# endomapper/NR-SLAM

Measured on AMD Instinct MI355X. Metric: deformable-BA LM iters/sec, higher is better.
Workload: dtype f64; 1 GPU; C2: 5000 map points x 20 keyframes, pinhole, every point a graph node; optimize(5) per step; landmarks=91749, springs=570178, dampers=512857, parallelism=1 GPU

## Files before the change

### nr-slam_amd/csrc/nrs_engine.hip

```cpp
#include <algorithm>
#include <atomic>
#include <chrono>
#include <climits>
#include <cmath>
#include <cstdlib>
#include <memory>
#include <new>
#include <system_error>
#include <thread>
#include "nrs_engine.hpp"

#include "nrs_engine_types.hpp"
#include "nrs_engine_linearize.hpp"
#include "nrs_engine_coarse.hpp"
#include "nrs_engine_pcg.hpp"
#include "nrs_engine_skin.hpp"
#include "nrs_engine_nd.hpp"
#include "nrs_engine_kft.hpp"
#include "nrs_engine_setup.hpp"
#include "nrs_engine_kft_setup.hpp"
#include "nrs_engine_devpack.hpp"

namespace nrs {

// ... 19 lines not shown
};

template <bool LIN, bool LDS>
static void launch_reg2(nrs_ctx* c, const Dev& d, const double* xl, size_t shm, int n, int cls) {
    const dim3 g(((n + 7) / 8) * 8), b(BLK);
    if constexpr (LIN && LDS) {
        if (d.plain) {
            const bool tp = d.tp_ok != 0;
            switch (d.T) {
                case 1: hipLaunchKernelGGL((k_lin_plain<1>), g, b, shm, c->stream, d, xl, cls); break;
                case 4: hipLaunchKernelGGL((k_lin_plain<4>), g, b, shm, c->stream, d, xl, cls); break;
                case 8:
                    if (tp) hipLaunchKernelGGL((k_lin_plain<8, 4, -1, true>), g, b, shm, c->stream, d, xl, cls);
                    else hipLaunchKernelGGL((k_lin_plain<8>), g, b, shm, c->stream, d, xl, cls);
                    break;
                case 16: hipLaunchKernelGGL((k_lin_plain<16>), g, b, shm, c->stream, d, xl, cls); break;
                default:
#ifdef NRS_DEBUG_PROBES
                    if (d.cam.model == 0 && tp && c->env("NRS_LIN_EXP")) {
                        switch (atoi(c->env("NRS_LIN_EXP"))) {
                            case 1: hipLaunchKernelGGL((k_lin_plain<2, 4, 0, true, 1>), g, b, shm, c->stream, d, xl, cls); break;
                            case 2: hipLaunchKernelGGL((k_lin_plain<2, 4, 0, true, 2>), g, b, shm, c->stream, d, xl, cls); break;
                            case 3: hipLaunchKernelGGL((k_lin_plain<2, 4, 0, true, 3>), g, b, shm, c->stream, d, xl, cls); break;
                            case 4: hipLaunchKernelGGL((k_lin_plain<2, 4, 0, true, 4>), g, b, shm, c->stream, d, xl, cls); break;
                            case 5: hipLaunchKernelGGL((k_lin_plain<2, 4, 0, true, 5, true>), g, b, shm, c->stream, d, xl, cls); break;
                            case 6: hipLaunchKernelGGL((k_lin_plain<2, 4, 0, true, 0, true, false, false, 4, true>), g, b, shm, c->stream, d, xl, cls); break;
                            case 7: hipLaunchKernelGGL((k_lin_plain<2, 2, 0, true, 0, true, false, false, 8>), g, b, shm, c->stream, d, xl, cls); break;
                            case 8: hipLaunchKernelGGL((k_lin_plain<2, 2, 0, true, 0, true, false, false, 10>), g, b, shm, c->stream, d, xl, cls); break;
                            case 9: hipLaunchKernelGGL((k_lin_plain<2, 3, 0, true, 0, true, false, false, 6>), g, b, shm, c->stream, d, xl, cls); break;
                            case 10: hipLaunchKernelGGL((k_lin_plain<2, 2, 0, true, 0, true, false, false, 8, true>), g, b, shm, c->stream, d, xl, cls); break;
                            default: hipLaunchKernelGGL((k_lin_plain<2, 4, 0, true, 0, true>), g, b, shm, c->stream, d, xl, cls); break;
                        }
                        break;
                    }
#endif
                    if (d.h4 && rc_of(d, cls)) {
#define NRS_LIN_RC(CAMV) switch (rc_of(d, cls)) { \
    case 1: hipLaunchKernelGGL((k_lin_plain<2, 4, CAMV, true, 0, true, true, false>), g, b, shm, c->stream, d, xl, cls); break; \
    case 2: hipLaunchKernelGGL((k_lin_plain<2, 4, CAMV, true, 0, true, false, true>), g, b, shm, c->stream, d, xl, cls); break; \
    default: hipLaunchKernelGGL((k_lin_plain<2, 4, CAMV, true, 0, true, true, true>), g, b, shm, c->stream, d, xl, cls); break; }
                        if (d.cam.model == 0) { NRS_LIN_RC(0) } else { NRS_LIN_RC(1) }
#undef NRS_LIN_RC
                    } else if (d.h4 && d.nt) {
                        if (d.cam.model == 0) hipLaunchKernelGGL((k_lin_plain<2, 4, 0, true, 0, true, false, false, 4, true>), g, b, shm, c->stream, d, xl, cls);
                        else hipLaunchKernelGGL((k_lin_plain<2, 4, 1, true, 0, true, false, false, 4, true>), g, b, shm, c->stream, d, xl, cls);
                    } else if (d.h4) {
                        if (d.cam.model == 0) hipLaunchKernelGGL((k_lin_plain<2, 4, 0, true, 0, true>), g, b, shm, c->stream, d, xl, cls);
                        else hipLaunchKernelGGL((k_lin_plain<2, 4, 1, true, 0, true>), g, b, shm, c->stream, d, xl, cls);
                    } else if (d.cam.model == 0) {
                        if (tp) hipLaunchKernelGGL((k_lin_plain<2, 4, 0, true>), g, b, shm, c->stream, d, xl, cls);
                        else hipLaunchKernelGGL((k_lin_plain<2, 4, 0, false>), g, b, shm, c->stream, d, xl, cls);
                    } else {
                        if (tp) hipLaunchKernelGGL((k_lin_plain<2, 4, 1, true>), g, b, shm, c->stream, d, xl, cls);
                        else hipLaunchKernelGGL((k_lin_plain<2, 4, 1, false>), g, b, shm, c->stream, d, xl, cls);
                    }
                    break;
            }
            return;
        }
        if (d.dform) {
            switch (d.T) {
                case 1: hipLaunchKernelGGL((k_reg<1, true, true, true>), g, b, shm, c->stream, d, xl, cls); break;
                case 4: hipLaunchKernelGGL((k_reg<4, true, true, true>), g, b, shm, c->stream, d, xl, cls); break;
                case 8: hipLaunchKernelGGL((k_reg<8, true, true, true>), g, b, shm, c->stream, d, xl, cls); break;
                case 16: hipLaunchKernelGGL((k_reg<16, true, true, true>), g, b, shm, c->stream, d, xl, cls); break;
                default: hipLaunchKernelGGL((k_reg<2, true, true, true>), g, b, shm, c->stream, d, xl, cls); break;
            }
            return;
        }
    }
    switch (d.T) {
        case 1: hipLaunchKernelGGL((k_reg<1, LIN, LDS>), g, b, shm, c->stream, d, xl, cls); break;
        case 4: hipLaunchKernelGGL((k_reg<4, LIN, LDS>), g, b, shm, c->stream, d, xl, cls); break;
        case 8: hipLaunchKernelGGL((k_reg<8, LIN, LDS>), g, b, shm, c->stream, d, xl, cls); break;
        case 16: hipLaunchKernelGGL((k_reg<16, LIN, LDS>), g, b, shm, c->stream, d, xl, cls); break;
        default: hipLaunchKernelGGL((k_reg<2, LIN, LDS>), g, b, shm, c->stream, d, xl, cls); break;
    }
}

template <bool LIN>
static void launch_reg(nrs_ctx* c, const Dev& d, const double* xl) {
    if (!d.use_lds) { launch_reg2<LIN, false>(c, d, xl, 0, d.n_regblk, 0); return; }
    for (int cls = 0; cls < 2; ++cls) {
        if (d.sh_nt[cls] == 0) continue;
        size_t shm = (LIN && d.dform) ? sizeof(double) * 9 * (size_t)(d.tile_rows + d.cap_h[cls] + 1)
                                      : sizeof(double) * 3 * (size_t)(d.tile_rows + d.cap_h[cls]) * (d.X0 ? 2 : 1);
        if (LIN) shm = std::max(shm, sizeof(double) * 4 * 64 * 8);
        launch_reg2<LIN, true>(c, d, xl, shm, d.sh_nt[cls], cls);
    }
}

template <bool LDS>
static void launch_spmv2(nrs_ctx* c, const Dev& d, double lam, size_t shm, int it) {
    const dim3 g(((d.n_regblk + 7) / 8) * 8), b(BLK);
    switch (d.T) {
        case 1: hipLaunchKernelGGL((k_spmv<1, LDS>), g, b, shm, c->stream, d, lam, it); break;
        case 4: hipLaunchKernelGGL((k_spmv<4, LDS>), g, b, shm, c->stream, d, lam, it); break;
        case 8: hipLaunchKernelGGL((k_spmv<8, LDS>), g, b, shm, c->stream, d, lam, it); break;
        case 16: hipLaunchKernelGGL((k_spmv<16, LDS>), g, b, shm, c->stream, d, lam, it); break;
        default: hipLaunchKernelGGL((k_spmv<2, LDS>), g, b, shm, c->stream, d, lam, it); break;
    }
}

static bool launch_spmv(nrs_ctx* c, const Dev& d0, double lam, int it, double tol2, bool with_skin_op = false) {
    if (!d0.use_lds) { launch_spmv2<false>(c, d0, lam, 0, it); return false; }
    bool merged = false;
    Dev d = d0;
#ifdef NRS_DEBUG_PROBES
    long long* dbg = nullptr;
    static bool dbg_done = false;
    if (d.h4 && it == 3 && !dbg_done && c->env("NRS_SPMV_DBG")) {
        dbg_done = true;
        const size_t ns = (size_t)d.n_rows / (64 / d.T);
        if (hipMalloc((void**)&dbg, sizeof(long long) * 8 * ns) == hipSuccess) { (void)hipMemsetAsync(dbg, 0, sizeof(long long) * 8 * ns, c->stream); d.dbg_clk = dbg; }
    }
    struct Dump {
        nrs_ctx* c; long long* buf; size_t ns;
        ~Dump() {
            if (!buf) return;
            (void)hipStreamSynchronize(c->stream);
            std::vector<long long> h(8 * ns);
            (void)hipMemcpy(h.data(), buf, sizeof(long long) * 8 * ns, hipMemcpyDeviceToHost);
            (void)hipFree(buf);
            double acc[5] = {0, 0, 0, 0, 0};
            long long t_min = LLONG_MAX, t_max = 0;
            size_t n = 0;
            for (size_t i = 0; i < ns; ++i) {
                const long long* q = &h[8 * i];
                if (!q[0] || !q[5]) continue;
                for (int k = 0; k < 5; ++k) acc[k] += (double)(q[k + 1] - q[k]);
                t_min = std::min(t_min, q[0]); t_max = std::max(t_max, q[5]);
                ++n;
            }
            if (n) fprintf(stderr, "[nrs] k_spmv_f phases (us per wave, mean over %zu waves): stage %.2f springs %.2f dampers %.2f row %.2f reduce %.2f | launch span %.1f us\n",
                           n, acc[0] / n / 100.0, acc[1] / n / 100.0, acc[2] / n / 100.0, acc[3] / n / 100.0, acc[4] / n / 100.0, (double)(t_max - t_min) / 100.0);
        }
    } dump{c, dbg, dbg ? (size_t)d.n_rows / (64 / d.T) : 0};
#endif
    for (int cls = 0; cls < 2; ++cls) {
        const int n = d.sh_nt[cls] + d.sh_ntb[cls];
        if (n == 0) continue;
        const dim3 g(((n + 7) / 8) * 8), b(BLK);
        if (d.dform) {
            const size_t shm = sizeof(double) * 3 * (3 * (size_t)(d.tile_rows + d.cap_h[cls] + 1) + d.tile_rows + d.cap_s[cls] + 1);
            switch (d.T) {
                case 1: hipLaunchKernelGGL((k_spmv_f<1, true>), g, b, shm, c->stream, d, lam, cls, it, tol2); break;
                case 4: hipLaunchKernelGGL((k_spmv_f<4, true>), g, b, shm, c->stream, d, lam, cls, it, tol2); break;
                case 8: hipLaunchKernelGGL((k_spmv_f<8, true>), g, b, shm, c->stream, d, lam, cls, it, tol2); break;
                case 16: hipLaunchKernelGGL((k_spmv_f<16, true>), g, b, shm, c->stream, d, lam, cls, it, tol2); break;
                default: hipLaunchKernelGGL((k_spmv_f<2, true>), g, b, shm, c->stream, d, lam, cls, it, tol2); break;
            }
            continue;
        }
        const size_t shm = sizeof(double) * 3 * (size_t)(2 * d.tile_rows + d.cap_h[cls] + ((rc_of(d, cls) & 2) ? d.cap_h[cls] : d.cap_s[cls]) + 2);
        const bool last_cls = cls == 1 || d.sh_nt[1] + d.sh_ntb[1] == 0;
        if (with_skin_op && last_cls && !(d.T == 2 && d.plain && d.tp_ok) && !c->env("NRS_SKIN_OP_OWN_LAUNCH")) {
            const dim3 g2(g.x + d.sk_nblk);
            switch (d.T) {
                case 1: hipLaunchKernelGGL((k_spmv_f_skin<1>), g2, b, shm, c->stream, d, lam, cls, it, tol2, (int)g.x); break;
                case 2: hipLaunchKernelGGL((k_spmv_f_skin<2>), g2, b, shm, c->stream, d, lam, cls, it, tol2, (int)g.x); break;
                case 4: hipLaunchKernelGGL((k_spmv_f_skin<4>), g2, b, shm, c->stream, d, lam, cls, it, tol2, (int)g.x); break;
                case 16: hipLaunchKernelGGL((k_spmv_f_skin<16>), g2, b, shm, c->stream, d, lam, cls, it, tol2, (int)g.x); break;
                default: hipLaunchKernelGGL((k_spmv_f_skin<8>), g2, b, shm, c->stream, d, lam, cls, it, tol2, (int)g.x); break;
            }
            merged = true;
            continue;
        }
        switch (d.T) {
            case 1: hipLaunchKernelGGL((k_spmv_f<1, false>), g, b, shm, c->stream, d, lam, cls, it, tol2); break;
            case 4: hipLaunchKernelGGL((k_spmv_f<4, false>), g, b, shm, c->stream, d, lam, cls, it, tol2); break;
            case 8: hipLaunchKernelGGL((k_spmv_f<8, false>), g, b, shm, c->stream, d, lam, cls, it, tol2); break;
            case 16: hipLaunchKernelGGL((k_spmv_f<16, false>), g, b, shm, c->stream, d, lam, cls, it, tol2); break;
            default:
                if (d.plain && d.tp_ok && d.h4 && rc_of(d, cls) == 1) hipLaunchKernelGGL((k_spmv_f<2, false, true, true, true, false>), g, b, shm, c->stream, d, lam, cls, it, tol2);
                else if (d.plain && d.tp_ok && d.h4 && rc_of(d, cls) == 2) hipLaunchKernelGGL((k_spmv_f<2, false, true, true, false, true>), g, b, shm, c->stream, d, lam, cls, it, tol2);
                else if (d.plain && d.tp_ok && d.h4 && rc_of(d, cls) == 3) hipLaunchKernelGGL((k_spmv_f<2, false, true, true, true, true>), g, b, shm, c->stream, d, lam, cls, it, tol2);
                else if (d.plain && d.tp_ok && d.h4 && d.nt) hipLaunchKernelGGL((k_spmv_f<2, false, true, true, false, false, true>), g, b, shm, c->stream, d, lam, cls, it, tol2);
                else if (d.plain && d.tp_ok && d.h4) hipLaunchKernelGGL((k_spmv_f<2, false, true, true>), g, b, shm, c->stream, d, lam, cls, it, tol2);
                else if (d.plain && d.tp_ok) hipLaunchKernelGGL((k_spmv_f<2, false, true>), g, b, shm, c->stream, d, lam, cls, it, tol2);
                else hipLaunchKernelGGL((k_spmv_f<2, false>), g, b, shm, c->stream, d, lam, cls, it, tol2);
                break;
        }
    }
    return merged;
}

template <bool LIN>
static int evaluate(nrs_ctx* c, Engine* e, int which, bool reproj_done = false) {
    if (LIN) { e->d.lin_pose = e->d.pose[which]; e->d.lin_xl = e->d.xl[which]; }
    const Dev& d = e->d;
    const dim3 gg(((d.sh_ng + 7) / 8) * 8), b(BLK);
#ifdef NRS_DEBUG_PROBES
    if (LIN && d.plain && c->env("NRS_LIN_DBG")) {
        static bool done = false;
        if (!done) {
            done = true;
            const size_t ns = (size_t)d.n_rows / (64 / d.T);
            long long* buf = nullptr;
            NRS_HIP(c, hipMalloc((void**)&buf, sizeof(long long) * 8 * ns));
            NRS_HIP(c, hipMemsetAsync(buf, 0, sizeof(long long) * 8 * ns, c->stream));
            Dev dd = d;
            dd.dbg_clk = buf;
            launch_reg<LIN>(c, dd, d.xl[which]);
            NRS_HIP(c, hipStreamSynchronize(c->stream));
            std::vector<long long> h(8 * ns);
            NRS_HIP(c, hipMemcpy(h.data(), buf, sizeof(long long) * 8 * ns, hipMemcpyDeviceToHost));
            (void)hipFree(buf);
            double acc[5] = {0, 0, 0, 0, 0};
            long long t_min = LLONG_MAX, t_max = 0;
            size_t n = 0;
            for (size_t i = 0; i < ns; ++i) {
                const long long* q = &h[8 * i];
                if (!q[0] || !q[5]) continue;
                for (int k = 0; k < 5; ++k) acc[k] += (double)(q[k + 1] - q[k]);
                t_min = std::min(t_min, q[0]); t_max = std::max(t_max, q[5]);
                ++n;
            }
            fprintf(stderr, "[nrs] k_lin_plain phases (us per wave, mean over %zu waves): stage %.2f springs %.2f dampers %.2f reproj %.2f tail %.2f | launch span %.1f us\n",
                    n, acc[0] / n / 100.0, acc[1] / n / 100.0, acc[2] / n / 100.0, acc[3] / n / 100.0, acc[4] / n / 100.0, (double)(t_max - t_min) / 100.0);
        }
    }
#endif
    if (LIN) {
        const int reps = c->opt.profile ? PROFILE_REPS : 1;
        Timer t(c, &c->prof.linearize_ms, &c->prof.linearize_launches, reps);
        for (int r = 0; r < reps; ++r) {
            if (!d.use_lds) hipLaunchKernelGGL((k_reproj<LIN>), gg, b, 0, c->stream, d, d.pose[which], d.xl[which]);
            launch_reg<LIN>(c, d, d.xl[which]);
        }
    } else {
        if (!reproj_done) hipLaunchKernelGGL((k_reproj<LIN>), gg, b, 0, c->stream, d, d.pose[which], d.xl[which]);
        if (d.ec_on) hipLaunchKernelGGL(k_chi_edges, dim3(std::max(1, d.ec_nblk)), b, 0, c->stream, d, d.xl[which]);
        else launch_reg<LIN>(c, d, d.xl[which]);
    }
    if (LIN) hipLaunchKernelGGL(k_pose_sums, dim3(d.sh_nk), b, 0, c->stream, d);
    if (LIN && d.coarse && !(e->nd && e->nd->on)) {
        const size_t rows = (size_t)(d.tile_rows + d.max_halo);
        const size_t shm = sizeof(double) * 3 * rows + 3 * (rows + 8) + 16;
        const dim3 g(d.n_regblk);
        switch (d.T) {
            case 1: hipLaunchKernelGGL((k_coarse_tile<1>), g, b, shm, c->stream, d); break;
            case 2: hipLaunchKernelGGL((k_coarse_tile<2>), g, b, shm, c->stream, d); break;
            case 4: hipLaunchKernelGGL((k_coarse_tile<4>), g, b, shm, c->stream, d); break;
            case 16: hipLaunchKernelGGL((k_coarse_tile<16>), g, b, shm, c->stream, d); break;
            default: hipLaunchKernelGGL((k_coarse_tile<8>), g, b, shm, c->stream, d); break;
        }
        hipLaunchKernelGGL(k_coarse_reduce, dim3(1), b, 0, c->stream, d);
    }
    if (d.sk_n > 0) hipLaunchKernelGGL((k_skin<LIN>), dim3(d.sk_nblk), b, 0, c->stream, d, d.pose[which], d.xl[which]);
    if (LIN && d.sk_pcg) {
        if (d.D_op) NRS_HIP(c, hipMemcpyAsync(d.D_op, d.D, sizeof(double) * 6 * (size_t)d.n_rows, hipMemcpyDeviceToDevice, c->stream));
        if (d.sk_nrl > 0) hipLaunchKernelGGL(k_skin_rows, dim3((d.sk_nrl + SK_RPB - 1) / SK_RPB), b, 0, c->stream, d);
        hipLaunchKernelGGL(k_skin_pose, dim3((27 * d.sh_nk + BLK - 1) / BLK), b, 0, c->stream, d);
    }
    if (LIN && e->nd && e->nd->on) {
        const NdVals& nv = e->nd->slot->vals;
        if (nv.ske_ptr) hipLaunchKernelGGL(k_nd_values<true>, dim3((nv.n_ent * ND_SKL + 255) / 256), dim3(256), 0, c->stream, d, nv);
        else hipLaunchKernelGGL(k_nd_values<false>, dim3((nv.n_ent + 255) / 256), dim3(256), 0, c->stream, d, nv);
    }
    if (d.sh_on) {
        hipLaunchKernelGGL((k_finalize_pack<LIN>), dim3(1), b, 0, c->stream, d);
        NRS_HIP(c, hipGetLastError());
        NRS_TRY(c->comm->allreduce(c, d.pk_loc, d.pk, (size_t)(2 + d.sh_world + (LIN ? 27 * d.K : 0))));
        hipLaunchKernelGGL((k_finalize_unpack<LIN>), dim3(1), b, 0, c->stream, d, ++c->seq);
    } else {
        hipLaunchKernelGGL((k_finalize<LIN>), dim3(1), b, 0, c->stream, d, ++c->seq, (e->nd && e->nd->on) ? 1 : 0);
    }
    NRS_HIP(c, hipGetLastError());
    return NRS_OK;
}

static int wait_published(nrs_ctx* c, Engine* e) {
    volatile int* w = e->h_flags + 7;
    const auto t0 = std::chrono::steady_clock::now();
    for (uint64_t spins = 0; *w != c->seq; ++spins) {
        if (spins > 200000) std::this_thread::yield();
        if ((spins & 0xFFFF) == 0xFFFF && std::chrono::steady_clock::now() - t0 > std::chrono::seconds(2)) {
            NRS_HIP(c, hipStreamSynchronize(c->stream));
            if (*w != c->seq) return c->fail(NRS_ERR_HIP, "device results were not published");
            break;
        }
    }
    std::atomic_thread_fence(std::memory_order_acquire);
    return NRS_OK;
}

static int read_scalars(nrs_ctx* c, Engine* e) { return wait_published(c, e); }

static int wait_published_at(nrs_ctx* c, const int* hf, int seq, hipStream_t st) {
    const volatile int* w = hf + 7;
    const auto t0 = std::chrono::steady_clock::now();
    for (uint64_t spins = 0; *w != seq; ++spins) {
        if (spins > 200000) std::this_thread::yield();
        if ((spins & 0xFFFF) == 0xFFFF && std::chrono::steady_clock::now() - t0 > std::chrono::seconds(2)) {
            NRS_HIP(c, hipStreamSynchronize(st));
            if (*w != seq) return c->fail(NRS_ERR_HIP, "device results were not published");
            break;
        }
    }
    std::atomic_thread_fence(std::memory_order_acquire);
    return NRS_OK;
}

static int direct_trial_enqueue(nrs_ctx* c, Engine* e, int set, double lam, int* seq, int* solve_id, bool in_batch) {
    Dev& d = e->d;
    const int cur = e->cur, trial = 1 - e->cur;
    const dim3 g(((d.sh_ng + 7) / 8) * 8), b(BLK);
    if (set < 0) {
        NRS_TRY(nd_solve_enqueue(c, e->nd->S(), lam, nullptr, solve_id, nullptr, in_batch ? c->spec_back[0] : nullptr));
        hipLaunchKernelGGL(k_apply_reproj, g, b, 0, c->stream, d, lam, d.pose[cur], d.xl[cur], d.pose[trial], d.xl[trial]);
        NRS_TRY(evaluate<false>(c, e, trial, true));
        *seq = c->seq;
        return NRS_OK;
    }
    const SpecSet& q = e->spec[set];
    struct Restore {
        nrs_ctx* c; Engine* e; Dev saved; hipStream_t main;
        ~Restore() { e->d = saved; c->stream = main; }
    } restore{c, e, d, c->stream};
    d.xv = q.xv; d.xp = q.xp; d.part_apply = q.part_apply; d.part_rchi = q.part_rchi; d.part_reg = q.part_reg; d.scal = q.scal; d.flags = q.flags;
    d.h_scal = q.h_scal; d.h_flags = q.h_flags;
    if (d.sk_n > 0) { d.sk_part = q.sk_part; d.sk_chi = q.sk_chi; }
    d.pose[trial] = q.pose; d.xl[trial] = q.xl;
    c->stream = c->spec_stream[set];
    NRS_HIP(c, hipStreamWaitEvent(c->stream, c->spec_fork, 0));
    NdDev nd = nd_alt_dev(e->nd->S(), set);
    nd.out_rows = q.xv; nd.out_pose = q.xp; nd.flags = q.flags; nd.abort = q.abort;
    NRS_TRY(nd_solve_enqueue(c, e->nd->S(), lam, &nd, solve_id, c->spec_back[set], c->spec_back[set + 1]));
    hipLaunchKernelGGL(k_apply_reproj, g, b, 0, c->stream, d, lam, d.pose[cur], d.xl[cur], q.pose, q.xl);
    NRS_TRY(evaluate<false>(c, e, trial, true));
    *seq = c->seq;
    NRS_HIP(c, hipEventRecord(c->spec_join[set], c->stream));
    return NRS_OK;
}

struct PcgSetView {
    nrs_ctx* c; Engine* e; Dev saved; hipStream_t main; double* hs; int* hf; bool on;
    PcgSetView(nrs_ctx* c_, Engine* e_, int set, int abort_id)
        : c(c_), e(e_), saved(e_->d), main(c_->stream), hs(e_->h_scal), hf(e_->h_flags), on(set >= 0) {
        if (!on) return;
        const SpecSet& q = e->spec[set];
        Dev& d = e->d;
        d.xv = q.xv; d.rv = q.rv; d.uv3 = q.uv3; d.pv = q.pv; d.sv = q.sv; d.wv = q.wv; d.Dinv = q.Dinv; d.Hppinv = q.Hppinv;
        d.xp = q.xp; d.rp = q.rp; d.rp2 = q.rp2; d.up = q.up; d.up2 = q.up2; d.pp = q.pp; d.sp = q.sp;
        d.part_spmv = q.part_spmv; d.part_ru = q.part_ru; d.red = q.red; d.part_ec = q.part_ec;
        d.part_apply = q.part_apply; d.part_rchi = q.part_rchi; d.part_reg = q.part_reg; d.scal = q.scal; d.flags = q.flags;
        d.h_scal = q.h_scal; d.h_flags = q.h_flags;
        d.pose[1 - e->cur] = q.pose; d.xl[1 - e->cur] = q.xl;
        d.abort = q.abort; d.abort_id = abort_id;
        e->h_scal = q.h_scal; e->h_flags = q.h_flags;
        c->stream = c->spec_stream[set];
    }
    ~PcgSetView() { if (on) { e->d = saved; c->stream = main; e->h_scal = hs; e->h_flags = hf; } }
    PcgSetView(const PcgSetView&) = delete;
    PcgSetView& operator=(const PcgSetView&) = delete;
};

constexpr double PEEK_RTOL = 1e-1;
constexpr int PEEK_LEVELS = 4;
constexpr double PEEK_MIN_REL_INCREASE = 1e-5;
constexpr double PEEK_RHO_LVL[5] = {0, -1.0, -0.25, -0.1, -0.03};

static int pcg_begin(nrs_ctx* c, Engine* e, double lam, int* it) {
    const Dev& d = e->d;
    NRS_HIP(c, hipMemsetAsync(d.flags, 0, sizeof(int) * 8, c->stream));
    if (d.coarse) hipLaunchKernelGGL(k_coarse_invert, dim3(1), dim3(BLK), sizeof(double) * (size_t)d.co_n * d.co_n, c->stream, d, lam);
    hipLaunchKernelGGL(k_trial_setup, dim3(d.sh_nvb), dim3(BLK), 0, c->stream, d, lam);
    if (e->kft && e->kft->on) {
        NRS_TRY(kft_factor(c, e, e->kft, lam));
        NRS_TRY(kft_apply(c, e->kft, d.rv, d.rp, d.uv3, d.up, d.flags));
        e->kft->apply_pending = false;
    }
    *it = 0;
    return NRS_OK;
}

static int pcg_enqueue_batch(nrs_ctx* c, Engine* e, double lam, int* it_io, int count = 0, int pub_seq = 0) {
    const Dev& d = e->d;
    const int n_poseblk = (d.K + 3) / 4;
    const double tol2 = c->opt.pcg_rtol * c->opt.pcg_rtol;
    int it = *it_io;
    int stop = std::min(it + (c->opt.profile ? 1 : count > 0 ? count : c->opt.pcg_batch), c->opt.pcg_max_iters);
    const bool kft_on = e->kft && e->kft->on;
    const bool kft_lazy = kft_on && it == 0 && stop > 0 && !c->opt.profile && !c->env("NRS_KFT_NO_RESIDUAL_TEST");
    if (kft_lazy) stop = 1;
    if (kft_on && e->kft->apply_pending) {
        NRS_TRY(kft_apply(c, e->kft, d.rv, ((it - 1) & 1) ? d.rp : d.rp2, d.uv3, ((it - 1) & 1) ? d.up : d.up2, d.flags));
        e->kft->apply_pending = false;
    }
    for (; it < stop; ++it) {
        const int pub = it + 1 == stop && !kft_lazy ? pub_seq : 0;
#ifdef NRS_DEBUG_PROBES
        if (d.fused && it == 20 && d.coarse && c->env("NRS_PCG_DBG")) {
            static bool dbg_done = false;
            if (!dbg_done) {
                dbg_done = true;
                long long* buf = nullptr;
                const size_t nb8 = 8 * (size_t)d.n_regblk;
                if (hipMalloc((void**)&buf, sizeof(long long) * nb8) == hipSuccess) {
                    (void)hipMemsetAsync(buf, 0, sizeof(long long) * nb8, c->stream);
                    Dev dd = d;
                    dd.dbg_clk = buf;
                    const dim3 g(((d.n_regblk + 7) / 8) * 8), bb(BLK);
                    const size_t shm = sizeof(double) * (6 * (size_t)(d.tile_rows + d.max_halo) + 12 * (size_t)d.n_regblk + 16 * CO_MAX);
                    (void)hipStreamSynchronize(c->stream);
                    std::vector<long long> h(nb8);
                    hipLaunchKernelGGL((k_pcg_fused<8, true>), g, bb, shm, c->stream, dd, lam, it, tol2, PEEK_RTOL * PEEK_RTOL, pub);
                    (void)hipStreamSynchronize(c->stream);
                    (void)hipMemcpy(h.data(), buf, sizeof(long long) * nb8, hipMemcpyDeviceToHost);
                    (void)hipFree(buf);
                    double acc[6] = {0, 0, 0, 0, 0, 0};
                    long long t_min = LLONG_MAX, t_max = 0;
                    int n = 0;
                    for (int b2 = 0; b2 < d.n_regblk; ++b2) {
                        const long long* q = &h[8 * (size_t)b2];
                        if (!q[0] || !q[6]) continue;
                        for (int k = 0; k < 6; ++k) acc[k] += (double)(q[k + 1] - q[k]);
                        t_min = std::min(t_min, q[0]); t_max = std::max(t_max, q[6]);
                        ++n;
                    }
                    if (n) fprintf(stderr, "[nrs] k_pcg_fused<8,true> phases (us per tile, mean over %d tiles): loads+pose %.2f coarse products %.2f scalars+corrections %.2f update+stage %.2f operator %.2f reduce+store %.2f | launch span %.1f us\n",
                                   n, acc[0] / n / 100.0, acc[1] / n / 100.0, acc[2] / n / 100.0, acc[3] / n / 100.0, acc[4] / n / 100.0, acc[5] / n / 100.0, (double)(t_max - t_min) / 100.0);
                    continue;
                }
            }
        }
#endif
        if (d.fused) {
            const bool one_xcd_off = c->env("NRS_NO_ONE_XCD") != nullptr;
            const bool one_xcd = !one_xcd_off && d.n_regblk <= 32;
            Dev d1 = d;
            d1.one_xcd = one_xcd ? 1 : 0;
            const Dev& d = d1;
            const dim3 g(one_xcd ? 8 * d.n_regblk : ((d.n_regblk + 7) / 8) * 8), bb(BLK);
            const size_t shm = sizeof(double) * (6 * (size_t)(d.tile_rows + d.max_halo) + (d.coarse ? 12 * (size_t)d.n_regblk + 16 * CO_MAX : 0));
            const bool check_fused = c->env("NRS_CHECK_FUSED") != nullptr;
            if (check_fused && !d.coarse && d.T == 8) {
                struct Arr { void* p; size_t bytes; const char* name; };
                const size_t nv = sizeof(double) * 3 * (size_t)d.n_rows, np6 = sizeof(double) * 6 * (size_t)d.K, npart = sizeof(double) * NPART * (size_t)d.n_regblk;
                const Arr arr[] = {{d.rv, nv, "r0"}, {d.rv2, nv, "r1"}, {d.sv, nv, "s0"}, {d.sv2, nv, "s1"}, {d.wv, nv, "w0"}, {d.wv2, nv, "w1"}, {d.xv, nv, "x"},
                                   {d.pv, nv, "p"}, {d.uv3, nv, "u"}, {d.rp, np6, "rp0"}, {d.rp2, np6, "rp1"}, {d.sp, np6, "sp0"}, {d.sp2, np6, "sp1"},
                                   {d.up, np6, "up0"}, {d.up2, np6, "up1"}, {d.pp, np6, "pp"}, {d.xp, np6, "xp"}, {d.part_spmv, npart, "part0"},
                                   {d.part_spmv2, npart, "part1"}, {d.scal, sizeof(double) * SC_N, "scal"}, {d.flags, sizeof(int) * 8, "flags"}};
                size_t total = 0;
                for (const Arr& a : arr) total += (a.bytes + 255) & ~(size_t)255;
                static char* snap = nullptr; static size_t snap_cap = 0;
                if (snap_cap < total) { if (snap) (void)hipFree(snap); NRS_HIP(c, hipMalloc((void**)&snap, total)); snap_cap = total; }
                std::vector<char> h1(total), h2(total);
                auto gather = [&](char* dst, hipMemcpyKind kind) -> int {
                    size_t o = 0;
                    for (const Arr& a : arr) { NRS_HIP(c, hipMemcpyAsync(dst + o, a.p, a.bytes, kind, c->stream)); o += (a.bytes + 255) & ~(size_t)255; }
                    NRS_HIP(c, hipStreamSynchronize(c->stream));
                    return NRS_OK;
                };
                NRS_TRY(gather(snap, hipMemcpyDeviceToDevice));
                hipLaunchKernelGGL((k_pcg_fused<8, false>), g, bb, shm, c->stream, d, lam, it, tol2, PEEK_RTOL * PEEK_RTOL, pub);
                NRS_TRY(gather(h1.data(), hipMemcpyDeviceToHost));
                { size_t o = 0; for (const Arr& a : arr) { NRS_HIP(c, hipMemcpyAsync(a.p, snap + o, a.bytes, hipMemcpyDeviceToDevice, c->stream)); o += (a.bytes + 255) & ~(size_t)255; } }
                hipLaunchKernelGGL((k_pcg_fused<8, false>), g, bb, shm, c->stream, d, lam, it, tol2, PEEK_RTOL * PEEK_RTOL, pub);
                NRS_TRY(gather(h2.data(), hipMemcpyDeviceToHost));
                size_t o = 0;
                bool any = false;
                for (const Arr& a : arr) {
                    if (memcmp(h1.data() + o, h2.data() + o, a.bytes) != 0) {
                        any = true;
                        const size_t nel = a.bytes / 8;
                        size_t ndiff = 0, first = 0, last = 0;
                        for (size_t el = 0; el < nel; ++el)
                            if (memcmp(h1.data() + o + 8 * el, h2.data() + o + 8 * el, 8) != 0) { if (!ndiff) first = el; last = el; ++ndiff; }
                        double v1, v2; memcpy(&v1, h1.data() + o + 8 * first, 8); memcpy(&v2, h2.data() + o + 8 * first, 8);
                        fprintf(stderr, "[nrs] fused launch it %d: array %s differs in %zu elements, first %zu (tile %zu) last %zu (tile %zu): %.6g / %.6g\n", it, a.name, ndiff, first,
                                first / 3 / (size_t)d.tile_rows, last, last / 3 / (size_t)d.tile_rows, v1, v2);
                    }
                    o += (a.bytes + 255) & ~(size_t)255;
                }
                if (any) {
                    const size_t o_fl = total - 256, o_sc = o_fl - ((sizeof(double) * SC_N + 255) & ~(size_t)255);
                    const int* f1 = reinterpret_cast<const int*>(h1.data() + o_fl); const int* f2 = reinterpret_cast<const int*>(h2.data() + o_fl);
                    const int* f0 = nullptr; (void)f0;
                    fprintf(stderr, "[nrs]    flags after run 1: %d %d %d %d | run 2: %d %d %d %d ; scal gamma0 %.6g/%.6g slot0 %.6g %.6g / %.6g %.6g slot1 %.6g %.6g / %.6g %.6g\n", f1[0], f1[1], f1[2], f1[3], f2[0], f2[1], f2[2], f2[3],
                            reinterpret_cast<const double*>(h1.data() + o_sc)[SC_GAMMA0], reinterpret_cast<const double*>(h2.data() + o_sc)[SC_GAMMA0],
                            reinterpret_cast<const double*>(h1.data() + o_sc)[SC_SLOT0], reinterpret_cast<const double*>(h1.data() + o_sc)[SC_SLOT0 + 1],
                            reinterpret_cast<const double*>(h2.data() + o_sc)[SC_SLOT0], reinterpret_cast<const double*>(h2.data() + o_sc)[SC_SLOT0 + 1],
                            reinterpret_cast<const double*>(h1.data() + o_sc)[SC_SLOT1], reinterpret_cast<const double*>(h1.data() + o_sc)[SC_SLOT1 + 1],
                            reinterpret_cast<const double*>(h2.data() + o_sc)[SC_SLOT1], reinterpret_cast<const double*>(h2.data() + o_sc)[SC_SLOT1 + 1]);
                }
            } else
            switch (d.T) {
                case 1: if (d.coarse) hipLaunchKernelGGL((k_pcg_fused<1, true>), g, bb, shm, c->stream, d, lam, it, tol2, PEEK_RTOL * PEEK_RTOL, pub);
                        else hipLaunchKernelGGL((k_pcg_fused<1, false>), g, bb, shm, c->stream, d, lam, it, tol2, PEEK_RTOL * PEEK_RTOL, pub);
                        break;
                case 2: if (d.coarse) hipLaunchKernelGGL((k_pcg_fused<2, true>), g, bb, shm, c->stream, d, lam, it, tol2, PEEK_RTOL * PEEK_RTOL, pub);
                        else hipLaunchKernelGGL((k_pcg_fused<2, false>), g, bb, shm, c->stream, d, lam, it, tol2, PEEK_RTOL * PEEK_RTOL, pub);
                        break;
                case 4: if (d.coarse) hipLaunchKernelGGL((k_pcg_fused<4, true>), g, bb, shm, c->stream, d, lam, it, tol2, PEEK_RTOL * PEEK_RTOL, pub);
                        else hipLaunchKernelGGL((k_pcg_fused<4, false>), g, bb, shm, c->stream, d, lam, it, tol2, PEEK_RTOL * PEEK_RTOL, pub);
// ... 539 lines not shown
```

### nr-slam_amd/csrc/nrs_engine_devpack.hpp

```cpp
#pragma once
#include <rocprim/rocprim.hpp>

namespace nrs {

constexpr int DP_HCAP = 2048, DP_HASH = 4096;

__device__ inline uint64_t dp_spread(uint64_t v) {
    v &= 0x1fffff;
    v = (v | v << 32) & 0x1f00000000ffffULL;
    v = (v | v << 16) & 0x1f0000ff0000ffULL;
    v = (v | v << 8) & 0x100f00f00f00f00fULL;
    v = (v | v << 4) & 0x10c30c30c30c30c3ULL;
    v = (v | v << 2) & 0x1249249249249249ULL;
    return v;
}

__global__ __launch_bounds__(1024) void k_dp_minmax(int M, const double* __restrict__ xyz, double* out ) {
    __shared__ double lo[3][1024], hi[3][1024];
    const int tid = threadIdx.x;
    double l[3] = {1e300, 1e300, 1e300}, h[3] = {-1e300, -1e300, -1e300};
    for (int v = tid; v < M; v += 1024)
        for (int a = 0; a < 3; ++a) { const double p = xyz[3 * (size_t)v + a]; l[a] = fmin(l[a], p); h[a] = fmax(h[a], p); }
    for (int a = 0; a < 3; ++a) { lo[a][tid] = l[a]; hi[a][tid] = h[a]; }
    __syncthreads();
// ... 562 lines not shown
    NRS_HIP(c, hipMemsetAsync(S_side, 0, nnz_s, st));
    NRS_HIP(c, hipMemsetAsync(D_o, 0xFF, sizeof(int) * 3 * nnz_d, st));
    NRS_HIP(c, hipMemsetAsync(D_role, 0xFF, nnz_d, st));
    NRS_HIP(c, hipMemsetAsync(d_flag, 0, sizeof(int) * 16, st));
    NRS_HIP(c, hipMemsetAsync(t_d0, 0, sizeof(float) * nnz_s, st));
    NRS_HIP(c, hipMemsetAsync(t_w, 0, sizeof(float) * nnz_d, st));
    hipLaunchKernelGGL(k_dp_fill_s, nb(ni_s), dim3(256), 0, st, ni_s, T, key_s2, rs_s, d_ss, r_sp, r_d0, vrow, S_other, t_d0, S_side);
    hipLaunchKernelGGL(k_dp_fill_d, nb(ni_d), dim3(256), 0, st, ni_d, T, key_d2, rs_d, d_sd, r_dm, r_w, vrow, D_o, t_w, D_role);
    hipLaunchKernelGGL((k_dp_halo<0>), dim3(n_tiles), dim3(256), 0, st, d.tile_rows, T, (uint16_t*)nullptr, d_ss, d_sd, S_other, S_side, D_o, D_role, hs, hns, (const int*)nullptr,
                       (int*)nullptr, (uint32_t*)nullptr, (uint2*)nullptr, d_flag);
    std::vector<int> h_hs(n_tiles), h_hns(n_tiles), h_vrow(M);
    int h_flag = 0;
    NRS_HIP(c, hipMemcpyAsync(h_hs.data(), hs, sizeof(int) * n_tiles, hipMemcpyDeviceToHost, st));
    NRS_HIP(c, hipMemcpyAsync(h_hns.data(), hns, sizeof(int) * n_tiles, hipMemcpyDeviceToHost, st));
    NRS_HIP(c, hipMemcpyAsync(&h_flag, d_flag, sizeof(int), hipMemcpyDeviceToHost, st));
    NRS_HIP(c, hipMemcpyAsync(h_vrow.data(), vrow, sizeof(int) * (size_t)M, hipMemcpyDeviceToHost, st));
    NRS_HIP(c, hipStreamSynchronize(st));
    mark("fill + halo sizes");
    if (h_flag) return NRS_OK;
    std::vector<int> halo_ptr(n_tiles + 1, 0), tile_list(n_tiles);
    d.max_halo = 0; d.max_halo_s = 0;
    for (int b = 0; b < n_tiles; ++b) {
        halo_ptr[b + 1] = halo_ptr[b] + h_hs[b];
        d.max_halo = std::max(d.max_halo, h_hs[b]);
        d.max_halo_s = std::max(d.max_halo_s, h_hns[b]);
    }
    const size_t n_halo = (size_t)halo_ptr[n_tiles];
    {
        std::vector<int> sorted = h_hs;
        std::sort(sorted.begin(), sorted.end());
        int cut = d.max_halo;
        if (n_tiles >= 1024) {
            const int p97 = sorted[(size_t)(0.97 * (n_tiles - 1))];
            const bool fits = sizeof(double) * 3 * (size_t)(2 * d.tile_rows + d.max_halo + d.max_halo_s + 2) <= 48 * 1024;
            if (4 * d.max_halo > 5 * p97 && (n_tiles - (int)(0.97 * n_tiles) >= 1024 || !fits) && !c->env("NRS_ONE_CLASS")) cut = p97;
        }
        int n0 = 0;
        for (int b = 0; b < n_tiles; ++b) if (h_hs[b] <= cut) tile_list[n0++] = b;
        int n1 = n0;
        for (int b = 0; b < n_tiles; ++b) if (h_hs[b] > cut) tile_list[n1++] = b;
        d.n_tiles_cls[0] = n0; d.n_tiles_cls[1] = n_tiles - n0;
        for (int b = 0; b < n_tiles; ++b) {
            const int cls = h_hs[b] <= cut ? 0 : 1;
            d.cap_h[cls] = std::max(d.cap_h[cls], h_hs[b]);
            d.cap_s[cls] = std::max(d.cap_s[cls], h_hns[b]);
        }
    }
    size_t lds_need = 0;
    for (int cls = 0; cls < 2; ++cls) {
        if (!d.n_tiles_cls[cls]) continue;
        lds_need = std::max(lds_need, sizeof(double) * 3 * (size_t)(d.tile_rows + d.cap_h[cls]));
        lds_need = std::max(lds_need, sizeof(double) * 3 * (size_t)(2 * d.tile_rows + d.cap_h[cls] + d.cap_s[cls] + 2));
    }
    if (lds_need > 64 * 1024 - 512 || d.tile_rows + d.max_halo >= 65535) return NRS_OK;
    d.use_lds = 1; d.dform = 0; d.coarse = 0;
    d.fused = d.n_rows < 32768 ? 1 : 0;
    d.hier = n_tiles > 4096 ? 1 : 0;
    d.ecd = (!d.fused && !c->opt.profile) ? 1 : 0;
    d.co_n = 3 * d.n_groups + 6;
    d.sh_on = 0; d.sh_rank = 0; d.sh_world = 1; d.sh_lead = 1;
    d.sh_k0 = 0; d.sh_nk = K; d.sh_g0 = 0; d.sh_ng = d.n_groups; d.sh_vb0 = 0; d.sh_nvb = d.n_vecblk;
    for (int cls = 0; cls < 2; ++cls) { d.sh_t0[cls] = 0; d.sh_nt[cls] = d.n_tiles_cls[cls]; }
    d.ec_on = 1; d.plain = 1;
    d.lin_rb = ROW_ALIGN / (64 / T);
    d.ec_nsp = n_sp; d.ec_ndm = n_dm;
    d.ec_nblk = std::min((n_sp + n_dm + BLK - 1) / BLK, 2048);
    e->pack_rows = n_rows;
    if (tm) fprintf(stderr, "[nrs] device pack: tiles %d x %d rows, halo rows: max %d, mean %.1f, spring part max %d, classes %d (cap %d/%d) + %d (cap %d/%d)\n", n_tiles, d.tile_rows,
                    d.max_halo, (double)n_halo / n_tiles, d.max_halo_s, d.n_tiles_cls[0], d.cap_h[0], d.cap_s[0], d.n_tiles_cls[1], d.cap_h[1], d.cap_s[1]);
    ArenaPlan dry{arena, true};
    {
        Dev tmpd = d;
        Engine te;
        spec_pcg_sets(c, e, 0);
        te.n_spec = e->n_spec; te.spec_pcg = e->spec_pcg;
        carve(dry, tmpd, false, nnz_s, nnz_d, (size_t)n_slices, n_halo, &te);
    }
    if (dry.off > arena->cap) {
        arena_release(arena);
        const size_t want = dry.off + dry.off / 8;
        hipError_t he = hipMalloc((void**)&arena->base, want);
        if (he != hipSuccess) return c->fail(NRS_ERR_ALLOC, "hipMalloc(%zu) failed: %s", want, hipGetErrorString(he));
        arena->cap = want;
        if (c->env("NRS_POISON")) { (void)hipMemset(arena->base, 0xFF, want); (void)hipDeviceSynchronize(); }
    }
    ArenaPlan real{arena, false};
    carve(real, d, false, nnz_s, nnz_d, (size_t)n_slices, n_halo, e);
    e->arena_bytes = real.off;
    mark("arena");
    NRS_HIP(c, hipMemcpyAsync(d.grp_pose, grp_pose.data(), sizeof(int) * grp_pose.size(), hipMemcpyHostToDevice, st));
    NRS_HIP(c, hipMemcpyAsync(d.pose_grp_ptr, pose_grp_ptr.data(), sizeof(int) * (K + 1), hipMemcpyHostToDevice, st));
    NRS_HIP(c, hipMemcpyAsync(d.halo_ptr, halo_ptr.data(), sizeof(int) * (n_tiles + 1), hipMemcpyHostToDevice, st));
    NRS_HIP(c, hipMemcpyAsync(d.tile_list, tile_list.data(), sizeof(int) * n_tiles, hipMemcpyHostToDevice, st));
    NRS_HIP(c, hipMemcpyAsync(d.halo_ns, hns, sizeof(int) * n_tiles, hipMemcpyDeviceToDevice, st));
    NRS_HIP(c, hipMemcpyAsync(d.ss_ptr, d_ss, sizeof(int) * ((size_t)n_slices + 1), hipMemcpyDeviceToDevice, st));
    NRS_HIP(c, hipMemcpyAsync(d.sd_ptr, d_sd, sizeof(int) * ((size_t)n_slices + 1), hipMemcpyDeviceToDevice, st));
    NRS_HIP(c, hipMemcpyAsync(d.s_d0, t_d0, sizeof(float) * nnz_s, hipMemcpyDeviceToDevice, st));
    NRS_HIP(c, hipMemcpyAsync(d.d_w, t_w, sizeof(float) * nnz_d, hipMemcpyDeviceToDevice, st));
    std::vector<Pose> poses(s.poses, s.poses + K);
    NRS_HIP(c, hipMemcpyAsync(d.pose_init, poses.data(), sizeof(Pose) * K, hipMemcpyHostToDevice, st));
    NRS_HIP(c, hipMemsetAsync(d.pose_fixed, 0, K, st));
    NRS_HIP(c, hipMemsetAsync(d.row_tp, 0xFF, sizeof(uint32_t) * (size_t)n_rows, st));
    hipLaunchKernelGGL((k_dp_halo<1>), dim3(n_tiles), dim3(256), 0, st, d.tile_rows, T, reinterpret_cast<uint16_t*>(d.row_tp), d.ss_ptr, d.sd_ptr, S_other, S_side, D_o, D_role, hs, hns, d.halo_ptr,
                       d.halo_rows, d.s_om, d.d_hdr, d_flag);
    if (d.fused) {
        std::vector<int> tile_desc(8 * (size_t)n_tiles, 0);
        const int rb = ROW_ALIGN / d.tile_rows;
        for (int b = 0; b < n_tiles; ++b) {
            const int kf = grp_pose[(size_t)b * d.tile_rows / ROW_ALIGN];
            int* td = &tile_desc[8 * (size_t)b];
            td[0] = kf; td[1] = pose_grp_ptr[kf] * rb; td[2] = pose_grp_ptr[kf + 1] * rb;
            td[3] = halo_ptr[b]; td[4] = halo_ptr[b + 1] - halo_ptr[b];
        }
        NRS_HIP(c, hipMemcpyAsync(d.tile_desc, tile_desc.data(), sizeof(int) * tile_desc.size(), hipMemcpyHostToDevice, st));
        hipLaunchKernelGGL(k_dp_halofix, dim3(n_tiles), dim3(BLK), 0, st, n_tiles, d.halo_ptr, d.halo_rows, d.halo_fix, BLK, 0);
        NRS_HIP(c, hipStreamSynchronize(st));
    } else if (d.use_lds)
        hipLaunchKernelGGL(k_dp_halofix, dim3(n_tiles), dim3(BLK), 0, st, n_tiles, d.halo_ptr, d.halo_rows, d.halo_fix, HALO_FIX, -1);
    hipLaunchKernelGGL(k_dp_rowdata, nb(n_rows), dim3(256), 0, st, n_rows, row_v, r_x, r_uv, d.rflag, d.uv, d.xl_init);
    hipLaunchKernelGGL(k_dp_rowcnt, nb(n_rows), dim3(256), 0, st, n_rows, cnt_s, cnt_d, d.row_cnt);
    hipLaunchKernelGGL(k_dp_eckeys, nb(std::max(n_sp, n_dm)), dim3(256), 0, st, n_sp, r_sp, n_dm, r_dm, vrow, ek_s, ek_d);
    tb = tmp_bytes; NRS_HIP(c, rocprim::radix_sort_keys(tmp, tb, ek_s, ek_s2, (size_t)n_sp, 0, 32 + row_bits, st));
    tb = tmp_bytes; NRS_HIP(c, rocprim::radix_sort_keys(tmp, tb, ek_d, ek_d2, (size_t)n_dm, 0, 32 + row_bits, st));
    hipLaunchKernelGGL(k_dp_ecfill, nb(std::max(n_sp, n_dm)), dim3(256), 0, st, n_sp, ek_s2, r_sp, r_d0, n_dm, ek_d2, r_dm, r_w, vrow, d.ec_sp, d.ec_dm, d.ec_w);
    NRS_HIP(c, hipMemsetAsync(d.s_qc, 0, sizeof(double) * nnz_s, st));
    NRS_HIP(c, hipMemsetAsync(d.d_s, 0, sizeof(double) * nnz_d, st));
    NRS_HIP(c, hipMemsetAsync(d.part_apply, 0, sizeof(double) * (size_t)d.n_vecblk, st));
    NRS_HIP(c, hipMemsetAsync(d.scal, 0, sizeof(double) * SC_N, st));
    NRS_HIP(c, hipMemsetAsync(d.flags, 0, sizeof(int) * 8, st));
    NRS_HIP(c, hipGetLastError());
    e->vrow.swap(h_vrow);
    e->h_rflag.assign(n_rows, RF_FIXED);
    for (int v = 0; v < M; ++v) e->h_rflag[e->vrow[v]] = RF_OBS | RF_REPROJ_ACTIVE;
    e->h_pose_fixed.assign(K, 0);
    e->dev_edges = true;
    e->raw_sp = r_sp; e->raw_d0 = r_d0; e->raw_dm = r_dm; e->raw_w = r_w;
    e->serial = ++c->engine_serial;
    if (!c->pin_scal) NRS_HIP(c, hipHostMalloc((void**)&c->pin_scal, sizeof(double) * SC_N, hipHostMallocMapped | hipHostMallocCoherent));
    if (!c->pin_flags) {
        NRS_HIP(c, hipHostMalloc((void**)&c->pin_flags, sizeof(int) * 8, hipHostMallocMapped | hipHostMallocCoherent));
        memset(c->pin_flags, 0, sizeof(int) * 8);
    }
    e->h_scal = c->pin_scal; e->h_flags = c->pin_flags;
    d.h_scal = c->pin_scal; d.h_flags = c->pin_flags;
    if (e->n_spec > 0) NRS_TRY(spec_prepare(c, e));
    NRS_HIP(c, hipStreamSynchronize(st));
    int h_fl2[2] = {0, 0};
    NRS_HIP(c, hipMemcpy(h_fl2, d_flag, sizeof(int) * 2, hipMemcpyDeviceToHost));
    if (h_fl2[0]) return c->fail(NRS_ERR_HIP, "device pack: halo hash overflow in the second pass");
    d.tp_ok = h_fl2[1] ? 0 : 1;
    if (c->pack_ws2.cap > ((size_t)512 << 20)) c->release(c->pack_ws2);
    mark("final arrays");
    engine_compact_headers(c, e);
    NRS_TRY(engine_reset(c, e));
    *done = true;
    return NRS_OK;
}

}
```

### nr-slam_amd/csrc/nrs_engine_linearize.hpp

```cpp
#pragma once

namespace nrs {

template <bool LIN>
__global__ __launch_bounds__(BLK) void k_reproj(Dev P, const Pose* __restrict__ poses,
                                                const double* __restrict__ xl) {
    __shared__ double lds[4 * 28];
    const int gi = xcd_tile(blockIdx.x, P.sh_ng);
    if (gi >= P.sh_ng) return;
    const int g = P.sh_g0 + gi;
    const int tid = threadIdx.x, lane = tid & 63, wave = tid >> 6;
    const int row = g * ROW_ALIGN + tid;
    const int kf = P.grp_pose[g];
    const Pose Tcw = poses[kf];
    const bool pfix = P.pose_fixed[kf] != 0;
    double R[9];
    quat_to_R(Tcw.q, R);
    double acc[28];
#pragma unroll
    for (int k = 0; k < 28; ++k) acc[k] = 0;
    const int rf = P.rflag[row];
    const bool rfix = (rf & RF_FIXED) != 0;
    const bool active = (rf & RF_OBS) && (rf & RF_REPROJ_ACTIVE) && !(pfix && rfix);
    bool wrote = false;
// ... 430 lines not shown
            double* Dr = P.D + 6 * (size_t)row;
            double dd[6];
            if (LDS) {
#pragma unroll
                for (int k = 0; k < 6; ++k) { dd[k] = D[k]; Dr[k] = dd[k]; }
#pragma unroll
                for (int k = 0; k < 3; ++k) P.bl[3 * row + k] = bb[k];
            } else {
#pragma unroll
                for (int k = 0; k < 6; ++k) { dd[k] = Dr[k] + D[k]; Dr[k] = dd[k]; }
#pragma unroll
                for (int k = 0; k < 3; ++k) P.bl[3 * row + k] += bb[k];
            }
            part[1] = fmax(fabs(dd[0]), fmax(fabs(dd[3]), fabs(dd[5])));
        }
    }
    double c = wave_sum(part[0]);
    double m = part[1];
#pragma unroll
    for (int off = 32; off > 0; off >>= 1) m = fmax(m, __shfl_xor(m, off, 64));
    if (lane == 0) { lds[wave * 2] = c; lds[wave * 2 + 1] = m; }
    __syncthreads();
    if (tid == 0) {
        P.part_reg[2 * (size_t)b] = lds[0] + lds[2] + lds[4] + lds[6];
        P.part_reg[2 * (size_t)b + 1] = fmax(fmax(lds[1], lds[3]), fmax(lds[5], lds[7]));
    }
}

__device__ inline double fast_rcp_pos(double a) {
    double y = __builtin_amdgcn_rcp(a);
    double e = fma(-a, y, 1.0);
    y = fma(y, e, y);
    e = fma(-a, y, 1.0);
    return fma(y, e, y);
}
__device__ inline double fast_rsqrt_pos(double a) {
    const double y = __builtin_amdgcn_rsq(a);
    const double e = fma(-a * y, y, 1.0);
    return fma(y * e, fma(e, 0.375, 0.5), y);
}
__device__ inline double fast_sqrt_pos(double a) {
    const double y = __builtin_amdgcn_rsq(a);
    double g = a * y, h = 0.5 * y;
    const double e = fma(-h, g, 0.5);
    g = fma(g, e, g);
    h = fma(h, e, h);
    const double e2 = fma(-g, g, a);
    return fma(e2, h, g);
}

__device__ inline double sq3(double a, double b, double c) { return fma(c, c, fma(b, b, a * a)); }
__device__ inline double spring_qc(double d2, double d0, double ks, double ip) {
#pragma clang fp contract(off)
    const double c = 2.0 * ks * fast_rcp_pos(d0);
    return ip * (c * c) * fast_rsqrt_pos(d2);
}
__device__ inline double damper_s(double g0, double g1, double g2, double w, double isp, double dsp, double& rho0) {
#pragma clang fp contract(off)
    const double r0 = w * g0, r1 = w * g1, r2 = w * g2;
    const double e = isp * sq3(r0, r1, r2), dsqr = dsp * dsp;
    const bool act = dsp > 0 && e > dsqr;
    const double ea = act ? e : 1.0, y = fast_rsqrt_pos(ea);
    rho0 = act ? 2.0 * (ea * y) * dsp - dsqr : e;
    return (act ? dsp * y : 1.0) * isp * w * w;
}

template <int T, int OCC = 4, int CAM = -1, bool TPC = false, int EXP = 0, bool H4 = false, bool RCS = false, bool RCD = false, int NBT = 4, bool NT = false>
__global__ __launch_bounds__(BLK, OCC) void k_lin_plain(Dev P, const double* __restrict__ xl_g, int cls) {
    __shared__ double mfb[4 * 128];
    __shared__ double spose[8];
    extern __shared__ double dyn[];
    constexpr int R = 64 / T;
    int b = xcd_tile(blockIdx.x, P.sh_nt[cls]);
    if (b >= P.sh_nt[cls]) return;
    b = P.tile_list[(cls ? P.n_tiles_cls[0] : 0) + P.sh_t0[cls] + b];
    const int tid = threadIdx.x, lane = tid & 63, wave = __builtin_amdgcn_readfirstlane(tid >> 6);
    const int slice = b * 4 + wave;
    const int row = slice * R + lane / T;
    const int t = lane % T;
    auto stamp = [&](int k) { if (P.dbg_clk && lane == 0) P.dbg_clk[(size_t)slice * 8 + k] = wall_clock64(); };
    stamp(0);
    const uint32_t rcn = P.row_cnt[row];
    const int my_s = ((int)(rcn & 0xFFFFu) + T - 1 - t) / T, my_d = ((int)(rcn >> 16) + T - 1 - t) / T;
    if (tid < 7) spose[tid] = reinterpret_cast<const double*>(P.lin_pose + P.grp_pose[row / ROW_ALIGN])[tid];
    const int s_beg = P.ss_ptr[slice], s_end = P.ss_ptr[slice + 1];
    const int d_beg = P.sd_ptr[slice], d_end = EXP == 5 ? P.sd_ptr[slice] + (((P.sd_ptr[slice + 1] - P.sd_ptr[slice]) / 64 + 1) / 2) * 64 : P.sd_ptr[slice + 1];
    constexpr int NB = NBT;
    uint32_t rs_om[NB], rs_d0[NB];
    auto req_s = [&](int q, int idx) {
        if (EXP == 3) { rs_om[q] = (uint32_t)(idx & 63) | 0x10000u; rs_d0[q] = 0x3F800000u; return; }
        rs_om[q] = 0xFFFFu; rs_d0[q] = 0x3F800000u;
        if ((idx - s_beg - lane) / 64 < my_s) {
            if (NT) { rs_om[q] = __builtin_nontemporal_load(P.s_om + idx); rs_d0[q] = __float_as_uint(__builtin_nontemporal_load(P.s_d0 + idx)); }
            else { rs_om[q] = P.s_om[idx]; rs_d0[q] = __float_as_uint(P.s_d0[idx]); }
        }
    };
#pragma unroll
    for (int q = 0; q < NB; ++q) req_s(q, s_beg + lane + 64 * q);
    __builtin_amdgcn_sched_barrier(0);
    double* lx = dyn;
    if (P.fused) stage_rows(P, b, tid, xl_g, nullptr, lx);
    else stage_rows<true>(P, b, tid, xl_g, nullptr, lx);
    __syncthreads();
    stamp(1);
    const int self = row - b * P.tile_rows;
    const double xo0 = lx[3 * self], xo1 = lx[3 * self + 1], xo2 = lx[3 * self + 2];
    double D0 = 0, D1 = 0, D2 = 0, D3 = 0, D4 = 0, D5 = 0, bb0 = 0, bb1 = 0, bb2 = 0, chi = 0;
    const double ks = P.k_spring, ip = P.info_pos;
    auto do_s = [&](int o16, bool live, bool count, float d0f, int idx) {
        const bool pad = !live || o16 == REC_NONE;
        const int o = EXP == 2 ? self : (pad ? self : o16) & 0xFFFF;
        const double v0 = xo0 - lx[3 * o], v1 = xo1 - lx[3 * o + 1], v2 = xo2 - lx[3 * o + 2];
        double d2 = sq3(v0, v1, v2);
        d2 = pad ? 1.0 : d2;
        const double d0 = pad ? 1.0 : (double)d0f;
        const double rs = fast_rsqrt_pos(d2), id0 = fast_rcp_pos(d0);
        const double r = ks * fma(d2, rs, -d0) * id0;
        const double cg = 2.0 * ks * id0 * fast_sqrt_pos(rs);
        const double qc = pad ? 0.0 : spring_qc(d2, d0, ks, ip);
        if (live && EXP != 1 && !RCS) { if (NT) __builtin_nontemporal_store(qc, P.s_qc + idx); else P.s_qc[idx] = qc; }
        chi += count && !pad ? ip * r * r : 0.0;
        const double t0 = qc * v0, t1 = qc * v1, t2 = qc * v2;
        D0 = fma(t0, v0, D0); D1 = fma(t0, v1, D1); D2 = fma(t0, v2, D2);
        D3 = fma(t1, v1, D3); D4 = fma(t1, v2, D4); D5 = fma(t2, v2, D5);
        const double qr = ip * r * cg;
        bb0 = fma(-qr, v0, bb0); bb1 = fma(-qr, v1, bb1); bb2 = fma(-qr, v2, bb2);
    };
    for (int ub = s_beg; ub < (EXP == 4 ? s_beg : s_end); ub += 64 * NB) {
        const int base = ub + lane;
        if (ub != s_beg) {
#pragma unroll
            for (int q = 0; q < NB; ++q) req_s(q, base + 64 * q);
        }
        __builtin_amdgcn_sched_barrier(0);
#pragma unroll
        for (int q = 0; q < NB; ++q) {
            const uint32_t om = consume(rs_om[q]);
            const float d0f = __uint_as_float(consume(rs_d0[q]));
            do_s((int)(om & 0xFFFFu), base + 64 * q < s_end, (om & ((uint32_t)SR_COUNT << 16)) != 0, d0f, base + 64 * q);
        }
        __builtin_amdgcn_sched_barrier(0);
    }
    stamp(2);
    double en0 = 0, en1 = 0, en2 = 0, ep0 = 0, ep1 = 0, ep2 = 0;
    if (TPC) {
        const uint32_t tp = P.row_tp[row];
        const int tn = (int)(tp & 0xFFFFu) == REC_NONE ? self : (int)(tp & 0xFFFFu), tq = (int)(tp >> 16) == REC_NONE ? self : (int)(tp >> 16);
        en0 = xo0 - lx[3 * tn]; en1 = xo1 - lx[3 * tn + 1]; en2 = xo2 - lx[3 * tn + 2];
        ep0 = xo0 - lx[3 * tq]; ep1 = xo1 - lx[3 * tq + 1]; ep2 = xo2 - lx[3 * tq + 2];
    }
    const double isp = P.info_spatial, dsp = P.delta_spatial;
    uint32_t rd_w[NB];
    uint2 rd_h[NB];
    auto req_d = [&](int q, int idx) {
        if (EXP == 3) { rd_h[q] = make_uint2((uint32_t)(idx & 63) | ((uint32_t)((idx + 1) & 63) << 16), (uint32_t)((idx + 2) & 63) | 0x80000u); rd_w[q] = 0x3F800000u; return; }
        rd_h[q] = make_uint2(0xFFFFFFFFu, 0xFFFFFFFFu); rd_w[q] = 0u;
        if (H4) { if ((idx - d_beg - lane) / 64 < my_d) {
            if (NT) { rd_h[q].x = __builtin_nontemporal_load(P.d_h4 + idx); rd_w[q] = __float_as_uint(__builtin_nontemporal_load(P.d_w + idx)); }
            else { rd_h[q].x = P.d_h4[idx]; rd_w[q] = __float_as_uint(P.d_w[idx]); } } }
        else if ((idx - d_beg - lane) / 64 < my_d) { rd_h[q] = P.d_hdr[idx]; rd_w[q] = __float_as_uint(P.d_w[idx]); }
    };
    auto do_d = [&](uint32_t hx, uint32_t hy, float wf, int idx) {
        const uint32_t m16 = H4 ? (hx == 0xFFFFFFFFu ? (uint32_t)REC_NONE : hx >> 24) : hy >> 16;
        const bool live = idx < d_end;
        const bool pad = !live || m16 == REC_NONE;
        const int o0 = EXP == 2 ? self : (pad ? self : (int)(hx & (H4 ? 0xFFFu : 0xFFFFu))) & 0xFFFF, o1 = EXP == 2 || H4 ? self : (pad ? self : (int)(hx >> 16)) & 0xFFFF,
                  o2 = EXP == 2 ? self : (pad ? self : (int)(H4 ? (hx >> 12) & 0xFFFu : hy & 0xFFFFu)) & 0xFFFF;
        double g0, g1, g2;
        if (TPC) {
            const bool fwd = (m16 & 2u) == 0;
            g0 = (fwd ? en0 : ep0) - (lx[3 * o0] - lx[3 * o2]);
            g1 = (fwd ? en1 : ep1) - (lx[3 * o0 + 1] - lx[3 * o2 + 1]);
            g2 = (fwd ? en2 : ep2) - (lx[3 * o0 + 2] - lx[3 * o2 + 2]);
        } else {
            g0 = (xo0 - lx[3 * o1]) - (lx[3 * o0] - lx[3 * o2]);
            g1 = (xo1 - lx[3 * o1 + 1]) - (lx[3 * o0 + 1] - lx[3 * o2 + 1]);
            g2 = (xo2 - lx[3 * o1 + 2]) - (lx[3 * o0 + 2] - lx[3 * o2 + 2]);
        }
        const double w = pad ? 0.0 : (double)wf;
        double rho0;
        const double sfac = damper_s(g0, g1, g2, w, isp, dsp, rho0);
        chi += (m16 & DM_COUNT) ? rho0 : 0.0;
        if (live && EXP != 1 && !RCD) { if (NT) __builtin_nontemporal_store(sfac, P.d_s + idx); else P.d_s[idx] = sfac; }
        D0 += sfac; D3 += sfac; D5 += sfac;
        bb0 = fma(-sfac, g0, bb0); bb1 = fma(-sfac, g1, bb1); bb2 = fma(-sfac, g2, bb2);
    };
    for (int ub = d_beg; ub < (EXP == 4 ? d_beg : d_end); ub += 64 * NB) {
        const int base = ub + lane;
#pragma unroll
        for (int q = 0; q < NB; ++q) req_d(q, base + 64 * q);
        __builtin_amdgcn_sched_barrier(0);
#pragma unroll
        for (int q = 0; q < NB; ++q) {
            const uint32_t hx = consume(rd_h[q].x), hy = H4 ? 0u : consume(rd_h[q].y);
            const float wf = __uint_as_float(consume(rd_w[q]));
            do_d(hx, hy, wf, base + 64 * q);
        }
        __builtin_amdgcn_sched_barrier(0);
    }
    stamp(3);
    constexpr int NRR = T == 1 ? 2 : 1;
    const int rf = P.rflag[row];
    const float uvx = P.uv[2 * row], uvy = P.uv[2 * row + 1];
    const bool active = (rf & RF_OBS) && (rf & RF_REPROJ_ACTIVE);
    RowRec rc;
#pragma unroll
    for (int q = 0; q < 6; ++q) rc.J[q] = 0.f;
    rc.w = 0;
    double Jp[NRR][6], rres[NRR], w = 0, chi_r = 0;
#pragma unroll
    for (int a = 0; a < NRR; ++a) {
        rres[a] = 0;
#pragma unroll
        for (int q = 0; q < 6; ++q) Jp[a][q] = 0;
    }
    if (active && t < (T == 1 ? 1 : 2)) {
        Pose Tcw;
#pragma unroll
        for (int q = 0; q < 4; ++q) Tcw.q[q] = spose[q];
#pragma unroll
        for (int q = 0; q < 3; ++q) Tcw.t[q] = spose[4 + q];
        double Rm[9];
        quat_to_R(Tcw.q, Rm);
        const double px = Rm[0] * xo0 + Rm[1] * xo1 + Rm[2] * xo2 + Tcw.t[0];
        const double py = Rm[3] * xo0 + Rm[4] * xo1 + Rm[5] * xo2 + Tcw.t[1];
        const double pz = Rm[6] * xo0 + Rm[7] * xo1 + Rm[8] * xo2 + Tcw.t[2];
        float u, v, Jf[6];
        Cam cam = P.cam;
        if (CAM >= 0) cam.model = CAM;
        project_f32(cam, (float)px, (float)py, (float)pz, u, v);
        projection_jacobian_f32(cam, (float)px, (float)py, (float)pz, Jf);
        const double r2[2] = {(double)uvx - (double)u, (double)uvy - (double)v};
        double rho0, rho1;
        huber(P.info_reproj * (r2[0] * r2[0] + r2[1] * r2[1]), P.delta_reproj, rho0, rho1);
        if (t == 0) chi_r = rho0;
        w = rho1 * P.info_reproj;
#pragma unroll
        for (int a = 0; a < NRR; ++a) {
            const int rr = T == 1 ? a : t;
            const double j0 = -(double)(rr ? Jf[3] : Jf[0]), j1 = -(double)(rr ? Jf[4] : Jf[1]), j2 = -(double)(rr ? Jf[5] : Jf[2]);
            const double r = rr ? r2[1] : r2[0];
            rres[a] = r;
            Jp[a][0] = -j1 * pz + j2 * py;
            Jp[a][1] = j0 * pz - j2 * px;
            Jp[a][2] = -j0 * py + j1 * px;
            Jp[a][3] = j0; Jp[a][4] = j1; Jp[a][5] = j2;
            const double Jl0 = j0 * Rm[0] + j1 * Rm[3] + j2 * Rm[6];
            const double Jl1 = j0 * Rm[1] + j1 * Rm[4] + j2 * Rm[7];
            const double Jl2 = j0 * Rm[2] + j1 * Rm[5] + j2 * Rm[8];
            D0 += w * (Jl0 * Jl0); D1 += w * (Jl0 * Jl1); D2 += w * (Jl0 * Jl2);
            D3 += w * (Jl1 * Jl1); D4 += w * (Jl1 * Jl2); D5 += w * (Jl2 * Jl2);
            bb0 -= w * (Jl0 * r); bb1 -= w * (Jl1 * r); bb2 -= w * (Jl2 * r);
        }
        if (t == 0) {
#pragma unroll
            for (int q = 0; q < 6; ++q) rc.J[q] = Jf[q];
            rc.w = w;
        }
    }
    if (t == 0) P.rowrec[row] = rc;
    stamp(4);
    double* slot = P.part_lin + (size_t)slice * 32;
    {
        typedef double v4d __attribute__((ext_vector_type(4)));
        double* mb = mfb + wave * 128;
        const int e = lane & 15, kk = lane >> 4;
        v4d acc = {0.0, 0.0, 0.0, 0.0};
#pragma unroll
        for (int a = 0; a < NRR; ++a) {
#pragma unroll
            for (int c4 = 0; c4 < 4; ++c4) {
                __builtin_amdgcn_fence(__ATOMIC_ACQ_REL, "wavefront");
                __builtin_amdgcn_wave_barrier();
                if (kk == c4) {
#pragma unroll
                    for (int q = 0; q < 6; ++q) mb[e * 8 + q] = Jp[a][q];
                    mb[e * 8 + 6] = -rres[a];
                    mb[e * 8 + 7] = w;
                }
                __builtin_amdgcn_fence(__ATOMIC_RELEASE, "wavefront");
                __builtin_amdgcn_wave_barrier();
                __builtin_amdgcn_fence(__ATOMIC_ACQUIRE, "wavefront");
#pragma unroll
                for (int m = 0; m < 4; ++m) {
                    const int kq = 4 * m + kk;
                    const double val = e < 7 ? mb[kq * 8 + e] : 0.0;
                    const double av = e < 6 ? mb[kq * 8 + 7] * val : 0.0;
                    acc = __builtin_amdgcn_mfma_f64_16x16x4f64(av, val, acc, 0, 0, 0);
                }
            }
        }
        auto put = [&](int prow, double c) {
            if (prow < 6) {
                if (e >= prow && e < 6) slot[prow * 6 - (prow * (prow - 1)) / 2 + (e - prow)] = c;
                if (e == 6) slot[21 + prow] = c;
            }
        };
        put(kk, acc.x);
        put(4 + kk, acc.y);
    }
    D0 = sub_sum_t<T>(D0); D1 = sub_sum_t<T>(D1); D2 = sub_sum_t<T>(D2);
    D3 = sub_sum_t<T>(D3); D4 = sub_sum_t<T>(D4); D5 = sub_sum_t<T>(D5);
    bb0 = sub_sum_t<T>(bb0); bb1 = sub_sum_t<T>(bb1); bb2 = sub_sum_t<T>(bb2);
    double md = 0;
    if (t == 0) {
        double* Dr = P.D + 6 * (size_t)row;
        Dr[0] = D0; Dr[1] = D1; Dr[2] = D2; Dr[3] = D3; Dr[4] = D4; Dr[5] = D5;
        P.bl[3 * row] = bb0; P.bl[3 * row + 1] = bb1; P.bl[3 * row + 2] = bb2;
        md = fmax(fabs(D0), fmax(fabs(D3), fabs(D5)));
    }
    const double cr = wave_sum(chi_r), cg2 = wave_sum(chi);
#pragma unroll
    for (int off = 32; off > 0; off >>= 1) md = fmax(md, __shfl_xor(md, off, 64));
    if (lane == 0) { slot[27] = cr; slot[28] = cg2; slot[29] = md; }
    stamp(5);
}

__global__ __launch_bounds__(BLK) void k_chi_edges(Dev P, const double* __restrict__ xl) {
    __shared__ double lds[4];
    if (spec_aborted(P)) return;
    const int tid = threadIdx.x, n = P.ec_nsp + P.ec_ndm;
    const int per = (int)((((int64_t)n + P.ec_nblk - 1) / P.ec_nblk + BLK - 1) / BLK) * BLK;
    const int64_t beg = (int64_t)blockIdx.x * per;
    const int end = (int)(beg + per < n ? beg + per : n);
    double rho[1] = {0};
    for (int i = (int)beg + tid; i < end; i += BLK) {
        double r0v, rho1;
        if (i < P.ec_nsp) {
            const EcSpring s = P.ec_sp[i];
            const double v0 = xl[3 * (size_t)s.a] - xl[3 * (size_t)s.b], v1 = xl[3 * (size_t)s.a + 1] - xl[3 * (size_t)s.b + 1],
                         v2 = xl[3 * (size_t)s.a + 2] - xl[3 * (size_t)s.b + 2];
            const double d = sqrt(v0 * v0 + v1 * v1 + v2 * v2), d0 = (double)s.d0;
            const double r = P.k_spring * (d - d0) / d0;
            huber(P.info_pos * r * r, P.delta_pos, r0v, rho1);
        } else {
            const EcDamper dd = P.ec_dm[i - P.ec_nsp];
            const double w = (double)P.ec_w[i - P.ec_nsp];
            double s0 = 0, s1 = 0, s2 = 0;
#pragma unroll
            for (int k = 0; k < 4; ++k) {
                if (dd.r[k] >= 0) {
                    const double sg = damper_sign(k);
                    s0 += sg * xl[3 * (size_t)dd.r[k]]; s1 += sg * xl[3 * (size_t)dd.r[k] + 1]; s2 += sg * xl[3 * (size_t)dd.r[k] + 2];
                }
            }
            const double r0 = w * s0, r1 = w * s1, r2 = w * s2;
            huber(P.info_spatial * (r0 * r0 + r1 * r1 + r2 * r2), P.delta_spatial, r0v, rho1);
        }
        rho[0] += r0v;
// ... 165 lines not shown
```

### nr-slam_amd/csrc/nrs_engine_pcg.hpp

```cpp
#pragma once

namespace nrs {

__device__ inline bool inv6_spd(const double* Hu, double lam, double* Ainv ) {
    double L[6][6];
    double A[6][6];
    int k = 0;
    for (int i = 0; i < 6; ++i)
        for (int j = i; j < 6; ++j) { A[i][j] = Hu[k]; A[j][i] = Hu[k]; ++k; }
    for (int i = 0; i < 6; ++i) A[i][i] += lam;
    for (int i = 0; i < 6; ++i)
        for (int j = 0; j < 6; ++j) L[i][j] = 0;
    bool ok = true;
    for (int j = 0; j < 6; ++j) {
        double d = A[j][j];
        for (int q = 0; q < j; ++q) d -= L[j][q] * L[j][q];
        if (!(d > 0)) { ok = false; d = 1; }
        const double l = sqrt(d);
        L[j][j] = l;
        for (int i = j + 1; i < 6; ++i) {
            double s = A[i][j];
            for (int q = 0; q < j; ++q) s -= L[i][q] * L[j][q];
            L[i][j] = s / l;
        }
    }
    for (int c = 0; c < 6; ++c) {
        double y[6], x[6];
        for (int i = 0; i < 6; ++i) {
            double s = (i == c) ? 1.0 : 0.0;
            for (int q = 0; q < i; ++q) s -= L[i][q] * y[q];
            y[i] = s / L[i][i];
        }
        for (int i = 5; i >= 0; --i) {
            double s = y[i];
            for (int q = i + 1; q < 6; ++q) s -= L[q][i] * x[q];
            x[i] = s / L[i][i];
        }
        for (int i = 0; i < 6; ++i) Ainv[i * 6 + c] = x[i];
    }
    return ok;
}

__global__ __launch_bounds__(BLK) void k_trial_setup(Dev P, double lam) {
    __shared__ double lds_ru[4];
    if (spec_aborted(P)) return;
    const int i = (P.sh_vb0 + blockIdx.x) * BLK + threadIdx.x;
    double ru[1] = {0};
    if (i < P.n_rows) {
        double Di[6];
        const bool ok = inv3_sym(P.D + 6 * (size_t)i, lam, Di);
        if (!ok || !isfinite(Di[0])) P.flags[2] = 1;
#pragma unroll
        for (int k = 0; k < 6; ++k) P.Dinv[6 * (size_t)i + k] = Di[k];
        const double r0 = P.bl[3 * i], r1 = P.bl[3 * i + 1], r2 = P.bl[3 * i + 2];
        P.rv[3 * i] = r0; P.rv[3 * i + 1] = r1; P.rv[3 * i + 2] = r2;
        double y0 = 0, y1 = 0, y2 = 0;
        if (P.coarse && !(P.rflag[i] & RF_FIXED)) {
            const int g = i / ROW_ALIGN, tl = i / P.tile_rows;
            double yt[3];
            tile_level(P.co_bti + 6 * (size_t)tl, P.co_tb + 4 * (size_t)tl, yt);
            y0 = P.co_y0[3 * g] + yt[0]; y1 = P.co_y0[3 * g + 1] + yt[1]; y2 = P.co_y0[3 * g + 2] + yt[2];
        }
        const double u0 = Di[0] * r0 + Di[1] * r1 + Di[2] * r2 + y0;
        const double u1 = Di[1] * r0 + Di[3] * r1 + Di[4] * r2 + y1;
        const double u2 = Di[2] * r0 + Di[4] * r1 + Di[5] * r2 + y2;
        P.uv3[3 * i] = u0; P.uv3[3 * i + 1] = u1; P.uv3[3 * i + 2] = u2;
        ru[0] = r0 * u0 + r1 * u1 + r2 * u2;
#pragma unroll
        for (int k = 0; k < 3; ++k) { P.xv[3 * i + k] = 0; P.pv[3 * i + k] = 0; P.sv[3 * i + k] = 0; }
    }
    if (blockIdx.x * BLK + threadIdx.x < P.K) {
        const int i = blockIdx.x * BLK + threadIdx.x;
        double Ai[36];
        if (!inv6_spd(P.Hpp + 21 * i, lam, Ai)) P.flags[2] = 1;
        for (int k = 0; k < 36; ++k) P.Hppinv[36 * i + k] = Ai[k];
        for (int a = 0; a < 6; ++a) {
            double s = 0;
            for (int c = 0; c < 6; ++c) s += Ai[a * 6 + c] * P.bp[6 * i + c];
            if (P.coarse && !P.pose_fixed[i]) s += P.co_y0[3 * P.n_groups + a];
            P.up[6 * i + a] = s;
            P.rp[6 * i + a] = P.bp[6 * i + a];
            P.xp[6 * i + a] = 0; P.pp[6 * i + a] = 0; P.sp[6 * i + a] = 0;
        }
    }
    if (P.ecd) {
        block_sum<1>(ru, lds_ru, threadIdx.x & 63, threadIdx.x >> 6);
        if (threadIdx.x == 0) P.part_ru[P.sh_vb0 + blockIdx.x] = ru[0];
    }
}

template <int T, bool LDS>
__global__ __launch_bounds__(BLK) void k_spmv(Dev P, double lam, int it) {
    static_assert(!LDS, "gather fallback only: the LDS-staged path is k_spmv_f");
    __shared__ double lds[4 * 9];
    constexpr int R = 64 / T;
    const int b = xcd_tile(blockIdx.x, P.n_regblk);
    if (b >= P.n_regblk) return;
    const int tid = threadIdx.x, lane = tid & 63, wave = tid >> 6;
    const int slice = b * 4 + wave;
    const int row = slice * R + lane / T;
    const int t = lane % T;
    const bool rfix = (P.rflag[row] & RF_FIXED) != 0;
    const double* u = P.uv3;
    const int self = row;
    double a0 = 0, a1 = 0, a2 = 0;
    double part[9] = {0, 0, 0, 0, 0, 0, 0, 0, 0};
    const double ul0 = u[3 * self], ul1 = u[3 * self + 1], ul2 = u[3 * self + 2];
    {
        const int kf = P.grp_pose[row / ROW_ALIGN];
        if (t == 0) {
            const double* D = (P.D_op ? P.D_op : P.D) + 6 * (size_t)row;
            a0 = (D[0] + lam) * ul0 + D[1] * ul1 + D[2] * ul2;
            a1 = D[1] * ul0 + (D[3] + lam) * ul1 + D[4] * ul2;
            a2 = D[2] * ul0 + D[4] * ul1 + (D[5] + lam) * ul2;
        }
        double h0 = 0, h1 = 0, h2 = 0;
#pragma unroll
        for (int p = t; p < 6; p += T) {
            const double upk = ((it & 1) ? P.up2 : P.up)[6 * kf + p];
            const double e0 = P.Hpl[(size_t)(p * 3) * P.n_rows + row];
            const double e1 = P.Hpl[(size_t)(p * 3 + 1) * P.n_rows + row];
            const double e2 = P.Hpl[(size_t)(p * 3 + 2) * P.n_rows + row];
            h0 += e0 * upk; h1 += e1 * upk; h2 += e2 * upk;
            part[3 + p] = e0 * ul0 + e1 * ul1 + e2 * ul2;
        }
        a0 += h0; a1 += h1; a2 += h2;
        part[2] = ul0 * h0 + ul1 * h1 + ul2 * h2;
    }
    if (!rfix) {
        const int beg = P.ss_ptr[slice], end = P.ss_ptr[slice + 1];
        const size_t nz = (size_t)P.ss_nnz;
        for (int idx = beg + lane; idx < end; idx += 64) {
            const int o = P.s_other[idx];
            if (o < 0) continue;
            const double g0 = P.s_g[idx], g1 = P.s_g[nz + idx], g2 = P.s_g[2 * nz + idx];
            const double dot = g0 * u[3 * o] + g1 * u[3 * o + 1] + g2 * u[3 * o + 2];
            a0 -= g0 * dot; a1 -= g1 * dot; a2 -= g2 * dot;
        }
    }
    if (!rfix) {
        const int beg = P.sd_ptr[slice], end = P.sd_ptr[slice + 1];
        for (int idx = beg + lane; idx < end; idx += 64) {
            const int meta = P.d_meta[idx];
            if (meta < 0 || (meta & DM_UNARY)) continue;
            const int o[3] = {P.d_o0[idx], P.d_o1[idx], P.d_o2[idx]};
            const int role = meta & 3;
            double s0 = 0, s1 = 0, s2 = 0;
#pragma unroll
            for (int k = 0; k < 3; ++k) {
                const double sg = damper_sign(k + (k >= role ? 1 : 0));
                if (o[k] >= 0) { s0 += sg * u[3 * o[k]]; s1 += sg * u[3 * o[k] + 1]; s2 += sg * u[3 * o[k] + 2]; }
            }
            const double c = damper_sign(role) * P.d_s[idx];
            a0 += c * s0; a1 += c * s1; a2 += c * s2;
        }
    }
    a0 = sub_sum_t<T>(a0); a1 = sub_sum_t<T>(a1); a2 = sub_sum_t<T>(a2);
    if (t == 0) {
        P.wv[3 * row] = a0; P.wv[3 * row + 1] = a1; P.wv[3 * row + 2] = a2;
        part[0] = P.rv[3 * row] * ul0 + P.rv[3 * row + 1] * ul1 + P.rv[3 * row + 2] * ul2;
        part[1] = a0 * ul0 + a1 * ul1 + a2 * ul2;
    }
    block_sum_store<9>(part, lds, tid, P.part_spmv + (size_t)b * NPART);
}

template <int T, bool DF, bool TPC = false, bool H4 = false, bool RCS = false, bool RCD = false, bool NT = false>
__device__ __forceinline__ void spmv_f_body(const Dev& P, const double lam, const int cls, const int it, const double tol2, const int blk) {
    static_assert(!(RCS || RCD) || (TPC && H4 && !DF), "factor recomputation: plain windows with cached partners and 4-byte headers");
    __shared__ double lds[4 * 9];
    extern __shared__ double dyn[];
    constexpr int R = 64 / T;
    constexpr int U = 2;
    const int bi = xcd_tile(blk, P.sh_nt[cls] + P.sh_ntb[cls]);
    if (bi >= P.sh_nt[cls] + P.sh_ntb[cls]) return;
    const int b = P.tile_list[(cls ? P.n_tiles_cls[0] : 0) + (bi < P.sh_nt[cls] ? P.sh_t0[cls] + bi : P.sh_t0b[cls] + bi - P.sh_nt[cls])];
    const int tid = threadIdx.x, lane = tid & 63, wave = __builtin_amdgcn_readfirstlane(tid >> 6);
    const int slice = b * 4 + wave;
    const int row = slice * R + lane / T;
    const int t = lane % T;
    auto stamp = [&](int k) { if (H4 && P.dbg_clk && lane == 0) P.dbg_clk[(size_t)slice * 8 + k] = wall_clock64(); };
    stamp(0);
    const bool rfix = (P.rflag[row] & RF_FIXED) != 0;
    const uint32_t tp = TPC ? P.row_tp[row] : 0u;
    const uint32_t rcn = TPC ? P.row_cnt[row] : 0u;
    const int my_s = ((int)(rcn & 0xFFFFu) + T - 1 - t) / T, my_d = ((int)(rcn >> 16) + T - 1 - t) / T;
    const int kf = P.grp_pose[row / ROW_ALIGN];
    const int sbeg = P.ss_ptr[slice], send = rfix ? sbeg : P.ss_ptr[slice + 1];
    const int dbeg = P.sd_ptr[slice], dend = rfix ? dbeg : P.sd_ptr[slice + 1];
    const size_t nst = (size_t)(P.tile_rows + P.cap_h[cls] + 1);
    double* lu = dyn;
    double* lgf = dyn + 3 * nst;
    double* lgb = dyn + 6 * nst;
    double* lx = dyn + (DF ? 9 : 3) * nst;
    const int ZROW = P.tile_rows + P.cap_h[cls], ZROWX = RCD ? ZROW : P.tile_rows + P.cap_s[cls];
    if (tid < 3) {
        lu[3 * ZROW + tid] = 0; lx[3 * ZROWX + tid] = 0;
        if (DF) { lgf[3 * ZROW + tid] = 0; lgb[3 * ZROW + tid] = 0; }
    }
    double gsum = 0;
    if (P.ecd) {
        const double* pr = P.part_ru + (size_t)(it & 1) * P.n_vecblk;
        if (P.hier) { if (tid == 0) gsum = P.red[3 + 6 * P.K]; }
        else for (int i = tid; i < P.n_vecblk; i += BLK) gsum += pr[i];
        const double* upp = (it & 1) ? P.up2 : P.up;
        const double* rpp = (it & 1) ? P.rp2 : P.rp;
        for (int i = tid; i < 6 * P.K; i += BLK) gsum += rpp[i] * upp[i];
        gsum = wave_sum(gsum);
        if (lane == 0) lds[wave] = gsum;
    }
    const double gamma0 = P.scal[SC_GAMMA0];
    const int done_flag = P.flags[0] | (P.abort && *reinterpret_cast<const volatile int*>(P.abort) == P.abort_id);
    if (DF) {
        stage_rows_d(P, b, tid, P.uv3, lu, lgf, lgb);
        const int row0 = b * P.tile_rows, hb = P.halo_ptr[b], ns = P.halo_ns[b];
        for (int i = tid; i < P.tile_rows + ns; i += BLK) {
            const size_t r = 3 * (size_t)(i < P.tile_rows ? row0 + i : P.halo_rows[hb + i - P.tile_rows]);
            lx[3 * i] = P.lin_xl[r]; lx[3 * i + 1] = P.lin_xl[r + 1]; lx[3 * i + 2] = P.lin_xl[r + 2];
        }
    } else stage_rows2<TPC, RCD>(P, b, tid, P.uv3, P.lin_xl, P.X0, lu, lx);
    RowRec rc;
    rc.w = 0;
    double rv0 = 0, rv1 = 0, rv2 = 0;
    if (t == 0) {
        rc = P.rowrec[row];
        if (!P.ecd) { rv0 = P.rv[3 * row]; rv1 = P.rv[3 * row + 1]; rv2 = P.rv[3 * row + 2]; }
    }
    const int send_u = P.ss_ptr[slice + 1], dend_u = P.sd_ptr[slice + 1];
    const int s_last = max(send_u - 1, 0), d_last = max(dend_u - 1, 0);
    uint32_t somA[U], somB[U], sd0A[U], sd0B[U];
    double sqcA[U], sqcB[U], dsA[U], dsB[U];
    uint2 dhA[U], dhB[U];
    auto load_springs = [&](uint32_t* om, double* qc, uint32_t* d0w, int idx) {
#pragma unroll
        for (int q = 0; q < U; ++q) {
            if (TPC) {
                om[q] = 0xFFFFu; qc[q] = 0.0;
                if (RCS) { d0w[q] = 0x3F800000u; if ((idx + 64 * q - sbeg - lane) / 64 < my_s) { om[q] = P.s_om[idx + 64 * q]; d0w[q] = __float_as_uint(P.s_d0[idx + 64 * q]); } continue; }
                if ((idx + 64 * q - sbeg - lane) / 64 < my_s) {
                    if (NT) { om[q] = __builtin_nontemporal_load(P.s_om + idx + 64 * q); qc[q] = __builtin_nontemporal_load(P.s_qc + idx + 64 * q); }
                    else { om[q] = P.s_om[idx + 64 * q]; qc[q] = P.s_qc[idx + 64 * q]; }
                }
                continue;
            }
            const int j = min(idx + 64 * q, s_last);
            om[q] = P.s_om[j];
            qc[q] = P.s_qc[j];
        }
    };
    auto load_dampers = [&](uint2* h, double* sv, int idx) {
#pragma unroll
        for (int q = 0; q < U; ++q) {
            if (TPC) {
                h[q] = make_uint2(0xFFFFFFFFu, 0xFFFFFFFFu); sv[q] = 0.0;
                if (H4 && RCD) { if ((idx + 64 * q - dbeg - lane) / 64 < my_d) { h[q].x = P.d_h4[idx + 64 * q]; h[q].y = __float_as_uint(P.d_w[idx + 64 * q]); } }
                else if (H4) { if ((idx + 64 * q - dbeg - lane) / 64 < my_d) {
                    if (NT) { h[q].x = __builtin_nontemporal_load(P.d_h4 + idx + 64 * q); sv[q] = __builtin_nontemporal_load(P.d_s + idx + 64 * q); }
                    else { h[q].x = P.d_h4[idx + 64 * q]; sv[q] = P.d_s[idx + 64 * q]; } } }
                else if ((idx + 64 * q - dbeg - lane) / 64 < my_d) { h[q] = P.d_hdr[idx + 64 * q]; sv[q] = P.d_s[idx + 64 * q]; }
                continue;
            }
            const int j = min(idx + 64 * q, d_last);
            if (DF) h[q] = make_uint2(P.d_om[j], 0u);
            else h[q] = P.d_hdr[j];
            sv[q] = P.d_s[j];
        }
    };
    load_springs(somA, sqcA, sd0A, sbeg + lane);
    load_dampers(dhA, dsA, dbeg + lane);
    __builtin_amdgcn_sched_barrier(0);
    const int done_wg = __syncthreads_or(done_flag);
    stamp(1);
    if (done_wg && !(H4 && P.dbg_clk)) return;
    if (P.ecd && it > 0) {
        const double gamma = lds[0] + lds[1] + lds[2] + lds[3];
        const bool bad = !isfinite(gamma);
        if (gamma <= tol2 * gamma0 || bad || gamma == 0.0) {
            if (blk == 0 && tid == 0 && cls == 0) {
                if (bad) P.flags[2] = 1;
                P.flags[1] = it;
                __threadfence();
                P.flags[0] = 1;
            }
            return;
        }
        __syncthreads();
    }
    const int self = row - b * P.tile_rows;
    const double ul[3] = {lu[3 * self], lu[3 * self + 1], lu[3 * self + 2]};
    const double xs[3] = {lx[3 * self], lx[3 * self + 1], lx[3 * self + 2]};
    double a0 = 0, a1 = 0, a2 = 0;
    double en[3] = {0, 0, 0}, ep[3] = {0, 0, 0}, exn[3] = {0, 0, 0}, exq[3] = {0, 0, 0};
    const double ks = P.k_spring, ip = P.info_pos, isp = P.info_spatial;
    if (TPC) {
        const int tn = (int)(tp & 0xFFFFu) == REC_NONE ? ZROW : (int)(tp & 0xFFFFu), tq = (int)(tp >> 16) == REC_NONE ? ZROW : (int)(tp >> 16);
#pragma unroll
        for (int k = 0; k < 3; ++k) { en[k] = ul[k] - lu[3 * tn + k]; ep[k] = ul[k] - lu[3 * tq + k]; }
        if (RCD) {
            const int xn = (int)(tp & 0xFFFFu) == REC_NONE ? self : (int)(tp & 0xFFFFu), xq = (int)(tp >> 16) == REC_NONE ? self : (int)(tp >> 16);
#pragma unroll
            for (int k = 0; k < 3; ++k) { exn[k] = xs[k] - lx[3 * xn + k]; exq[k] = xs[k] - lx[3 * xq + k]; }
        }
    }
    auto do_springs = [&](const uint32_t* om, const double* qcv, const uint32_t* d0w, int idx) {
#pragma unroll
        for (int q = 0; q < U; ++q) {
            const int o16 = (int)(consume(om[q]) & 0xFFFFu);
            const bool pad = idx + 64 * q >= send || o16 == REC_NONE;
            const int o = pad ? ZROW : o16, ox = pad ? ZROWX : o16;
            double qc = pad || RCS ? 0.0 : consume(qcv[q]);
            const double v0 = xs[0] - lx[3 * ox], v1 = xs[1] - lx[3 * ox + 1], v2 = xs[2] - lx[3 * ox + 2];
            if (RCS) { const double d2 = sq3(v0, v1, v2); qc = pad ? 0.0 : spring_qc(pad ? 1.0 : d2, (double)__uint_as_float(consume(d0w[q])), ks, ip); }
            const double dot = qc * (v0 * (ul[0] - lu[3 * o]) + v1 * (ul[1] - lu[3 * o + 1]) + v2 * (ul[2] - lu[3 * o + 2]));
            a0 += dot * v0; a1 += dot * v1; a2 += dot * v2;
        }
    };
    const double gfo[3] = {DF ? lgf[3 * self] : 0.0, DF ? lgf[3 * self + 1] : 0.0, DF ? lgf[3 * self + 2] : 0.0};
    const double gbo[3] = {DF ? lgb[3 * self] : 0.0, DF ? lgb[3 * self + 1] : 0.0, DF ? lgb[3 * self + 2] : 0.0};
    auto do_dampers = [&](const uint2* hd, const double* dsv, int idx) {
#pragma unroll
        for (int q = 0; q < U; ++q) {
            const bool live = idx + 64 * q < dend;
            if (DF) {
                const uint32_t hx = consume(hd[q].x);
                const int p16 = (int)(hx & 0xFFFFu), m16 = (int)(hx >> 16);
                const bool pad = !live || m16 == REC_NONE || p16 == REC_NONE;
                const int o = pad ? ZROW : p16;
                const double sv = pad ? 0.0 : consume(dsv[q]);
                const bool bw = (m16 & 2) != 0;
                const double* lg = bw ? lgb : lgf;
                const double g0 = (bw ? gbo[0] : gfo[0]) - lg[3 * o], g1 = (bw ? gbo[1] : gfo[1]) - lg[3 * o + 1], g2 = (bw ? gbo[2] : gfo[2]) - lg[3 * o + 2];
                a0 += sv * g0; a1 += sv * g1; a2 += sv * g2;
                continue;
            }
            const uint32_t hx = consume(hd[q].x), hy = H4 ? 0u : consume(hd[q].y);
            const int r0 = (int)(hx & (H4 ? 0xFFFu : 0xFFFFu)), r1 = H4 ? 0 : (int)(hx >> 16), r2 = (int)(H4 ? (hx >> 12) & 0xFFFu : hy & 0xFFFFu),
                      m16 = H4 ? (hx == 0xFFFFFFFFu ? (int)REC_NONE : (int)(hx >> 24)) : (int)(hy >> 16);
            const bool pad = !live || m16 == REC_NONE;
            double sv = pad || RCD ? 0.0 : consume(dsv[q]);
            const bool un = pad || (m16 & DM_UNARY) != 0;
            const int o0 = H4 ? (pad ? ZROW : r0) : (un || r0 == REC_NONE) ? ZROW : r0;
            const int o1 = (un || r1 == REC_NONE) ? ZROW : r1;
            const int o2 = H4 ? (pad ? ZROW : r2) : (un || r2 == REC_NONE) ? ZROW : r2;
            double g0, g1, g2;
            if (TPC) {
                const bool fwd = (m16 & 2) == 0;
                g0 = (fwd ? en[0] : ep[0]) - (lu[3 * o0] - lu[3 * o2]);
                g1 = (fwd ? en[1] : ep[1]) - (lu[3 * o0 + 1] - lu[3 * o2 + 1]);
                g2 = (fwd ? en[2] : ep[2]) - (lu[3 * o0 + 2] - lu[3 * o2 + 2]);
                if (RCD) {
                    const double x0 = (fwd ? exn[0] : exq[0]) - (lx[3 * o0] - lx[3 * o2]), x1 = (fwd ? exn[1] : exq[1]) - (lx[3 * o0 + 1] - lx[3 * o2 + 1]),
                                 x2 = (fwd ? exn[2] : exq[2]) - (lx[3 * o0 + 2] - lx[3 * o2 + 2]);
                    double rho0;
                    sv = pad ? 0.0 : damper_s(x0, x1, x2, (double)__uint_as_float(consume(hd[q].y)), isp, P.delta_spatial, rho0);
                }
            } else {
                g0 = (ul[0] - lu[3 * o1]) - (lu[3 * o0] - lu[3 * o2]);
                g1 = (ul[1] - lu[3 * o1 + 1]) - (lu[3 * o0 + 1] - lu[3 * o2 + 1]);
                g2 = (ul[2] - lu[3 * o1 + 2]) - (lu[3 * o0 + 2] - lu[3 * o2 + 2]);
            }
            a0 += sv * g0; a1 += sv * g1; a2 += sv * g2;
        }
    };
    for (int base = sbeg; base < send_u; base += 128 * U) {
        load_springs(somB, sqcB, sd0B, base + 64 * U + lane);
        __builtin_amdgcn_sched_barrier(0);
        do_springs(somA, sqcA, sd0A, base + lane);
        __builtin_amdgcn_sched_barrier(0);
        load_springs(somA, sqcA, sd0A, base + 128 * U + lane);
        __builtin_amdgcn_sched_barrier(0);
        do_springs(somB, sqcB, sd0B, base + 64 * U + lane);
        __builtin_amdgcn_sched_barrier(0);
    }
    stamp(2);
    for (int base = dbeg; base < dend_u; base += 128 * U) {
        load_dampers(dhB, dsB, base + 64 * U + lane);
        __builtin_amdgcn_sched_barrier(0);
        do_dampers(dhA, dsA, base + lane);
        __builtin_amdgcn_sched_barrier(0);
        load_dampers(dhA, dsA, base + 128 * U + lane);
        __builtin_amdgcn_sched_barrier(0);
        do_dampers(dhB, dsB, base + 64 * U + lane);
        __builtin_amdgcn_sched_barrier(0);
    }
    stamp(3);
    double part[9] = {0, 0, 0, 0, 0, 0, 0, 0, 0};
    if (t == 0) {
        a0 += lam * ul[0]; a1 += lam * ul[1]; a2 += lam * ul[2];
        if (rc.w != 0.0) {
            double up[6];
#pragma unroll
            for (int p = 0; p < 6; ++p) up[p] = ((it & 1) ? P.up2 : P.up)[6 * kf + p];
            row_factored(rc, P.lin_pose[kf], xs, ul, up, P.pose_fixed[kf] ? 0.0 : 1.0, a0, a1, a2, part);
        }
    }
    a0 = sub_sum_t<T>(a0); a1 = sub_sum_t<T>(a1); a2 = sub_sum_t<T>(a2);
    if (t == 0) {
        P.wv[3 * row] = a0; P.wv[3 * row + 1] = a1; P.wv[3 * row + 2] = a2;
        part[0] = P.ecd ? 0.0 : rv0 * ul[0] + rv1 * ul[1] + rv2 * ul[2];
        part[1] = a0 * ul[0] + a1 * ul[1] + a2 * ul[2];
    }
    stamp(4);
    block_sum_store<9>(part, lds, tid, P.part_spmv + (size_t)b * NPART);
    stamp(5);
}
template <int T, bool DF, bool TPC = false, bool H4 = false, bool RCS = false, bool RCD = false, bool NT = false>
__global__ __launch_bounds__(BLK, RCD ? 3 : 4) void k_spmv_f(Dev P, double lam, int cls, int it, double tol2) {
    spmv_f_body<T, DF, TPC, H4, RCS, RCD, NT>(P, lam, cls, it, tol2, (int)blockIdx.x);
}

__global__ __launch_bounds__(BLK) void k_reduce_ru(Dev P, int it) {
    __shared__ double lds[4];
    const int tid = threadIdx.x;
    const double* pr = P.part_ru + (size_t)(it & 1) * P.n_vecblk;
    double v[1] = {0};
    for (int i = tid; i < P.n_vecblk; i += BLK) v[0] += pr[i];
    block_sum<1>(v, lds, tid & 63, tid >> 6);
    if (tid == 0) P.red[3 + 6 * P.K] = v[0];
}

__global__ __launch_bounds__(BLK) void k_reduce_partials(Dev P) {
    __shared__ double lds[4 * 6];
    if (P.flags[0]) return;
    const int tid = threadIdx.x, lane = tid & 63, wave = tid >> 6;
    if (blockIdx.x == 0) {
        double v[3] = {0, 0, 0};
        for (int b = tid; b < P.n_regblk; b += BLK) {
            v[0] += P.part_spmv[(size_t)b * NPART];
            v[1] += P.part_spmv[(size_t)b * NPART + 1];
            v[2] += P.part_spmv[(size_t)b * NPART + 2];
        }
        if (P.sk_pcg) {
            for (int b = tid; b < P.sk_nblk; b += BLK) { v[1] += P.sk_opart[(size_t)b * 8 + 7]; v[2] += P.sk_opart[(size_t)b * 8 + 6]; }
        }
        block_sum<3>(v, lds, lane, wave);
        if (tid == 0) { P.red[0] = v[0]; P.red[1] = v[1]; P.red[2] = v[2]; }
    } else {
        const int k = blockIdx.x - 1;
        const int rb = ROW_ALIGN / (BLK / P.T);
        const int g0 = P.pose_grp_ptr[k] * rb, g1 = P.pose_grp_ptr[k + 1] * rb;
        double acc[6] = {0, 0, 0, 0, 0, 0};
        for (int g = g0 + tid; g < g1; g += BLK) {
#pragma unroll
            for (int a = 0; a < 6; ++a) acc[a] += P.part_spmv[(size_t)g * NPART + 3 + a];
        }
        if (P.sk_pcg)
            for (int b = P.sk_pose_blk[k] + tid; b < P.sk_pose_blk[k + 1]; b += BLK) {
#pragma unroll
                for (int a = 0; a < 6; ++a) acc[a] += P.sk_opart[(size_t)b * 8 + a];
            }
        block_sum<6>(acc, lds, lane, wave);
        if (tid == 0) {
#pragma unroll
            for (int a = 0; a < 6; ++a) P.red[3 + 6 * k + a] = acc[a];
        }
    }
}

__device__ __forceinline__ void skin_row_gather(const Dev& P, const int q0, const int q1, const int t, double a[3]) {
    int q = q0 + t;
    for (; q + SK_RL < q1; q += 2 * SK_RL) {
        const double om0 = P.sk_rl_om[q], om1 = P.sk_rl_om[q + SK_RL];
        const double* g0 = P.sk_g + 4 * (size_t)P.sk_rl_obs[q];
        const double* g1 = P.sk_g + 4 * (size_t)P.sk_rl_obs[q + SK_RL];
        const double x0 = g0[0], x1 = g0[1], x2 = g0[2], y0 = g1[0], y1 = g1[1], y2 = g1[2];
        a[0] += om0 * x0; a[1] += om0 * x1; a[2] += om0 * x2;
        a[0] += om1 * y0; a[1] += om1 * y1; a[2] += om1 * y2;
    }
    if (q < q1) {
        const double om = P.sk_rl_om[q];
        const double* g = P.sk_g + 4 * (size_t)P.sk_rl_obs[q];
#pragma unroll
        for (int k = 0; k < 3; ++k) a[k] += om * g[k];
    }
}

template <bool SKR = false>
__global__ __launch_bounds__(BLK) void k_pcg_update(Dev P, double lam, int it, double tol2, double peek_tol2, int pub_seq) {
    __shared__ double lds[4 * 3];
    const int n_vecblk = P.sh_nvb;
    const int tid = threadIdx.x, lane = tid & 63, wave = tid >> 6;
    const double* up_in = (it & 1) ? P.up2 : P.up;   double* up_out = (it & 1) ? P.up : P.up2;
    const double* rp_in = (it & 1) ? P.rp2 : P.rp;   double* rp_out = (it & 1) ? P.rp : P.rp2;
    const int done_flag = P.flags[0] | (P.abort && *reinterpret_cast<const volatile int*>(P.abort) == P.abort_id);
    const double sc_gamma0 = P.scal[SC_GAMMA0];
    const double sc_slot0 = P.scal[(it & 1) ? SC_SLOT1 : SC_SLOT0], sc_slot1 = P.scal[((it & 1) ? SC_SLOT1 : SC_SLOT0) + 1];
    const int n_vec2 = (n_vecblk + 1) >> 1;
    const int n_vec8 = SKR ? n_vecblk * BLK / SK_RPB : ((n_vec2 + 7) >> 3) << 3;
    const bool row_wg = (int)blockIdx.x < n_vec8;
    const int pair = (row_wg && !SKR) ? P.sh_vb0 * (BLK / 2) + xcd_tile(blockIdx.x, n_vec2) * BLK + tid : 0;
    const int sk_r = P.sh_vb0 * BLK + (int)blockIdx.x * SK_RPB + tid / SK_RL, sk_t = tid % SK_RL;
    const bool has_rows = SKR ? row_wg && sk_t == 0 : row_wg && 2 * pair < (P.sh_vb0 + n_vecblk) * BLK;
    const size_t o = SKR ? 3 * (size_t)sk_r : 6 * (size_t)pair;
    double uu[6], pp[6], ww[6], ss[6], rr[6], xx[6], Di[12];
    double ska[3] = {0, 0, 0};
    bool sk_add = false;
    if (SKR) {
        if (row_wg) {
            const int q0 = P.sk_row_q[2 * (size_t)sk_r], q1 = P.sk_row_q[2 * (size_t)sk_r + 1];
            sk_add = q1 > q0 && !(P.rflag[sk_r] & RF_FIXED);
            if (has_rows) {
#pragma unroll
                for (int k = 0; k < 3; ++k) {
                    uu[k] = P.uv3[o + k]; pp[k] = P.pv[o + k]; ww[k] = P.wv[o + k]; ss[k] = P.sv[o + k]; rr[k] = P.rv[o + k]; xx[k] = P.xv[o + k];
                }
#pragma unroll
                for (int k = 0; k < 6; ++k) Di[k] = P.Dinv[2 * o + k];
            }
            if (sk_add) skin_row_gather(P, q0, q1, sk_t, ska);
#pragma unroll
            for (int k = 0; k < 3; ++k) ska[k] = sub_sum_t<SK_RL>(ska[k]);
        }
    } else if (has_rows) {
#pragma unroll
        for (int k = 0; k < 3; ++k) {
            const double2 a = *reinterpret_cast<const double2*>(P.uv3 + o + 2 * k);
            const double2 b = *reinterpret_cast<const double2*>(P.pv + o + 2 * k);
            const double2 c = *reinterpret_cast<const double2*>(P.wv + o + 2 * k);
            const double2 d = *reinterpret_cast<const double2*>(P.sv + o + 2 * k);
            const double2 e = *reinterpret_cast<const double2*>(P.rv + o + 2 * k);
            const double2 f = *reinterpret_cast<const double2*>(P.xv + o + 2 * k);
            uu[2 * k] = a.x; uu[2 * k + 1] = a.y; pp[2 * k] = b.x; pp[2 * k + 1] = b.y;
            ww[2 * k] = c.x; ww[2 * k + 1] = c.y; ss[2 * k] = d.x; ss[2 * k + 1] = d.y;
            rr[2 * k] = e.x; rr[2 * k + 1] = e.y; xx[2 * k] = f.x; xx[2 * k + 1] = f.y;
        }
#pragma unroll
        for (int k = 0; k < 6; ++k) {
            const double2 a = *reinterpret_cast<const double2*>(P.Dinv + 2 * o + 2 * k);
            Di[2 * k] = a.x; Di[2 * k + 1] = a.y;
        }
    }
    const int pk_pose = row_wg ? P.K : (int)(blockIdx.x - n_vec8) * 4 + wave;
    const bool has_pose = pk_pose < P.K;
    const int pa = lane < 6 ? lane : 0;
    double q_up[6], q_H[6], q_Hi[6], q_pp = 0, q_sp = 0, q_rp = 0, q_xp = 0, q_acc[6] = {0, 0, 0, 0, 0, 0};
    int pg0 = 0, pg1 = 0;
    if (has_pose) {
        const int rb = ROW_ALIGN / (BLK / P.T);
        pg0 = P.pose_grp_ptr[pk_pose] * rb; pg1 = P.pose_grp_ptr[pk_pose + 1] * rb;
#pragma unroll
        for (int c = 0; c < 6; ++c) {
            const int lo = pa < c ? pa : c, hi = pa < c ? c : pa;
            const int pk = lo * 6 - (lo * (lo - 1)) / 2 + (hi - lo);
            q_up[c] = up_in[6 * pk_pose + c];
            q_H[c] = P.Hpp[21 * pk_pose + pk];
            q_Hi[c] = P.Hppinv[36 * pk_pose + pa * 6 + c];
        }
        q_pp = P.pp[6 * pk_pose + pa]; q_sp = P.sp[6 * pk_pose + pa]; q_rp = rp_in[6 * pk_pose + pa]; q_xp = P.xp[6 * pk_pose + pa];
        if (P.hier) {
#pragma unroll
            for (int a = 0; a < 6; ++a) q_acc[a] = P.red[3 + 6 * pk_pose + a];
        } else if (pg0 + lane < pg1) {
#pragma unroll
            for (int a = 0; a < 6; ++a) q_acc[a] += P.part_spmv[(size_t)(pg0 + lane) * NPART + 3 + a];
        }
    }
    double v[3] = {0, 0, 0};
    if (P.hier) {
        if (tid == 0) { v[0] = P.ecd ? P.red[3 + 6 * P.K] : P.red[0]; v[1] = P.red[1]; v[2] = P.red[2]; }
    } else {
        for (int b = tid; b < P.n_regblk; b += BLK) {
            if (!P.ecd) v[0] += P.part_spmv[(size_t)b * NPART];
            v[1] += P.part_spmv[(size_t)b * NPART + 1];
            v[2] += P.part_spmv[(size_t)b * NPART + 2];
        }
        if (P.ecd) {
            const double* pr = P.part_ru + (size_t)(it & 1) * P.n_vecblk;
            for (int b = tid; b < P.n_vecblk; b += BLK) v[0] += pr[b];
        }
        if (P.sk_pcg) {
            for (int b = tid; b < P.sk_nblk; b += BLK) { v[1] += P.sk_opart[(size_t)b * 8 + 7]; v[2] += P.sk_opart[(size_t)b * 8 + 6]; }
        }
    }
    for (int i = tid; i < 6 * P.K; i += BLK) {
        const int k = i / 6, a = i % 6;
        const double ua = up_in[i];
        v[0] += rp_in[i] * ua;
        double s = lam * ua;
        for (int c = 0; c < 6; ++c) {
            const int lo = a < c ? a : c, hi = a < c ? c : a;
            const int pk = lo * 6 - (lo * (lo - 1)) / 2 + (hi - lo);
            s += P.Hpp[21 * k + pk] * up_in[6 * k + c];
        }
        v[1] += ua * s;
    }
    const bool publisher = pub_seq != 0 && blockIdx.x == 0 && tid == 0;
    if (__syncthreads_or(done_flag)) {
        if (publisher) publish_flags(P, pub_seq);
        return;
    }
    block_sum<3>(v, lds, lane, wave);
    const double gamma = v[0], delta = v[1] + v[2];
    double* nslot = P.scal + ((it & 1) ? SC_SLOT0 : SC_SLOT1);
    const double gamma0 = it == 0 ? gamma : sc_gamma0;
    const bool bad = !isfinite(gamma) || !isfinite(delta);
    const bool conv = (gamma <= tol2 * gamma0) || bad || gamma == 0.0;
    if (conv) {
        if (blockIdx.x == 0 && tid == 0) {
            if (bad) P.flags[2] = 1;
            P.flags[1] = it;
            __threadfence();
            P.flags[0] = 1;
            if (publisher) publish_flags(P, pub_seq);
        }
        return;
    }
    const double beta = it == 0 ? 0.0 : gamma / sc_slot0;
    const double alpha = it == 0 ? gamma / delta : gamma / (delta - beta * gamma / sc_slot1);
    if (blockIdx.x == 0 && tid == 0) {
        nslot[0] = gamma;
        nslot[1] = alpha;
        if (it == 0) P.scal[SC_GAMMA0] = gamma;
        P.flags[1] = it + 1;
        if (gamma <= peek_tol2 * gamma0) {
            P.flags[3] = max(P.flags[3], (gamma <= 1e-6 * peek_tol2 * gamma0 ? 4 : gamma <= 1e-4 * peek_tol2 * gamma0 ? 3 : gamma <= 1e-2 * peek_tol2 * gamma0 ? 2 : 1));
            if (P.flags[4] == 0) P.flags[4] = it + 1;
        }
        if (publisher) publish_flags(P, pub_seq);
    }
    if (SKR) {
        if (has_rows) {
#pragma unroll
            for (int k = 0; k < 3; ++k) {
                if (sk_add) ww[k] += ska[k];
                pp[k] = uu[k] + beta * pp[k];
                ss[k] = ww[k] + beta * ss[k];
                xx[k] += alpha * pp[k];
                rr[k] -= alpha * ss[k];
            }
            uu[0] = Di[0] * rr[0] + Di[1] * rr[1] + Di[2] * rr[2];
            uu[1] = Di[1] * rr[0] + Di[3] * rr[1] + Di[4] * rr[2];
            uu[2] = Di[2] * rr[0] + Di[4] * rr[1] + Di[5] * rr[2];
#pragma unroll
            for (int k = 0; k < 3; ++k) { P.pv[o + k] = pp[k]; P.sv[o + k] = ss[k]; P.xv[o + k] = xx[k]; P.rv[o + k] = rr[k]; P.uv3[o + k] = uu[k]; }
        }
    }
    if (row_wg && !SKR) {
        if (has_rows) {
#pragma unroll
            for (int k = 0; k < 6; ++k) {
                pp[k] = uu[k] + beta * pp[k];
                ss[k] = ww[k] + beta * ss[k];
                xx[k] += alpha * pp[k];
                rr[k] -= alpha * ss[k];
            }
#pragma unroll
            for (int h = 0; h < 2; ++h) {
                const double* Dh = Di + 6 * h;
                const double r0 = rr[3 * h], r1 = rr[3 * h + 1], r2 = rr[3 * h + 2];
                uu[3 * h] = Dh[0] * r0 + Dh[1] * r1 + Dh[2] * r2;
                uu[3 * h + 1] = Dh[1] * r0 + Dh[3] * r1 + Dh[4] * r2;
                uu[3 * h + 2] = Dh[2] * r0 + Dh[4] * r1 + Dh[5] * r2;
            }
#pragma unroll
            for (int k = 0; k < 3; ++k) {
                *reinterpret_cast<double2*>(P.pv + o + 2 * k) = make_double2(pp[2 * k], pp[2 * k + 1]);
                *reinterpret_cast<double2*>(P.sv + o + 2 * k) = make_double2(ss[2 * k], ss[2 * k + 1]);
                *reinterpret_cast<double2*>(P.xv + o + 2 * k) = make_double2(xx[2 * k], xx[2 * k + 1]);
                *reinterpret_cast<double2*>(P.rv + o + 2 * k) = make_double2(rr[2 * k], rr[2 * k + 1]);
                *reinterpret_cast<double2*>(P.uv3 + o + 2 * k) = make_double2(uu[2 * k], uu[2 * k + 1]);
            }
        }
        if (P.ecd) {
            double ru[1] = {0};
            if (has_rows) {
#pragma unroll
                for (int k = 0; k < 6; ++k) ru[0] += rr[k] * uu[k];
            }
            block_sum<1>(ru, lds, lane, wave);
            const int w2 = 2 * xcd_tile(blockIdx.x, n_vec2);
            double* pw = P.part_ru + (size_t)((it + 1) & 1) * P.n_vecblk;
            if (tid == 0 && w2 < P.n_vecblk) pw[w2] = ru[0];
            if (tid == 1 && w2 + 1 < P.n_vecblk) pw[w2 + 1] = 0.0;
        }
    } else if (!row_wg) {
        if (has_pose) {
            const int k = pk_pose;
            double acc[6];
#pragma unroll
            for (int a = 0; a < 6; ++a) acc[a] = q_acc[a];
            if (!P.hier) {
                for (int g = pg0 + lane + 64; g < pg1; g += 64) {
#pragma unroll
                    for (int a = 0; a < 6; ++a) acc[a] += P.part_spmv[(size_t)g * NPART + 3 + a];
                }
                if (P.sk_pcg)
                    for (int b = P.sk_pose_blk[k] + lane; b < P.sk_pose_blk[k + 1]; b += 64) {
#pragma unroll
                        for (int a = 0; a < 6; ++a) acc[a] += P.sk_opart[(size_t)b * 8 + a];
                    }
#pragma unroll
                for (int a = 0; a < 6; ++a) acc[a] = wave_sum(acc[a]);
            }
            const int a = pa;
            double hw = acc[0], ua = q_up[0];
#pragma unroll
            for (int q = 1; q < 6; ++q) { hw = (a == q) ? acc[q] : hw; ua = (a == q) ? q_up[q] : ua; }
            const int i = 6 * k + a;
            double w = lam * ua + hw;
#pragma unroll
            for (int c = 0; c < 6; ++c) w += q_H[c] * q_up[c];
            const double p = ua + beta * q_pp;
            const double sN = w + beta * q_sp;
            const double rnew = q_rp - alpha * sN;
            double unew = 0;
#pragma unroll
            for (int c = 0; c < 6; ++c) unew += q_Hi[c] * __shfl(rnew, c, 64);
            if (lane < 6) {
                P.pp[i] = p;
                P.sp[i] = sN;
                P.xp[i] = q_xp + alpha * p;
                rp_out[i] = rnew;
                up_out[i] = unew;
            }
        }
    }
}

template <int T, bool CO>
__global__ __launch_bounds__(BLK) void k_pcg_fused(Dev P, double lam, int it, double tol2, double peek_tol2, int pub_seq) {
    __shared__ double lds[4 * 9];
    __shared__ double s_up[6];
    extern __shared__ double dyn[];
    constexpr int R = 64 / T;
    constexpr int U = 4;
    if (P.one_xcd && (blockIdx.x & 7)) return;
    const int b = P.one_xcd ? (int)(blockIdx.x >> 3) : xcd_tile(blockIdx.x, P.n_regblk);
    if (b >= P.n_regblk) return;
    const int tid = threadIdx.x, lane = tid & 63, wave = tid >> 6;
    const int hin = it == 0 ? 0 : ((it + 1) & 1), hout = it & 1;
    const double* r_in = hin ? P.rv2 : P.rv;    double* r_out = hout ? P.rv2 : P.rv;
    const double* s_in = hin ? P.sv2 : P.sv;    double* s_out = hout ? P.sv2 : P.sv;
    const double* w_in = hin ? P.wv2 : P.wv;    double* w_out = hout ? P.wv2 : P.wv;
    const double* rp_in = hin ? P.rp2 : P.rp;   double* rp_out = hout ? P.rp2 : P.rp;
    const double* sp_in = hin ? P.sp2 : P.sp;   double* sp_out = hout ? P.sp2 : P.sp;
    const double* up_in = hin ? P.up2 : P.up;   double* up_out = hout ? P.up2 : P.up;
    const double* part_in = hin ? P.part_spmv2 : P.part_spmv;
    double* part_out = hout ? P.part_spmv2 : P.part_spmv;
    const double* ts_in = hin ? P.part_ts2 : P.part_ts;
    double* ts_out = hout ? P.part_ts2 : P.part_ts;
    const int slice = b * 4 + wave;
    const int row = slice * R + lane / T;
    const int t = lane % T;
    const int row0 = b * P.tile_rows;
    auto stamp = [&](int k) { if (P.dbg_clk && tid == 0) P.dbg_clk[(size_t)b * 8 + k] = wall_clock64(); };
    stamp(0);
    const int4 td = *reinterpret_cast<const int4*>(P.tile_desc + 8 * (size_t)b);
    const int kf = td.x, pg0 = td.y, pg1 = td.z, hb = td.w;
    const int hn = P.tile_desc[8 * (size_t)b + 4];
    const int done_flag = P.flags[0];
    const int ipq = it > 0 ? it - 1 : 0;
    const double sc_gamma0 = P.scal[SC_GAMMA0];
    const double sc_slot0 = P.scal[(ipq & 1) ? SC_SLOT1 : SC_SLOT0], sc_slot1 = P.scal[((ipq & 1) ? SC_SLOT1 : SC_SLOT0) + 1];
    const int self = row - row0;
    const bool rfix = (P.rflag[row] & RF_FIXED) != 0;
    double* lu = dyn;
    double* lx = dyn + 3 * (size_t)(P.tile_rows + P.max_halo);

    double v[3] = {0, 0, 0};
    const bool coarse = CO && it > 0;
    double ts9[9] = {0, 0, 0, 0, 0, 0, 0, 0, 0};
    if (it > 0) {
        for (int q = tid; q < P.n_regblk; q += BLK) {
            v[0] += part_in[(size_t)q * NPART];
            v[1] += part_in[(size_t)q * NPART + 1];
            v[2] += part_in[(size_t)q * NPART + 2];
        }
        if (coarse && tid < P.n_regblk) {
#pragma unroll
            for (int c = 0; c < 9; ++c) ts9[c] = ts_in[(size_t)c * P.n_regblk + tid];
        }
        for (int i = tid; i < 6 * P.K; i += BLK) {
            const int k = i / 6, a = i % 6;
            const double ua = up_in[i];
            v[0] += rp_in[i] * ua;
            double sacc = lam * ua;
            for (int c = 0; c < 6; ++c) {
                const int lo = a < c ? a : c, hi = a < c ? c : a;
                const int pk = lo * 6 - (lo * (lo - 1)) / 2 + (hi - lo);
                sacc += P.Hpp[21 * k + pk] * up_in[6 * k + c];
            }
            v[1] += ua * sacc;
        }
    }
    const bool own = tid < P.tile_rows;
    const size_t orow = (size_t)(row0 + (own ? tid : 0));
    double o_u[3], o_p[3], o_w[3], o_s[3], o_r[3], o_x[3], o_D[6];
    const bool hh = tid < hn;
    const size_t hrow = (size_t)P.halo_fix[(size_t)b * BLK + tid];
    double h_w[3], h_s[3], h_r[3], h_D[6];
    double x_own[3] = {0, 0, 0}, x_h[3] = {0, 0, 0};
    const bool o_free = own && !(P.rflag[orow] & RF_FIXED);
    const bool h_free = hh && !(P.rflag[hrow] & RF_FIXED);
    const int cn = P.co_n, cG = P.n_groups;
    double bt_q[6];
// ... 528 lines not shown
```

### nr-slam_amd/csrc/nrs_engine_setup.hpp

```cpp
#pragma once

namespace nrs {

int engine_num_poses(const Engine* e) { return e->d.K; }
void engine_edge_counts(const Engine* e, int* n_sp, int* n_dm) { *n_sp = e->d.n_sp; *n_dm = e->d.n_dm; }

void arena_release(Arena* a) {
    if (a->base) (void)hipFree(a->base);
    a->base = nullptr;
    a->cap = a->off = 0;
}

struct ArenaPlan {
    Arena* a;
    bool dry;
    size_t off = 0;
    size_t row_lo = 0, row_n = 0;
    template <class Tp> Tp* get(size_t n) {
        const size_t bytes = ((n * sizeof(Tp) + 255) / 256) * 256 + 256;
        Tp* p = dry ? nullptr : reinterpret_cast<Tp*>(a->base + off);
        off += bytes;
        return p;
    }
    template <class Tp> Tp* get_rows(size_t per_row) {
        Tp* p = get<Tp>(row_n * per_row);
        return dry ? nullptr : p - row_lo * per_row;
    }
};

static int spec_prepare(nrs_ctx* c, Engine* e) {
    const Dev& d = e->d;
    if (!c->pin_spec_scal) {
        NRS_HIP(c, hipHostMalloc((void**)&c->pin_spec_scal, sizeof(double) * SC_N * SPEC_MAX, hipHostMallocMapped | hipHostMallocCoherent));
        NRS_HIP(c, hipHostMalloc((void**)&c->pin_spec_flags, sizeof(int) * 8 * SPEC_MAX, hipHostMallocMapped | hipHostMallocCoherent));
        memset(c->pin_spec_flags, 0, sizeof(int) * 8 * SPEC_MAX);
        for (int j = 0; j < SPEC_MAX; ++j) {
            NRS_HIP(c, hipStreamCreateWithFlags(&c->spec_stream[j], hipStreamNonBlocking));
            NRS_HIP(c, hipEventCreateWithFlags(&c->spec_join[j], hipEventDisableTiming));
        }
        NRS_HIP(c, hipEventCreateWithFlags(&c->spec_fork, hipEventDisableTiming));
        for (int j = 0; j < 1 + SPEC_MAX; ++j) NRS_HIP(c, hipEventCreateWithFlags(&c->spec_back[j], hipEventDisableTiming));
    }
    for (int j = 0; j < e->n_spec; ++j) {
        SpecSet& q = e->spec[j];
        q.h_scal = c->pin_spec_scal + SC_N * j; q.h_flags = c->pin_spec_flags + 8 * j;
        NRS_HIP(c, hipMemsetAsync(q.part_apply, 0, sizeof(double) * (size_t)d.n_vecblk, c->stream));
        NRS_HIP(c, hipMemsetAsync(q.part_rchi, 0, sizeof(double) * (size_t)d.n_groups, c->stream));
        NRS_HIP(c, hipMemsetAsync(q.part_reg, 0, sizeof(double) * 2 * (size_t)d.n_regblk, c->stream));
        NRS_HIP(c, hipMemsetAsync(q.scal, 0, sizeof(double) * SC_N, c->stream));
        NRS_HIP(c, hipMemsetAsync(q.flags, 0, sizeof(int) * 8, c->stream));
        NRS_HIP(c, hipMemsetAsync(q.abort, 0, sizeof(int), c->stream));
    }
    return NRS_OK;
}

static int spec_sets(const nrs_ctx* c) {
    if (c->opt.profile) return 0;
    if (const char* v = c->env("NRS_SPEC_TRIALS")) return std::max(0, std::min(SPEC_MAX, atoi(v)));
    return 2;
}

static void spec_pcg_sets(const nrs_ctx* c, Engine* e, int n_skin) {
    const Dev& d = e->d;
    const long max_rows = c->env("NRS_SPEC_MAX_ROWS") ? atol(c->env("NRS_SPEC_MAX_ROWS")) : (1L << 18);
    const bool on = !e->nd && !d.fused && !d.coarse && !d.sh_on && n_skin == 0 && !c->opt.profile && (long)d.n_rows <= max_rows;
    e->spec_pcg = on;
    e->n_spec = on ? spec_sets(c) : 0;
}

static void carve(ArenaPlan& A, Dev& d, bool has_X0, size_t nnz_s, size_t nnz_d, size_t n_slices, size_t n_halo, Engine* e) {
    const size_t nr = (size_t)d.n_rows, K = (size_t)d.K;
    if (d.row_hi <= 0) { d.row_lo = 0; d.row_hi = d.n_rows; }
    A.row_lo = (size_t)d.row_lo; A.row_n = (size_t)(d.row_hi - d.row_lo);
    d.grp_pose = A.get<int>(d.n_groups);
    d.pose_grp_ptr = A.get<int>(K + 1);
    d.rflag = A.get_rows<uint8_t>(1);
    d.pose_fixed = A.get<uint8_t>(K);
    d.uv = A.get_rows<float>(2);
    double* X0 = has_X0 ? A.get_rows<double>(3) : A.get<double>(1);
    d.X0 = has_X0 ? X0 : nullptr;
    d.ss_ptr = A.get<int>(n_slices + 1);
    d.sd_ptr = A.get<int>(n_slices + 1);
    d.halo_ptr = A.get<int>((size_t)d.n_regblk + 1);
    d.halo_rows = A.get<int>(n_halo);
    d.halo_ns = A.get<int>((size_t)d.n_regblk);
    d.tile_list = A.get<int>((size_t)d.n_regblk);
    d.s_om = A.get<uint32_t>(d.use_lds ? nnz_s : 1);
    d.s_qc = A.get<double>(d.use_lds ? nnz_s : 1);
    d.d_hdr = A.get<uint2>(d.use_lds && !d.dform ? nnz_d : 1);
    d.d_om = A.get<uint32_t>(d.use_lds && d.dform ? nnz_d : 1);
    d.nxt_row = A.get<int>(d.dform ? nr : 1); d.prv_row = A.get<int>(d.dform ? nr : 1);
    d.halo_nxt = A.get<int>(d.dform ? std::max<size_t>(1, n_halo) : 1); d.halo_prv = A.get<int>(d.dform ? std::max<size_t>(1, n_halo) : 1);
    const size_t us = d.use_lds ? 1 : nnz_s, ud = d.use_lds ? 1 : nnz_d;
    d.s_other = A.get<int>(us); d.s_d0 = A.get<float>(nnz_s); d.s_meta = A.get<int>(us);
    d.d_o0 = A.get<int>(ud); d.d_o1 = A.get<int>(ud); d.d_o2 = A.get<int>(ud);
    d.d_w = A.get<float>(nnz_d); d.d_meta = A.get<int>(ud);
    for (int s = 0; s < 2; ++s) { d.pose[s] = A.get<Pose>(K); d.xl[s] = A.get_rows<double>(3); }
    d.pose_init = A.get<Pose>(K);
    d.xl_init = A.get_rows<double>(3);
    d.D = A.get_rows<double>(6);
    d.Hpl = A.get<double>(d.use_lds ? 1 : 18 * nr);
    d.rowrec = d.use_lds ? A.get_rows<RowRec>(1) : A.get<RowRec>(1);
    d.row_tp = d.plain ? A.get_rows<uint32_t>(1) : A.get<uint32_t>(1);
    d.row_cnt = d.plain ? A.get_rows<uint32_t>(1) : A.get<uint32_t>(1);
    d.d_h4 = A.get<uint32_t>(d.plain && d.use_lds && !d.fused ? nnz_d : 1);
    d.s_g = A.get<double>(3 * us);
    d.d_s = A.get<double>(nnz_d);
    d.Hpp = A.get<double>(21 * K);
    d.bp = A.get<double>(6 * K);
    d.bl = A.get_rows<double>(3);
    d.Dinv = A.get_rows<double>(6);
    d.Hppinv = A.get<double>(36 * K);
    double** pv[] = {&d.xp, &d.rp, &d.up, &d.pp, &d.sp, &d.wp};
    for (auto p : pv) *p = A.get<double>(6 * K);
    double** rvv[] = {&d.xv, &d.rv, &d.uv3, &d.pv, &d.sv, &d.wv};
    for (auto p : rvv) *p = A.get_rows<double>(3);
    d.rp2 = A.get<double>(6 * K); d.sp2 = A.get<double>(6 * K); d.up2 = A.get<double>(6 * K);
    d.rv2 = A.get<double>(d.fused ? 3 * nr : 1); d.sv2 = A.get<double>(d.fused ? 3 * nr : 1); d.wv2 = A.get<double>(d.fused ? 3 * nr : 1);
    d.part_spmv2 = A.get<double>(d.fused ? NPART * (size_t)d.n_regblk : 1);
    {
        const size_t nb = d.coarse ? (size_t)d.n_regblk : 1, nc = d.coarse ? (size_t)d.co_n : 1;
        d.co_ct = A.get<double>(nb * (d.coarse ? (size_t)d.n_groups : 1) * 6);
        d.co_cp = A.get<double>(nb * 18);
        d.co_tb = A.get<double>(nb * 4);
        d.co_bt = A.get<double>(nb * 6);
        d.co_bti = A.get<double>(nb * 6);
        d.part_ts = A.get<double>(nb * 9); d.part_ts2 = A.get<double>(nb * 9);
        d.co_c0 = A.get<double>(nc * nc); d.co_nn = A.get<double>(nc); d.co_bc = A.get<double>(nc);
        d.co_inv = A.get<double>(nc * nc); d.co_y0 = A.get<double>(nc);
    }
    d.tile_desc = A.get<int>(d.fused ? 8 * (size_t)d.n_regblk : 4);
    d.halo_fix = A.get<int>(d.fused ? BLK * (size_t)d.n_regblk : d.plain && d.use_lds ? HALO_FIX * (size_t)d.n_regblk : 4);
    d.red = A.get<double>(4 + 6 * K);
    d.red_loc = A.get<double>(4 + 6 * K);
    d.pk = A.get<double>(2 + 8 + 27 * K);
    d.pk_loc = A.get<double>(2 + 8 + 27 * K);
    d.part_ru = A.get<double>(d.ecd ? 2 * (size_t)d.n_vecblk : 1);
    d.part_lin = A.get<double>(32 * (size_t)d.n_groups * (size_t)d.lin_rb);
    d.part_rchi = A.get<double>((size_t)d.n_groups);
    d.part_pchi = A.get<double>(K);
    d.part_reg = A.get<double>(2 * (size_t)d.n_regblk);
    d.part_spmv = A.get<double>(NPART * (size_t)d.n_regblk);
    d.part_apply = A.get<double>((size_t)d.n_vecblk);
    d.scal = A.get<double>(SC_N);
    d.flags = A.get<int>(8);
    d.ec_sp = A.get<EcSpring>(d.ec_on ? std::max(1, d.ec_nsp) : 1);
    d.ec_dm = A.get<EcDamper>(d.ec_on ? std::max(1, d.ec_ndm) : 1);
    d.ec_w = A.get<float>(d.ec_on ? std::max(1, d.ec_ndm) : 1);
    d.part_ec = A.get<double>(d.ec_on ? std::max(1, d.ec_nblk) : 1);
    for (int j = 0; j < e->n_spec; ++j) {
        SpecSet& q = e->spec[j];
        q.xv = A.get_rows<double>(3); q.xp = A.get<double>(6 * K);
        q.pose = A.get<Pose>(K); q.xl = A.get_rows<double>(3);
        q.part_apply = A.get<double>((size_t)d.n_vecblk); q.part_rchi = A.get<double>((size_t)d.n_groups); q.part_reg = A.get<double>(2 * (size_t)d.n_regblk);
        q.scal = A.get<double>(SC_N); q.flags = A.get<int>(8); q.abort = A.get<int>(1);
        q.sk_part = q.sk_chi = nullptr;
        q.rv = q.uv3 = q.pv = q.sv = q.wv = q.Dinv = q.Hppinv = q.rp = q.rp2 = q.up = q.up2 = q.pp = q.sp = nullptr;
        q.part_spmv = q.part_ru = q.red = q.part_ec = nullptr;
        if (!e->spec_pcg) continue;
        double** rows[] = {&q.rv, &q.uv3, &q.pv, &q.sv, &q.wv};
        for (auto p : rows) *p = A.get_rows<double>(3);
        q.Dinv = A.get_rows<double>(6);
        q.Hppinv = A.get<double>(36 * K);
        double** poses[] = {&q.rp, &q.rp2, &q.up, &q.up2, &q.pp, &q.sp};
        for (auto p : poses) *p = A.get<double>(6 * K);
        q.part_spmv = A.get<double>(NPART * (size_t)d.n_regblk);
        q.part_ru = A.get<double>(d.ecd ? 2 * (size_t)d.n_vecblk : 1);
        q.red = A.get<double>(4 + 6 * K);
        q.part_ec = A.get<double>(d.ec_on ? std::max(1, d.ec_nblk) : 1);
    }
}

template <class Tp>
static int h2d(nrs_ctx* c, Tp* dst, const std::vector<Tp>& src) {
    if (!src.empty()) NRS_HIP(c, hipMemcpyAsync(dst, src.data(), sizeof(Tp) * src.size(), hipMemcpyHostToDevice, c->stream));
    return NRS_OK;
}

template <class Tp>
static int h2d_rows(nrs_ctx* c, const Dev& d, Tp* dst, const std::vector<Tp>& src, size_t per_row) {
    const size_t o = (size_t)d.row_lo * per_row, n = (size_t)(d.row_hi - d.row_lo) * per_row;
    if (n) NRS_HIP(c, hipMemcpyAsync(dst + o, src.data() + o, sizeof(Tp) * n, hipMemcpyHostToDevice, c->stream));
    return NRS_OK;
}

static int host_threads(const nrs_ctx* c, size_t work) {
    if (work < 600000) {
        if (const char* ev = c->env("NRS_HOST_THREADS_SMALL")) if (work >= 100000) return std::max(1, std::min(8, atoi(ev)));
        return 1;
    }
    int n = (int)std::min<unsigned>(16u, std::max(1u, std::thread::hardware_concurrency()));
    if (const char* ev = c->env("NRS_HOST_THREADS")) n = std::max(1, std::min(64, atoi(ev)));
    return n;
}
__global__ void k_compact_headers(size_t n, const uint2* __restrict__ hdr, uint32_t* __restrict__ h4) {
    const size_t i = (size_t)blockIdx.x * blockDim.x + threadIdx.x;
    if (i >= n) return;
    const uint2 h = hdr[i];
    const uint32_t m16 = h.y >> 16;
    h4[i] = m16 == REC_NONE ? 0xFFFFFFFFu : ((h.x & 0xFFFu) | ((h.y & 0xFFFu) << 12) | ((m16 & 0xFFu) << 24));
}
static void engine_compact_headers(nrs_ctx* c, Engine* e) {
    Dev& d = e->d;
    d.h4 = 0; d.rc = 0; d.nt = 0;
    if (!(d.plain && d.tp_ok && d.use_lds && !d.fused && d.T == 2) || c->env("NRS_NO_H4")) return;
    if (d.tile_rows + std::max(d.cap_h[0], d.cap_h[1]) + 2 >= 4096 || d.sd_nnz <= 0) return;
    hipLaunchKernelGGL(k_compact_headers, dim3((unsigned)(((size_t)d.sd_nnz + 255) / 256)), dim3(256), 0, c->stream, (size_t)d.sd_nnz, d.d_hdr, d.d_h4);
    d.h4 = 1;
    if (const char* v = c->env("NRS_RC")) d.rc = atoi(v) & 3;
    d.nt = 12 * ((size_t)d.ss_nnz + (size_t)d.sd_nnz) > ((size_t)128 << 20);
    if (const char* v = c->env("NRS_NT")) d.nt = atoi(v) != 0;
}

template <class F>
static void parallel_for(int nt, F&& fn) {
    if (nt <= 1) { fn(0, 1); return; }
    std::vector<std::thread> th;
    th.reserve(nt - 1);
    for (int t = 1; t < nt; ++t) {
        try { th.emplace_back([&fn, t, nt] { fn(t, nt); }); }
        catch (const std::system_error&) { fn(t, nt); }
    }
    fn(0, nt);
    for (auto& x : th) x.join();
}
static inline void chunk(int64_t n, int t, int nt, int64_t& a, int64_t& b) { a = n * t / nt; b = n * (t + 1) / nt; }
static inline void count_up(int* p, int nt) { if (nt == 1) ++*p; else __atomic_fetch_add(p, 1, __ATOMIC_RELAXED); }

static int push_masks(nrs_ctx* c, Engine* e, const uint8_t* sp_active, const uint8_t* dm_active) {
    Dev& d = e->d;
    auto vfixed = [&](int v) { return (e->h_rflag[e->vrow[v]] & RF_FIXED) != 0; };
    const int nt = host_threads(c, (size_t)d.n_sp + (size_t)d.n_dm);
    parallel_for(nt, [&](int ti, int n_thr) {
    int64_t q0, q1;
    chunk(d.n_sp, ti, n_thr, q0, q1);
    for (int s = (int)q0; s < (int)q1; ++s) {
        const int i = e->sp_ij[2 * s], j = e->sp_ij[2 * s + 1];
        const bool act = (!sp_active || sp_active[s]) && !(vfixed(i) && vfixed(j));
        const int m = act ? SM_ACTIVE : 0;
        if (e->sp_pos[2 * s] >= 0) e->h_s_meta[e->sp_pos[2 * s]] = m | (act ? SM_COUNT : 0);
        if (e->sp_pos[2 * s + 1] >= 0) e->h_s_meta[e->sp_pos[2 * s + 1]] = m;
    }
    chunk(d.n_dm, ti, n_thr, q0, q1);
    for (int s = (int)q0; s < (int)q1; ++s) {
        bool allfix = true;
        int first = -1;
        for (int r = 0; r < 4; ++r) {
            const int v = e->dm_idx[4 * s + r];
            if (v >= 0) { if (first < 0) first = r; allfix = allfix && vfixed(v); }
        }
        const bool act = (!dm_active || dm_active[s]) && !allfix;
        for (int r = 0; r < 4; ++r) {
            const int p = e->dm_pos[4 * s + r];
            if (p < 0) continue;
            e->h_d_meta[p] = r | (act ? DM_ACTIVE : 0) | ((act && r == first) ? DM_COUNT : 0);
        }
    }
    chunk(d.n_un, ti, n_thr, q0, q1);
    for (int s = (int)q0; s < (int)q1; ++s) {
        const bool act = !vfixed(e->un_ij[2 * s]);
        if (e->un_pos[s] >= 0) e->h_d_meta[e->un_pos[s]] = 2 | DM_UNARY | (act ? (DM_ACTIVE | DM_COUNT) : 0);
    }
    });
    if (d.use_lds) {
        parallel_for(nt, [&](int ti, int n_thr) {
            int64_t a, b;
            chunk((int64_t)e->h_s_om.size(), ti, n_thr, a, b);
            for (int64_t i = a; i < b; ++i) {
                const int m = e->h_s_meta[i];
                const uint32_t m16 = (uint32_t)(((m & SM_ACTIVE) ? SR_ACTIVE : 0) | ((m & SM_COUNT) ? SR_COUNT : 0));
                e->h_s_om[i] = (e->h_s_om[i] & 0xFFFFu) | (m16 << 16);
            }
            chunk((int64_t)e->h_d_hdr.size(), ti, n_thr, a, b);
            for (int64_t i = a; i < b; ++i) {
                const uint32_t m16 = e->h_d_meta[i] < 0 ? (uint32_t)REC_NONE : (uint32_t)(e->h_d_meta[i] & 0xFFFF);
                e->h_d_hdr[i].y = (e->h_d_hdr[i].y & 0xFFFFu) | (m16 << 16);
            }
        });
        for (size_t i = 0; i < e->h_d_om.size(); ++i) {
            const uint32_t m16 = e->h_d_meta[i] < 0 ? (uint32_t)REC_NONE : (uint32_t)(e->h_d_meta[i] & 0xFFFF);
            e->h_d_om[i] = (e->h_d_om[i] & 0xFFFFu) | (m16 << 16);
        }
        NRS_TRY(h2d(c, d.s_om, e->h_s_om));
        if (d.dform) NRS_TRY(h2d(c, d.d_om, e->h_d_om));
        else NRS_TRY(h2d(c, d.d_hdr, e->h_d_hdr));
    } else {
        NRS_TRY(h2d(c, d.s_meta, e->h_s_meta));
        NRS_TRY(h2d(c, d.d_meta, e->h_d_meta));
    }
    NRS_TRY(h2d_rows(c, d, d.rflag, e->h_rflag, 1));
    NRS_TRY(h2d(c, d.pose_fixed, e->h_pose_fixed));
    return NRS_OK;
}

void shard_plan(int K, const int* grp_ptr, int world, int* kb) {
    const int total = grp_ptr[K];
    kb[0] = 0;
    for (int r = 1; r < world; ++r) {
        const int64_t want = (int64_t)total * r / world;
        int k = kb[r - 1] + 1;
        while (k < K - (world - r) && grp_ptr[k] < want) ++k;
        if (k - 1 > kb[r - 1] && want - grp_ptr[k - 1] < grp_ptr[k] - want) --k;
        kb[r] = k;
    }
    kb[world] = K;
}

static bool devpack_eligible(nrs_ctx* c, const EngineSpec& s, int n_pad_rows);
static int engine_create_device(nrs_ctx* c, const EngineSpec& s, Arena* arena, Engine* e, bool* done);

int engine_create(nrs_ctx* c, const EngineSpec& s, Arena* arena, Engine** out) {
    *out = nullptr;
    c->err_local = false;
    if (s.K <= 0 || s.M <= 0 || !s.poses || !s.x || !s.lm_pose || !s.uv || !s.rflag || s.n_sp < 0 || s.n_dm < 0 || s.n_un < 0)
        return c->fail(NRS_ERR_INVALID, "engine: bad specification");
    for (int i = 0; i < s.M; ++i)
        if (s.lm_pose[i] < 0 || s.lm_pose[i] >= s.K || (i > 0 && s.lm_pose[i] < s.lm_pose[i - 1]))
            return c->fail(NRS_ERR_INVALID, "vertex pose index must be non-decreasing and in [0, n_poses)");
    if (!s.edges_on_device) {
        for (int64_t i = 0; i < 2 * (int64_t)s.n_sp; ++i)
            if (s.sp_ij[i] < 0 || s.sp_ij[i] >= s.M) return c->fail(NRS_ERR_INVALID, "spring index out of range");
        for (int64_t i = 0; i < 4 * (int64_t)s.n_dm; ++i)
            if (s.dm_idx[i] < -1 || s.dm_idx[i] >= s.M) return c->fail(NRS_ERR_INVALID, "damper index out of range");
    }
    for (int64_t i = 0; i < 2 * (int64_t)s.n_un; ++i)
        if (s.un_ij[i] < 0 || s.un_ij[i] >= s.M) return c->fail(NRS_ERR_INVALID, "unary damper index out of range");
    if (c->comm && s.shard) {
        if (c->comm->world > 8) return c->fail(NRS_ERR_INVALID, "sharded solve: at most 8 ranks");
        if (s.K < c->comm->world) return c->fail(NRS_ERR_INVALID, "sharded solve: %d keyframes cannot be split over %d ranks", s.K, c->comm->world);
    }
    c->err_local = true;
    const bool tm = c->env("NRS_TIMING") != nullptr;
    auto t_prev = std::chrono::steady_clock::now();
    auto mark = [&](const char* what) {
        if (!tm) return;
        auto now = std::chrono::steady_clock::now();
        fprintf(stderr, "[nrs] engine_create %-18s %.2f ms\n", what, std::chrono::duration<double, std::milli>(now - t_prev).count());
        t_prev = now;
    };
    NRS_HIP(c, hipSetDevice(c->device));
    Engine* e = new (std::nothrow) Engine();
    if (!e) return c->fail(NRS_ERR_ALLOC, "out of host memory");
    struct Guard { nrs_ctx* c; Engine* e; bool keep = false; ~Guard() { if (!keep) engine_destroy(c, e); } } guard{c, e};
    e->arena = arena;
    Dev& d = e->d;
    memset(&d, 0, sizeof(d));
    int n_pad_rows = 0;
    {
        std::vector<int> cnt(s.K, 0);
        for (int i = 0; i < s.M; ++i) cnt[s.lm_pose[i]]++;
        for (int k = 0; k < s.K; ++k) n_pad_rows += std::max(1, (cnt[k] + ROW_ALIGN - 1) / ROW_ALIGN) * ROW_ALIGN;
    }
    if (devpack_eligible(c, s, n_pad_rows)) {
        bool done = false;
        NRS_TRY(engine_create_device(c, s, arena, e, &done));
        if (done) { guard.keep = true; *out = e; return NRS_OK; }
        *e = Engine();
        e->arena = arena;
        memset(&d, 0, sizeof(d));
    }
    if (s.edges_on_device) return c->fail(NRS_ERR_STATE, "device-built edge lists need the device-side construction, which this window does not qualify for");
    if (s.n_skin > 0) {
        if ((!(arena == &c->arena_trk && s.K == 1) && !s.sk_pose) || !s.sk_uv || !s.sk_X0 || !s.sk_node || !s.sk_om)
            return c->fail(NRS_ERR_INVALID, "skinned observations: single-frame tracking engines, or BA windows with a pose per observation");
// ... 543 lines not shown
    e->dm_idx.assign(s.dm_idx, s.dm_idx + 4 * (size_t)s.n_dm);
    e->dm_w.assign(s.dm_w, s.dm_w + (size_t)s.n_dm);
    e->un_ij.assign(s.un_ij, s.un_ij + 2 * (size_t)s.n_un);
    e->un_w.assign(s.un_w, s.un_w + (size_t)s.n_un);
    e->h_rflag.assign(d.n_rows, RF_FIXED);
    for (int v = 0; v < s.M; ++v) e->h_rflag[e->vrow[v]] = s.rflag[v];
    e->h_pose_fixed.assign(s.K, 0);
    if (s.pose_fixed) e->h_pose_fixed.assign(s.pose_fixed, s.pose_fixed + s.K);
    std::vector<float> uv((size_t)d.n_rows * 2, 0.f);
    std::vector<double> xl((size_t)d.n_rows * 3, 0.0), X0;
    if (s.X0) X0.assign((size_t)d.n_rows * 3, 0.0);
    for (int v = 0; v < s.M; ++v) {
        const size_t row = (size_t)e->vrow[v];
        uv[2 * row] = s.uv[2 * v];
        uv[2 * row + 1] = s.uv[2 * v + 1];
        for (int k = 0; k < 3; ++k) {
            xl[3 * row + k] = s.x[3 * (size_t)v + k];
            if (s.X0) X0[3 * row + k] = s.X0[3 * (size_t)v + k];
        }
    }
    e->h_s_meta.assign(nnz_s, 0);
    e->h_d_meta.assign(nnz_d, -1);
    const int nt_mir = nt_all;
    parallel_for(nt_mir, [&](int ti, int n) {
        int64_t a, b;
        chunk((int64_t)nnz_d, ti, n, a, b);
        for (int64_t i = a; i < b; ++i)
            if (D_role[i] >= 0) e->h_d_meta[i] = D_role[i];
    });
    std::vector<int> d_o0, d_o1, d_o2;
    if (d.use_lds) {
        auto u16 = [](int v) { return v < 0 ? (uint32_t)REC_NONE : (uint32_t)(v & 0xFFFF); };
        e->h_s_om.resize(nnz_s);
        parallel_for(nt_mir, [&](int ti, int n) {
            int64_t a, b;
            chunk((int64_t)nnz_s, ti, n, a, b);
            for (int64_t i = a; i < b; ++i) e->h_s_om[i] = u16(L_s[i]);
        });
        if (d.dform) {
            e->h_d_om.resize(nnz_d);
            for (size_t i = 0; i < nnz_d; ++i) e->h_d_om[i] = D_role[i] < 0 ? (uint32_t)REC_NONE : u16(L_d[3 * i + (D_role[i] < 2 ? 0 : 2)]);
        } else {
            static const int perm[4][3] = {{0, 1, 2}, {0, 2, 1}, {2, 0, 1}, {2, 1, 0}};
            e->h_d_hdr.resize(nnz_d);
            parallel_for(nt_mir, [&](int ti, int n) {
                int64_t a, b;
                chunk((int64_t)nnz_d, ti, n, a, b);
                for (int64_t i = a; i < b; ++i) {
                    const int* pm = perm[D_role[i] < 0 ? 0 : D_role[i]];
                    e->h_d_hdr[i] = make_uint2(u16(L_d[3 * i + pm[0]]) | (u16(L_d[3 * i + pm[1]]) << 16), u16(L_d[3 * i + pm[2]]) | ((uint32_t)REC_NONE << 16));
                }
            });
        }
    } else {
        d_o0.resize(nnz_d); d_o1.resize(nnz_d); d_o2.resize(nnz_d);
        for (size_t i = 0; i < nnz_d; ++i) { d_o0[i] = D_o[3 * i]; d_o1[i] = D_o[3 * i + 1]; d_o2[i] = D_o[3 * i + 2]; }
    }
    const std::vector<int>& s_other = S_other;
    const std::vector<float>& s_d0 = S_d0;
    const std::vector<float>& d_w = D_w;
    mark("host mirrors");
    std::vector<Pose> poses(s.poses, s.poses + s.K);
    NRS_TRY(h2d(c, d.grp_pose, grp_pose));
    NRS_TRY(h2d(c, d.pose_grp_ptr, pose_grp_ptr));
    NRS_TRY(h2d_rows(c, d, d.uv, uv, 2));
    if (d.row_hi - d.row_lo < d.n_rows) e->h_uv = uv;
    NRS_TRY(h2d_rows(c, d, d.xl_init, xl, 3));
    if (s.X0) NRS_TRY(h2d_rows(c, d, d.X0, X0, 3));
    NRS_TRY(h2d(c, d.pose_init, poses));
    NRS_TRY(h2d(c, d.ss_ptr, ss_ptr));
    NRS_TRY(h2d(c, d.sd_ptr, sd_ptr));
    NRS_TRY(h2d(c, d.halo_ptr, halo_ptr));
    NRS_TRY(h2d(c, d.halo_rows, halo_rows));
    NRS_TRY(h2d(c, d.halo_ns, halo_ns));
    NRS_TRY(h2d(c, d.tile_list, tile_list));
    if (d.dform) {
        std::vector<int> hn(halo_rows.size()), hp(halo_rows.size());
        for (size_t i = 0; i < halo_rows.size(); ++i) { hn[i] = nxt_row[halo_rows[i]]; hp[i] = prv_row[halo_rows[i]]; }
        NRS_TRY(h2d(c, d.nxt_row, nxt_row));
        NRS_TRY(h2d(c, d.prv_row, prv_row));
        NRS_TRY(h2d(c, d.halo_nxt, hn));
        NRS_TRY(h2d(c, d.halo_prv, hp));
        NRS_HIP(c, hipStreamSynchronize(c->stream));
    }
    if (d.fused) {
        std::vector<int> tile_desc(8 * (size_t)d.n_regblk, 0), halo_fix((size_t)BLK * d.n_regblk, 0);
        const int rb = ROW_ALIGN / d.tile_rows;
        for (int b = 0; b < d.n_regblk; ++b) {
            const int kf = grp_pose[(size_t)b * d.tile_rows / ROW_ALIGN];
            int* td = &tile_desc[8 * (size_t)b];
            td[0] = kf; td[1] = pose_grp_ptr[kf] * rb; td[2] = pose_grp_ptr[kf + 1] * rb;
            td[3] = halo_ptr[b]; td[4] = halo_ptr[b + 1] - halo_ptr[b];
            for (int i = 0; i < td[4] && i < BLK; ++i) halo_fix[(size_t)b * BLK + i] = halo_rows[td[3] + i];
        }
        NRS_TRY(h2d(c, d.tile_desc, tile_desc));
        NRS_TRY(h2d(c, d.halo_fix, halo_fix));
    } else if (d.plain && d.use_lds) {
        std::vector<int> halo_fix((size_t)HALO_FIX * d.n_regblk, -1);
        for (int b = 0; b < d.n_regblk; ++b) {
            const int hn = std::min(halo_ptr[b + 1] - halo_ptr[b], HALO_FIX);
            for (int i = 0; i < hn; ++i) halo_fix[(size_t)b * HALO_FIX + i] = halo_rows[halo_ptr[b] + i];
        }
        NRS_TRY(h2d(c, d.halo_fix, halo_fix));
    }
    NRS_TRY(h2d(c, d.s_d0, s_d0));
    if (d.use_lds) {
        NRS_HIP(c, hipMemsetAsync(d.s_qc, 0, sizeof(double) * nnz_s, c->stream));
        NRS_HIP(c, hipMemsetAsync(d.d_s, 0, sizeof(double) * nnz_d, c->stream));
    }
    if (!d.use_lds) {
        NRS_TRY(h2d(c, d.s_other, s_other));
        NRS_TRY(h2d(c, d.d_o0, d_o0));
        NRS_TRY(h2d(c, d.d_o1, d_o1));
        NRS_TRY(h2d(c, d.d_o2, d_o2));
    }
    NRS_TRY(h2d(c, d.d_w, d_w));
    if (d.plain) NRS_TRY(h2d_rows(c, d, d.row_tp, row_tp, 1));
    if (d.plain) {
        std::vector<uint32_t> rc((size_t)d.n_rows);
        for (int r = 0; r < d.n_rows; ++r) rc[r] = (uint32_t)cnt_s[r] | ((uint32_t)cnt_d[r] << 16);
        NRS_TRY(h2d_rows(c, d, d.row_cnt, rc, 1));
        NRS_HIP(c, hipStreamSynchronize(c->stream));
    }
    if (d.ec_on) {
        NRS_TRY(h2d(c, d.ec_sp, ec_sp));
        NRS_TRY(h2d(c, d.ec_dm, ec_dm));
        NRS_TRY(h2d(c, d.ec_w, ec_w));
    }
    NRS_TRY(push_masks(c, e, s.sp_active, s.dm_active));
    e->serial = ++c->engine_serial;
    NRS_HIP(c, hipMemsetAsync(d.part_apply, 0, sizeof(double) * (size_t)d.n_vecblk, c->stream));
    if (d.sh_on) {
        NRS_HIP(c, hipMemsetAsync(d.part_lin, 0, sizeof(double) * 32 * (size_t)d.n_groups * (size_t)d.lin_rb, c->stream));
        NRS_HIP(c, hipMemsetAsync(d.part_rchi, 0, sizeof(double) * (size_t)d.n_groups, c->stream));
        NRS_HIP(c, hipMemsetAsync(d.part_reg, 0, sizeof(double) * 2 * (size_t)d.n_regblk, c->stream));
        NRS_HIP(c, hipMemsetAsync(d.part_spmv, 0, sizeof(double) * NPART * (size_t)d.n_regblk, c->stream));
        NRS_HIP(c, hipMemsetAsync(d.red, 0, sizeof(double) * (4 + 6 * (size_t)d.K), c->stream));
        NRS_HIP(c, hipMemsetAsync(d.red_loc, 0, sizeof(double) * (4 + 6 * (size_t)d.K), c->stream));
    }
    NRS_HIP(c, hipMemsetAsync(d.scal, 0, sizeof(double) * SC_N, c->stream));
    NRS_HIP(c, hipMemsetAsync(d.flags, 0, sizeof(int) * 8, c->stream));
    mark("uploads enqueued");
    if (!c->pin_scal) NRS_HIP(c, hipHostMalloc((void**)&c->pin_scal, sizeof(double) * SC_N, hipHostMallocMapped | hipHostMallocCoherent));
    if (!c->pin_flags) {
        NRS_HIP(c, hipHostMalloc((void**)&c->pin_flags, sizeof(int) * 8, hipHostMallocMapped | hipHostMallocCoherent));
        memset(c->pin_flags, 0, sizeof(int) * 8);
    }
    e->h_scal = c->pin_scal;
    e->h_flags = c->pin_flags;
    e->d.h_scal = c->pin_scal;
    e->d.h_flags = c->pin_flags;
    if (e->n_spec > 0) NRS_TRY(spec_prepare(c, e));
    engine_compact_headers(c, e);
    NRS_HIP(c, hipStreamSynchronize(c->stream));
    mark("pinned+sync");
    if (s.n_skin > 0) {
        const bool ba_form = s.sk_pose != nullptr;
        if (d.fused || (d.sh_on && !ba_form) || !s.sk_uv || !s.sk_X0 || !s.sk_node || !s.sk_om) return c->fail(NRS_ERR_INVALID, "skinned observations: two-kernel PCG path");
        if (!ba_form && !(arena == &c->arena_trk && s.K == 1)) return c->fail(NRS_ERR_INVALID, "skinned observations without a pose index: single-frame tracking engines only");
        const size_t n_in = (size_t)s.n_skin;
        std::vector<int> pose0;
        if (!ba_form) pose0.assign(n_in, 0);
        const int* sk_pose = ba_form ? s.sk_pose : pose0.data();
        const int own_k0 = d.sh_k0, own_k1 = d.sh_k0 + d.sh_nk;
        auto held = [&](size_t i) { return sk_pose[i] >= own_k0 && sk_pose[i] < own_k1; };
        std::vector<int> cnt(s.K + 1, 0), pose_blk(s.K + 1, 0);
        for (size_t i = 0; i < n_in; ++i) {
            if (sk_pose[i] < 0 || sk_pose[i] >= s.K) return c->fail(NRS_ERR_INVALID, "skinned observation: pose index out of range");
            if (held(i)) cnt[sk_pose[i] + 1]++;
        }
        for (int k = 0; k < s.K; ++k) pose_blk[k + 1] = pose_blk[k] + (cnt[k + 1] + BLK - 1) / BLK;
        if (d.sh_on && pose_blk[s.K] == 0)
            for (int k = own_k0; k < s.K; ++k) pose_blk[k + 1]++;
        const size_t nblk = (size_t)pose_blk[s.K], n = nblk * BLK;
        std::vector<int> next(s.K), blk_pose(nblk);
        for (int k = 0; k < s.K; ++k) { next[k] = pose_blk[k] * BLK; for (int b2 = pose_blk[k]; b2 < pose_blk[k + 1]; ++b2) blk_pose[b2] = k; }
        e->sk_slot.assign(n_in, -1);
        std::vector<float> uv(2 * n, 0.f);
        std::vector<double> X0(3 * n, 0.0), om(SK_MAX * n, 0.0);
        std::vector<int> rows(SK_MAX * n, -1);
        std::vector<uint8_t> act(n, 0);
        std::vector<int> rl_cnt(d.n_rows + 1, 0);
        for (size_t i = 0; i < n_in; ++i) {
            if (!held(i)) continue;
            const size_t sl = (size_t)next[sk_pose[i]]++;
            e->sk_slot[i] = (int)sl;
            uv[2 * sl] = s.sk_uv[2 * i]; uv[2 * sl + 1] = s.sk_uv[2 * i + 1];
            for (int k = 0; k < 3; ++k) X0[3 * sl + k] = s.sk_X0[3 * i + k];
            act[sl] = 1;
            for (int k = 0; k < SK_MAX; ++k) {
                const int v = s.sk_node[SK_MAX * i + k];
                if (v < 0) continue;
                if (s.lm_pose[v] != sk_pose[i]) return c->fail(NRS_ERR_INVALID, "skinned observation: a node copy of another keyframe");
                rows[(size_t)k * n + sl] = e->vrow[v];
                om[(size_t)k * n + sl] = s.sk_om[SK_MAX * i + k];
                rl_cnt[e->vrow[v] + 1]++;
            }
        }
        std::vector<int> rl_row, rl_ptr(1, 0), row_list(d.n_rows, -1);
        for (int r = 0; r < d.n_rows; ++r)
            if (rl_cnt[r + 1] > 0) { row_list[r] = (int)rl_row.size(); rl_row.push_back(r); rl_ptr.push_back(rl_ptr.back() + rl_cnt[r + 1]); }
        const size_t n_ent = (size_t)rl_ptr.back(), nrl = rl_row.size();
        if (d.sh_on) {
            const int own_lo = d.sh_g0 * ROW_ALIGN, own_hi = (d.sh_g0 + d.sh_ng) * ROW_ALIGN;
            for (size_t q = 0; q < rows.size(); ++q)
                if (rows[q] >= 0 && (rows[q] < own_lo || rows[q] >= own_hi)) return c->fail(NRS_ERR_INVALID, "skinned observation: node row %d outside the rank's rows [%d, %d)", rows[q], own_lo, own_hi);
            for (size_t l = 0; l < nrl; ++l)
                if (rl_row[l] < own_lo || rl_row[l] >= own_hi) return c->fail(NRS_ERR_INVALID, "skinned observations: row list %d outside the rank's rows [%d, %d)", rl_row[l], own_lo, own_hi);
        }
        std::vector<int> rl_obs(n_ent + 1), fill(rl_ptr.begin(), rl_ptr.end() - 1);
        std::vector<double> rl_om(n_ent + 1);
        for (size_t sl = 0; sl < n; ++sl)
            for (int k = 0; k < SK_MAX; ++k) {
                const int r = rows[(size_t)k * n + sl];
                if (r < 0) continue;
                const int q = fill[row_list[r]]++;
                rl_obs[q] = (int)sl; rl_om[q] = om[(size_t)k * n + sl];
            }
        auto al = [](size_t b2) { return (b2 + 255) & ~(size_t)255; };
        const size_t o_uv = 0, o_X0 = o_uv + al(8 * n), o_row = o_X0 + al(24 * n), o_om = o_row + al(4 * SK_MAX * n), o_act = o_om + al(8 * SK_MAX * n),
                     o_bp = o_act + al(n), o_pb = o_bp + al(4 * nblk), o_rr = o_pb + al(4 * (s.K + 1)), o_rp = o_rr + al(4 * (nrl + 1)), o_ro = o_rp + al(4 * (nrl + 1)),
                     o_rw = o_ro + al(4 * (n_ent + 1)), o_rec = o_rw + al(8 * (n_ent + 1)), o_part = o_rec + al(8 * 27 * n), o_chi = o_part + al(8 * 32 * nblk),
                     o_md = o_chi + al(8 * n), o_g = o_md + 256, o_op = o_g + al(8 * 4 * n), o_rq = o_op + al(8 * 8 * nblk), o_recT = o_rq + al(8 * (size_t)d.n_rows),
                     o_dop = o_recT + al(8 * 24 * n), o_spec = o_dop + (d.use_lds ? 0 : al(8 * 6 * (size_t)d.n_rows)),
                     spec_stride = al(8 * 32 * nblk) + al(8 * n), total = o_spec + (size_t)e->n_spec * spec_stride;
        DevBuf& buf = arena == &c->arena_trk ? c->nd_skin : c->dba_skin;
        NRS_TRY(c->ensure(buf, total));
        e->sk_bytes = total;
        char* sb = buf.as<char>();
        auto up = [&](size_t off, const void* src, size_t bytes) { return bytes ? hipMemcpyAsync(sb + off, src, bytes, hipMemcpyHostToDevice, c->stream) : hipSuccess; };
        NRS_HIP(c, up(o_uv, uv.data(), 8 * n)); NRS_HIP(c, up(o_X0, X0.data(), 24 * n)); NRS_HIP(c, up(o_row, rows.data(), 4 * SK_MAX * n));
        NRS_HIP(c, up(o_om, om.data(), 8 * SK_MAX * n)); NRS_HIP(c, up(o_act, act.data(), n)); NRS_HIP(c, up(o_bp, blk_pose.data(), 4 * nblk));
        NRS_HIP(c, up(o_pb, pose_blk.data(), 4 * (size_t)(s.K + 1))); NRS_HIP(c, up(o_rr, rl_row.data(), 4 * nrl)); NRS_HIP(c, up(o_rp, rl_ptr.data(), 4 * (nrl + 1)));
        NRS_HIP(c, up(o_ro, rl_obs.data(), 4 * n_ent)); NRS_HIP(c, up(o_rw, rl_om.data(), 8 * n_ent));
        NRS_HIP(c, hipMemsetAsync(sb + o_rec, 0, total - o_rec, c->stream));
        std::vector<int> row_q(2 * (size_t)d.n_rows, 0);
        for (size_t l = 0; l < nrl; ++l) { row_q[2 * (size_t)rl_row[l]] = rl_ptr[l]; row_q[2 * (size_t)rl_row[l] + 1] = rl_ptr[l + 1]; }
        NRS_HIP(c, up(o_rq, row_q.data(), 8 * (size_t)d.n_rows));
        NRS_HIP(c, hipStreamSynchronize(c->stream));
        d.sk_n = (int)n; d.sk_nblk = (int)nblk; d.sk_pcg = 1;
        d.sk_uv = reinterpret_cast<const float*>(sb + o_uv); d.sk_X0 = reinterpret_cast<const double*>(sb + o_X0);
        d.sk_row = reinterpret_cast<const int*>(sb + o_row); d.sk_om = reinterpret_cast<const double*>(sb + o_om);
        d.sk_active = reinterpret_cast<const uint8_t*>(sb + o_act);
        d.sk_blk_pose = reinterpret_cast<const int*>(sb + o_bp); d.sk_pose_blk = reinterpret_cast<const int*>(sb + o_pb);
        d.sk_nrl = (int)nrl; d.sk_rl_row = reinterpret_cast<const int*>(sb + o_rr); d.sk_rl_ptr = reinterpret_cast<const int*>(sb + o_rp);
        d.sk_rl_obs = reinterpret_cast<const int*>(sb + o_ro); d.sk_rl_om = reinterpret_cast<const double*>(sb + o_rw);
        d.sk_rec = reinterpret_cast<double*>(sb + o_rec); d.sk_part = reinterpret_cast<double*>(sb + o_part);
        d.sk_chi = reinterpret_cast<double*>(sb + o_chi); d.sk_maxdiag = reinterpret_cast<double*>(sb + o_md);
        d.sk_g = reinterpret_cast<double*>(sb + o_g); d.sk_opart = reinterpret_cast<double*>(sb + o_op); d.sk_row_q = reinterpret_cast<const int*>(sb + o_rq);
        d.sk_recT = reinterpret_cast<double*>(sb + o_recT);
        d.D_op = d.use_lds ? nullptr : reinterpret_cast<double*>(sb + o_dop);
        for (int j = 0; j < e->n_spec; ++j) {
            e->spec[j].sk_part = reinterpret_cast<double*>(sb + o_spec + (size_t)j * spec_stride);
            e->spec[j].sk_chi = reinterpret_cast<double*>(sb + o_spec + (size_t)j * spec_stride + al(8 * 32 * nblk));
        }
        d.sk_base = ba_form ? d.xl_init : nullptr;
        e->sk_vert.assign(s.sk_node, s.sk_node + SK_MAX * n_in);
        e->sk_om.assign(s.sk_om, s.sk_om + SK_MAX * n_in);
        e->sk_X0.assign(s.sk_X0, s.sk_X0 + 3 * n_in);
    }
    if (e->nd) {
        NRS_TRY(nd_engine_finish(c, e, e->nd, nd_prep));
        mark("direct solve plan");
    }
    d.sk_pcg = (d.sk_n > 0 && !(e->nd && e->nd->on)) ? 1 : 0;
    if (d.sk_pcg) d.ecd = 0;
    if (d.sk_pcg && s.sk_pose && d.use_lds && (d.sh_on ? c->opt.sharded_kft == 1 : !d.hier) && c->opt.embedded_solver != 2) {
        NRS_TRY(kft_setup(c, e, s, pose_grp_ptr));
        mark("keyframe-block factorisation plan");
    }
    NRS_TRY(engine_reset(c, e));
    guard.keep = true;
    *out = e;
    return NRS_OK;
}

void engine_stats(const Engine* e, int64_t stats[5]) {
    stats[0] = e->d.n_rows; stats[1] = e->pack_rows; stats[2] = e->d.ss_nnz; stats[3] = e->d.sd_nnz; stats[4] = (int64_t)e->arena_bytes;
}

void engine_destroy(nrs_ctx* c, Engine* e) {
    if (!e) return;
    (void)hipStreamSynchronize(c->stream);
    nd_engine_free(c, e->nd);
    delete e->kft;
    delete e;
}

int engine_update_flags(nrs_ctx* c, Engine* e, const uint8_t* rflag, const uint8_t* pose_fixed,
                        const uint8_t* sp_active, const uint8_t* dm_active) {
    if (e->d.plain) return c->fail(NRS_ERR_STATE, "masks on a plain BA window: not supported (its partial slots are per slice)");
    if (rflag)
        for (int v = 0; v < e->d.M; ++v) e->h_rflag[e->vrow[v]] = rflag[v];
    if (pose_fixed) e->h_pose_fixed.assign(pose_fixed, pose_fixed + e->d.K);
    e->d.ec_on = 0;
    NRS_TRY(push_masks(c, e, sp_active, dm_active));
    NRS_HIP(c, hipStreamSynchronize(c->stream));
    if (e->nd) {
        bool same = e->nd->sig.size() == (size_t)e->d.M + 1 && e->nd->sig[e->d.M] == e->h_pose_fixed[0];
        for (int v = 0; v < e->d.M && same; ++v) same = e->nd->sig[v] == (e->h_rflag[e->vrow[v]] & RF_FIXED);
        if (!same) NRS_TRY(nd_engine_setup(c, e, e->nd));
        e->d.sk_pcg = (e->d.sk_n > 0 && !e->nd->on) ? 1 : 0;
        if (e->d.sk_pcg) e->d.ecd = 0;
    }
    return NRS_OK;
}
// ... 76 lines not shown
```

### nr-slam_amd/csrc/nrs_engine_types.hpp

```cpp
#pragma once

namespace nrs {

constexpr int ROW_ALIGN = 256;
constexpr int BLK = 256;
constexpr int NPART = 12;
constexpr int SK_MAX = 11;
constexpr int SK_RL = 16;
constexpr int SK_RPB = BLK / SK_RL;
constexpr int CO_MAX = 84;
constexpr int CO_GMAX = (CO_MAX - 6) / 3;
static_assert(CO_GMAX <= 32, "k_coarse_tile keeps the reached groups in a 32-bit mask");

constexpr int SM_COUNT = 1 << 30;
constexpr int SM_ACTIVE = 1 << 29;
constexpr int DM_COUNT = 1 << 2;
constexpr int DM_ACTIVE = 1 << 3;
constexpr int DM_UNARY = 1 << 4;

struct SpringRec { double qc; uint16_t other, meta; };
struct __attribute__((aligned(16))) RowRec { float J[6]; double w; };
struct DamperRec { uint16_t o0, o1, o2, meta; double s; };
constexpr uint16_t REC_NONE = 0xFFFF;
constexpr uint16_t SR_ACTIVE = 1, SR_COUNT = 2;

struct __attribute__((aligned(16))) EcSpring { int a, b; float d0; int pad; };
struct __attribute__((aligned(16))) EcDamper { int r[4]; };

struct Dev {
    int K, M, n_rows, n_groups;
    int row_lo, row_hi;
    int T;
    int n_sp, n_dm, n_un;
    int n_regblk, n_vecblk;
    Cam cam;
    double info_reproj, delta_reproj, info_pos, delta_pos, info_spatial, delta_spatial, k_spring;
    int spring_form;
    int* grp_pose;
    int* pose_grp_ptr;
    uint8_t* rflag;
    uint8_t* pose_fixed;
    float* uv;
    double* X0;
    int* ss_ptr; int ss_nnz; int* sd_ptr; int sd_nnz;
    int* s_other; float* s_d0; int* s_meta;
    int* d_o0; int* d_o1; int* d_o2; float* d_w; int* d_meta;
    int use_lds, tile_rows, max_halo;
    int max_halo_s;
    int* tile_list; int n_tiles_cls[2]; int cap_h[2], cap_s[2];
    int* halo_ptr; int* halo_rows; int* halo_ns;
    uint32_t* s_om; double* s_qc; uint2* d_hdr;
    int dform;
    uint32_t* d_om;
    int* nxt_row; int* prv_row;
    int* halo_nxt; int* halo_prv;
    uint32_t* row_tp; int tp_ok;
    int rc;
    int nt;
    uint32_t* d_h4; int h4;
    uint32_t* row_cnt;
    RowRec* rowrec;
    Pose* lin_pose; double* lin_xl;
    Pose* pose[2]; double* xl[2];
    Pose* pose_init; double* xl_init;
    double* D;
    double* Hpl;
    double* s_g;
    double* d_s;
    double* Hpp;
    double* bp; double* bl;
    double* Dinv; double* Hppinv;
    double *xp, *rp, *up, *pp, *sp, *wp;
    double *xv, *rv, *uv3, *pv, *sv, *wv;
    double *rp2, *sp2, *up2, *rv2, *sv2, *wv2, *part_spmv2;
    int fused;
    int coarse, co_n;
    double* co_ct;
    double* co_cp;
    double* co_tb;
    double* part_ts; double* part_ts2;
    double* co_bt;
    double* co_bti;
    double* co_c0;
    double* co_nn; double* co_bc;
    double* co_inv;
    double* co_y0;
    int* tile_desc;
    int* halo_fix;
    int hier;
    int ecd; double* part_ru;
    double* red;
    double* part_lin;
    double* part_rchi;
    double* part_pchi;
    int lin_rb;
    double* part_reg;
    double* part_spmv;
    double* part_apply;
    double* scal;
    int ec_on, ec_nsp, ec_ndm, ec_nblk;
    long long* dbg_clk; int one_xcd;
    int plain;
    EcSpring* ec_sp; EcDamper* ec_dm; float* ec_w; double* part_ec;
    double* h_scal; int* h_flags;
    int* flags;
    const int* abort; int abort_id;
    int sh_on, sh_rank, sh_world;
    int sh_lead;
    int sh_k0, sh_nk;
    int sh_g0, sh_ng;
    int sh_vb0, sh_nvb;
    int sh_t0[2], sh_nt[2];
    int sh_t0b[2], sh_ntb[2];
    int sh_front[2], sh_back[2];
    double* red_loc;
    int sk_n, sk_nblk;
    const float* sk_uv; const double* sk_X0; const int* sk_row; const double* sk_om; const uint8_t* sk_active;
    double* sk_rec;
    double* sk_part;
    double* sk_chi;
    double* sk_maxdiag;
    int sk_pcg;
    const int* sk_blk_pose;
    const int* sk_pose_blk;
    const double* sk_base;
    int sk_nrl;
    const int* sk_rl_row; const int* sk_rl_ptr; const int* sk_rl_obs; const double* sk_rl_om;
    double* sk_recT;
    double* sk_g;
    double* sk_opart;
    const int* sk_row_q;
    double* D_op;
    double* pk; double* pk_loc;
};

inline int rc_of(const Dev& d, int cls) {
    if (!(d.rc & 2)) return d.rc;
    return sizeof(double) * 3 * (size_t)(2 * (d.tile_rows + d.cap_h[cls]) + 2) > 64 * 1024 - 512 ? (d.rc & 1) : d.rc;
}

enum { SC_CHI = 0, SC_MAXDIAG = 1, SC_SCALE = 2, SC_GAMMA0 = 3, SC_SLOT0 = 4, SC_SLOT1 = 6, SC_N = 16 };

constexpr int SPEC_MAX = 3;
struct SpecSet {
    double *xv, *xp, *part_apply, *part_rchi, *part_reg, *scal;
    double *sk_part, *sk_chi;
    int* flags;
    int* abort;
    Pose* pose; double* xl;
    double* h_scal; int* h_flags;
    double *rv, *uv3, *pv, *sv, *wv, *Dinv, *Hppinv;
    double *rp, *rp2, *up, *up2, *pp, *sp;
    double *part_spmv, *part_ru, *red, *part_ec;
};

struct NdEngine;
struct KftHost;
struct Engine {
    Dev d;
    NdEngine* nd = nullptr;
    KftHost* kft = nullptr;
    bool kft_wanted = false;
    Arena* arena = nullptr;
    int cur = 0;
    int n_spec = 0;
    bool spec_pcg = false;
    int spec_run = 4;
    int spec_gen = 0;
    unsigned spec_run_at = 0;
    int spec_follow_first = 0;
    SpecSet spec[SPEC_MAX];
    int pred_iters = 0;
    int pack_rows = 0;
    size_t arena_bytes = 0;
    int pred_peek = 0;
    bool first_trial_accepted = false;
    double* h_scal = nullptr;
    int* h_flags = nullptr;
    HaloPlan halo;
    std::vector<int> vrow;
    std::vector<int> sp_ij, dm_idx, un_ij;
    std::vector<float> sp_d0, dm_w, un_w;
    std::vector<int> sp_pos, dm_pos, un_pos;
    std::vector<int> h_s_meta, h_d_meta;
    std::vector<uint32_t> h_s_om;
    std::vector<uint2> h_d_hdr;
    std::vector<uint32_t> h_d_om;
    std::vector<uint8_t> h_rflag, h_pose_fixed;
    std::vector<float> h_uv;
    std::vector<int> sk_slot;
    size_t sk_bytes = 0;
    std::vector<int> sk_vert;
    std::vector<double> sk_om, sk_X0;
    unsigned long long serial = 0;
    bool dev_edges = false;
    const int *raw_sp = nullptr, *raw_dm = nullptr;
    const float *raw_d0 = nullptr, *raw_w = nullptr;
};

__device__ inline bool spec_aborted(const Dev& P) {
    return P.abort && __syncthreads_or(*reinterpret_cast<const volatile int*>(P.abort) == P.abort_id);
}

__device__ inline int xcd_tile(int b, int nb) {
    const int nb8 = (nb + 7) >> 3;
    return (b & 7) * nb8 + (b >> 3);
}

template <int N>
__device__ inline void block_sum(double* v, double* lds , int lane, int wave) {
#pragma unroll
    for (int k = 0; k < N; ++k) {
        const double s = wave_sum(v[k]);
        if (lane == 0) lds[wave * N + k] = s;
    }
    __syncthreads();
#pragma unroll
    for (int k = 0; k < N; ++k) v[k] = lds[k] + lds[N + k] + lds[2 * N + k] + lds[3 * N + k];
    __syncthreads();
}

template <int N>
__device__ inline void block_sum_store(const double* v, double* lds , int tid, double* out) {
    const int lane = tid & 63, wave = tid >> 6;
#pragma unroll
    for (int k = 0; k < N; ++k) {
        const double s = wave_sum(v[k]);
        if (lane == 0) lds[wave * N + k] = s;
    }
    __syncthreads();
    if (tid < N) out[tid] = lds[tid] + lds[N + tid] + lds[2 * N + tid] + lds[3 * N + tid];
}

template <int T>
__device__ inline double sub_sum_t(double v) { return group_sum<T>(v); }

__device__ inline bool inv3_sym(const double* d , double lam, double* o) {
    const double a = d[0] + lam, b = d[1], c = d[2], e = d[3] + lam, f = d[4], g = d[5] + lam;
    const double c00 = e * g - f * f, c01 = c * f - b * g, c02 = b * f - c * e;
    const double det = a * c00 + b * c01 + c * c02;
    const double id = 1.0 / det;
    o[0] = c00 * id; o[1] = c01 * id; o[2] = c02 * id;
    o[3] = (a * g - c * c) * id; o[4] = (b * c - a * f) * id; o[5] = (a * e - b * b) * id;
    return det > 0;
}

__device__ inline void tile_level(const double* Bi , const double* rc, double* y) {
    y[0] = Bi[0] * rc[0] + Bi[1] * rc[1] + Bi[2] * rc[2];
    y[1] = Bi[1] * rc[0] + Bi[3] * rc[1] + Bi[4] * rc[2];
    y[2] = Bi[2] * rc[0] + Bi[4] * rc[1] + Bi[5] * rc[2];
}

constexpr int STAGE_K = 4;
constexpr int HALO_FIX = 2 * BLK;
template <bool FIX = false>
__device__ inline void stage_rows(const Dev& P, int b, int tid, const double* __restrict__ v, const double* __restrict__ add,
                                  double* lds) {
    const int row0 = b * P.tile_rows;
    int idx[STAGE_K];
    if (FIX) {
#pragma unroll
        for (int k = 0; k < HALO_FIX / BLK; ++k) idx[k] = P.halo_fix[(size_t)b * HALO_FIX + k * BLK + tid];
    }
    const int hb = P.halo_ptr[b], hn = P.halo_ptr[b + 1] - hb;
#pragma unroll
    for (int k = FIX ? HALO_FIX / BLK : 0; k < STAGE_K; ++k) { const int i = tid + k * BLK; idx[k] = i < hn ? P.halo_rows[hb + i] : -1; }
    for (int i = tid; i < 3 * P.tile_rows; i += BLK) lds[i] = v[3 * (size_t)row0 + i] + (add ? add[3 * (size_t)row0 + i] : 0.0);
    double val[STAGE_K][3];
#pragma unroll
    for (int k = 0; k < STAGE_K; ++k) {
        if (idx[k] >= 0) {
            const size_t r = (size_t)idx[k];
#pragma unroll
            for (int c = 0; c < 3; ++c) val[k][c] = v[3 * r + c] + (add ? add[3 * r + c] : 0.0);
        }
    }
#pragma unroll
    for (int k = 0; k < STAGE_K; ++k) {
        if (idx[k] >= 0) {
            double* d = lds + 3 * (size_t)(P.tile_rows + tid + k * BLK);
            d[0] = val[k][0]; d[1] = val[k][1]; d[2] = val[k][2];
        }
    }
    for (int i = tid + STAGE_K * BLK; i < hn; i += BLK) {
        const size_t r = (size_t)P.halo_rows[hb + i];
        double* d = lds + 3 * (size_t)(P.tile_rows + i);
        d[0] = v[3 * r] + (add ? add[3 * r] : 0.0);
        d[1] = v[3 * r + 1] + (add ? add[3 * r + 1] : 0.0);
        d[2] = v[3 * r + 2] + (add ? add[3 * r + 2] : 0.0);
    }
}

__device__ inline void stage_rows_d(const Dev& P, int b, int tid, const double* __restrict__ v, double* lv, double* lf, double* lb) {
    const int row0 = b * P.tile_rows;
    const int hb = P.halo_ptr[b], hn = P.halo_ptr[b + 1] - hb;
    for (int i = tid; i < P.tile_rows + hn; i += BLK) {
        int r, rn, rp;
        if (i < P.tile_rows) { r = row0 + i; rn = P.nxt_row[r]; rp = P.prv_row[r]; }
        else { const int j = hb + i - P.tile_rows; r = P.halo_rows[j]; rn = P.halo_nxt[j]; rp = P.halo_prv[j]; }
        const size_t a = 3 * (size_t)r, an = 3 * (size_t)(rn >= 0 ? rn : r), ap = 3 * (size_t)(rp >= 0 ? rp : r);
        const double v0 = v[a], v1 = v[a + 1], v2 = v[a + 2];
        const double n0 = v[an], n1 = v[an + 1], n2 = v[an + 2];
        const double p0 = v[ap], p1 = v[ap + 1], p2 = v[ap + 2];
        lv[3 * i] = v0; lv[3 * i + 1] = v1; lv[3 * i + 2] = v2;
// ... 115 lines not shown
```

Baseline: 2004 LM iters/s.

## Store each damper once and scatter its contribution to the partner row

Adds a two-incidence damper path: each damper pair is kept only in the forward row's list (backward duplicates dropped), and the SpMV computes the difference against the next row's staged uv3. The result is added to the owning row and its negation is written to a per-row buffer hn for the partner row, which the vector update folds into s. The aim is to roughly halve the damper records streamed per SpMV. In exchange it adds setup kernels, a second staged halo layout, and an extra hn read and write per iteration, and it falls back to the old path when the derivation checks fail.

```diff
diff --git a/nr-slam_amd/csrc/nrs_engine.hip b/nr-slam_amd/csrc/nrs_engine.hip
--- a/nr-slam_amd/csrc/nrs_engine.hip
+++ b/nr-slam_amd/csrc/nrs_engine.hip
@@ -195,7 +195,8 @@
             }
             continue;
         }
-        const size_t shm = sizeof(double) * 3 * (size_t)(2 * d.tile_rows + d.cap_h[cls] + ((rc_of(d, cls) & 2) ? d.cap_h[cls] : d.cap_s[cls]) + 2);
+        const size_t shm = d.td ? td_lds_bytes(d, cls)
+                                : sizeof(double) * 3 * (size_t)(2 * d.tile_rows + d.cap_h[cls] + ((rc_of(d, cls) & 2) ? d.cap_h[cls] : d.cap_s[cls]) + 2);
         const bool last_cls = cls == 1 || d.sh_nt[1] + d.sh_ntb[1] == 0;
         if (with_skin_op && last_cls && !(d.T == 2 && d.plain && d.tp_ok) && !c->env("NRS_SKIN_OP_OWN_LAUNCH")) {
             const dim3 g2(g.x + d.sk_nblk);
@@ -218,6 +219,8 @@
                 if (d.plain && d.tp_ok && d.h4 && rc_of(d, cls) == 1) hipLaunchKernelGGL((k_spmv_f<2, false, true, true, true, false>), g, b, shm, c->stream, d, lam, cls, it, tol2);
                 else if (d.plain && d.tp_ok && d.h4 && rc_of(d, cls) == 2) hipLaunchKernelGGL((k_spmv_f<2, false, true, true, false, true>), g, b, shm, c->stream, d, lam, cls, it, tol2);
                 else if (d.plain && d.tp_ok && d.h4 && rc_of(d, cls) == 3) hipLaunchKernelGGL((k_spmv_f<2, false, true, true, true, true>), g, b, shm, c->stream, d, lam, cls, it, tol2);
+                else if (d.td && d.nt) hipLaunchKernelGGL((k_spmv_f<2, false, true, true, false, false, true, true>), g, b, shm, c->stream, d, lam, cls, it, tol2);
+                else if (d.td) hipLaunchKernelGGL((k_spmv_f<2, false, true, true, false, false, false, true>), g, b, shm, c->stream, d, lam, cls, it, tol2);
                 else if (d.plain && d.tp_ok && d.h4 && d.nt) hipLaunchKernelGGL((k_spmv_f<2, false, true, true, false, false, true>), g, b, shm, c->stream, d, lam, cls, it, tol2);
                 else if (d.plain && d.tp_ok && d.h4) hipLaunchKernelGGL((k_spmv_f<2, false, true, true>), g, b, shm, c->stream, d, lam, cls, it, tol2);
                 else if (d.plain && d.tp_ok) hipLaunchKernelGGL((k_spmv_f<2, false, true>), g, b, shm, c->stream, d, lam, cls, it, tol2);
@@ -384,7 +387,7 @@
         if (!on) return;
         const SpecSet& q = e->spec[set];
         Dev& d = e->d;
-        d.xv = q.xv; d.rv = q.rv; d.uv3 = q.uv3; d.pv = q.pv; d.sv = q.sv; d.wv = q.wv; d.Dinv = q.Dinv; d.Hppinv = q.Hppinv;
+        d.xv = q.xv; d.rv = q.rv; d.uv3 = q.uv3; d.pv = q.pv; d.sv = q.sv; d.wv = q.wv; d.hn = q.hn; d.Dinv = q.Dinv; d.Hppinv = q.Hppinv;
         d.xp = q.xp; d.rp = q.rp; d.rp2 = q.rp2; d.up = q.up; d.up2 = q.up2; d.pp = q.pp; d.sp = q.sp;
         d.part_spmv = q.part_spmv; d.part_ru = q.part_ru; d.red = q.red; d.part_ec = q.part_ec;
         d.part_apply = q.part_apply; d.part_rchi = q.part_rchi; d.part_reg = q.part_reg; d.scal = q.scal; d.flags = q.flags;
diff --git a/nr-slam_amd/csrc/nrs_engine_devpack.hpp b/nr-slam_amd/csrc/nrs_engine_devpack.hpp
--- a/nr-slam_amd/csrc/nrs_engine_devpack.hpp
+++ b/nr-slam_amd/csrc/nrs_engine_devpack.hpp
@@ -738,6 +738,7 @@
     if (c->pack_ws2.cap > ((size_t)512 << 20)) c->release(c->pack_ws2);
     mark("final arrays");
     engine_compact_headers(c, e);
+    NRS_TRY(engine_td_setup(c, e, false));
     NRS_TRY(engine_reset(c, e));
     *done = true;
     return NRS_OK;
diff --git a/nr-slam_amd/csrc/nrs_engine_linearize.hpp b/nr-slam_amd/csrc/nrs_engine_linearize.hpp
--- a/nr-slam_amd/csrc/nrs_engine_linearize.hpp
+++ b/nr-slam_amd/csrc/nrs_engine_linearize.hpp
@@ -606,15 +606,19 @@
     const double isp = P.info_spatial, dsp = P.delta_spatial;
     uint32_t rd_w[NB];
     uint2 rd_h[NB];
+    int rd_p[NB];
+    const bool td = !RCD && P.td;
     auto req_d = [&](int q, int idx) {
+        rd_p[q] = -1;
         if (EXP == 3) { rd_h[q] = make_uint2((uint32_t)(idx & 63) | ((uint32_t)((idx + 1) & 63) << 16), (uint32_t)((idx + 2) & 63) | 0x80000u); rd_w[q] = 0x3F800000u; return; }
         rd_h[q] = make_uint2(0xFFFFFFFFu, 0xFFFFFFFFu); rd_w[q] = 0u;
         if (H4) { if ((idx - d_beg - lane) / 64 < my_d) {
             if (NT) { rd_h[q].x = __builtin_nontemporal_load(P.d_h4 + idx); rd_w[q] = __float_as_uint(__builtin_nontemporal_load(P.d_w + idx)); }
-            else { rd_h[q].x = P.d_h4[idx]; rd_w[q] = __float_as_uint(P.d_w[idx]); } } }
-        else if ((idx - d_beg - lane) / 64 < my_d) { rd_h[q] = P.d_hdr[idx]; rd_w[q] = __float_as_uint(P.d_w[idx]); }
+            else { rd_h[q].x = P.d_h4[idx]; rd_w[q] = __float_as_uint(P.d_w[idx]); }
+            if (td) rd_p[q] = P.td_pos[idx]; } }
+        else if ((idx - d_beg - lane) / 64 < my_d) { rd_h[q] = P.d_hdr[idx]; rd_w[q] = __float_as_uint(P.d_w[idx]); if (td) rd_p[q] = P.td_pos[idx]; }
     };
-    auto do_d = [&](uint32_t hx, uint32_t hy, float wf, int idx) {
+    auto do_d = [&](uint32_t hx, uint32_t hy, float wf, int idx, int tdp) {
         const uint32_t m16 = H4 ? (hx == 0xFFFFFFFFu ? (uint32_t)REC_NONE : hx >> 24) : hy >> 16;
         const bool live = idx < d_end;
         const bool pad = !live || m16 == REC_NONE;
@@ -636,6 +640,7 @@
         const double sfac = damper_s(g0, g1, g2, w, isp, dsp, rho0);
         chi += (m16 & DM_COUNT) ? rho0 : 0.0;
         if (live && EXP != 1 && !RCD) { if (NT) __builtin_nontemporal_store(sfac, P.d_s + idx); else P.d_s[idx] = sfac; }
+        if (td && live && tdp >= 0) { if (NT) __builtin_nontemporal_store(sfac, P.td_s + tdp); else P.td_s[tdp] = sfac; }
         D0 += sfac; D3 += sfac; D5 += sfac;
         bb0 = fma(-sfac, g0, bb0); bb1 = fma(-sfac, g1, bb1); bb2 = fma(-sfac, g2, bb2);
     };
@@ -648,7 +653,7 @@
         for (int q = 0; q < NB; ++q) {
             const uint32_t hx = consume(rd_h[q].x), hy = H4 ? 0u : consume(rd_h[q].y);
             const float wf = __uint_as_float(consume(rd_w[q]));
-            do_d(hx, hy, wf, base + 64 * q);
+            do_d(hx, hy, wf, base + 64 * q, td ? (int)consume((uint32_t)rd_p[q]) : -1);
         }
         __builtin_amdgcn_sched_barrier(0);
     }
diff --git a/nr-slam_amd/csrc/nrs_engine_pcg.hpp b/nr-slam_amd/csrc/nrs_engine_pcg.hpp
--- a/nr-slam_amd/csrc/nrs_engine_pcg.hpp
+++ b/nr-slam_amd/csrc/nrs_engine_pcg.hpp
@@ -164,9 +164,29 @@
     block_sum_store<9>(part, lds, tid, P.part_spmv + (size_t)b * NPART);
 }
 
-template <int T, bool DF, bool TPC = false, bool H4 = false, bool RCS = false, bool RCD = false, bool NT = false>
+__device__ inline void stage_rows_td(const Dev& P, int b, int tid, double* lu, double* ld, double* lx) {
+    const int row0 = b * P.tile_rows, nh = P.td_nh[b], ns = P.halo_ns[b];
+    const size_t so = (size_t)b * P.max_halo;
+    for (int i = tid; i < P.tile_rows + nh; i += BLK) {
+        const bool own = i < P.tile_rows;
+        const int r = own ? row0 + i : P.td_rows[so + i - P.tile_rows];
+        const int nx = own ? P.td_nxt[row0 + i] : P.td_rnx[so + i - P.tile_rows];
+        const size_t a = 3 * (size_t)r, an = 3 * (size_t)(nx >= 0 ? nx : r);
+        double u[3], n[3];
+#pragma unroll
+        for (int k = 0; k < 3; ++k) { u[k] = P.uv3[a + k]; n[k] = P.uv3[an + k]; }
+#pragma unroll
+        for (int k = 0; k < 3; ++k) { lu[3 * i + k] = u[k]; ld[3 * i + k] = n[k] - u[k]; }
+        if (i < P.tile_rows + ns) {
+#pragma unroll
+            for (int k = 0; k < 3; ++k) lx[3 * i + k] = P.lin_xl[a + k] + (P.X0 ? P.X0[a + k] : 0.0);
+        }
+    }
+}
+template <int T, bool DF, bool TPC = false, bool H4 = false, bool RCS = false, bool RCD = false, bool NT = false, bool TD = false>
 __device__ __forceinline__ void spmv_f_body(const Dev& P, const double lam, const int cls, const int it, const double tol2, const int blk) {
     static_assert(!(RCS || RCD) || (TPC && H4 && !DF), "factor recomputation: plain windows with cached partners and 4-byte headers");
+    static_assert(!TD || (TPC && H4 && !RCS && !RCD && T == 2), "two-incidence dampers: the h4 path with stored factors");
     __shared__ double lds[4 * 9];
     extern __shared__ double dyn[];
     constexpr int R = 64 / T;
@@ -183,19 +203,22 @@
     const bool rfix = (P.rflag[row] & RF_FIXED) != 0;
     const uint32_t tp = TPC ? P.row_tp[row] : 0u;
     const uint32_t rcn = TPC ? P.row_cnt[row] : 0u;
-    const int my_s = ((int)(rcn & 0xFFFFu) + T - 1 - t) / T, my_d = ((int)(rcn >> 16) + T - 1 - t) / T;
+    const int my_s = ((int)(rcn & 0xFFFFu) + T - 1 - t) / T, my_d = ((int)(TD ? P.td_cnt[row] : rcn >> 16) + T - 1 - t) / T;
     const int kf = P.grp_pose[row / ROW_ALIGN];
     const int sbeg = P.ss_ptr[slice], send = rfix ? sbeg : P.ss_ptr[slice + 1];
-    const int dbeg = P.sd_ptr[slice], dend = rfix ? dbeg : P.sd_ptr[slice + 1];
-    const size_t nst = (size_t)(P.tile_rows + P.cap_h[cls] + 1);
+    const int dend_s = TD ? P.td_end[slice] : P.sd_ptr[slice + 1];
+    const int dbeg = P.sd_ptr[slice], dend = rfix ? dbeg : dend_s;
+    const int hcap = TD ? P.td_cap : P.cap_h[cls];
+    const size_t nst = (size_t)(P.tile_rows + hcap + 1);
     double* lu = dyn;
     double* lgf = dyn + 3 * nst;
     double* lgb = dyn + 6 * nst;
-    double* lx = dyn + (DF ? 9 : 3) * nst;
-    const int ZROW = P.tile_rows + P.cap_h[cls], ZROWX = RCD ? ZROW : P.tile_rows + P.cap_s[cls];
+    double* lx = dyn + (DF ? 9 : TD ? 6 : 3) * nst;
+    const int ZROW = P.tile_rows + hcap, ZROWX = RCD ? ZROW : P.tile_rows + P.cap_s[cls];
     if (tid < 3) {
         lu[3 * ZROW + tid] = 0; lx[3 * ZROWX + tid] = 0;
         if (DF) { lgf[3 * ZROW + tid] = 0; lgb[3 * ZROW + tid] = 0; }
+        if (TD) lgf[3 * ZROW + tid] = 0;
     }
     double gsum = 0;
     if (P.ecd) {
@@ -217,7 +240,8 @@
             const size_t r = 3 * (size_t)(i < P.tile_rows ? row0 + i : P.halo_rows[hb + i - P.tile_rows]);
             lx[3 * i] = P.lin_xl[r]; lx[3 * i + 1] = P.lin_xl[r + 1]; lx[3 * i + 2] = P.lin_xl[r + 2];
         }
-    } else stage_rows2<TPC, RCD>(P, b, tid, P.uv3, P.lin_xl, P.X0, lu, lx);
+    } else if (TD) stage_rows_td(P, b, tid, lu, lgf, lx);
+    else stage_rows2<TPC, RCD>(P, b, tid, P.uv3, P.lin_xl, P.X0, lu, lx);
     RowRec rc;
     rc.w = 0;
     double rv0 = 0, rv1 = 0, rv2 = 0;
@@ -225,7 +249,7 @@
         rc = P.rowrec[row];
         if (!P.ecd) { rv0 = P.rv[3 * row]; rv1 = P.rv[3 * row + 1]; rv2 = P.rv[3 * row + 2]; }
     }
-    const int send_u = P.ss_ptr[slice + 1], dend_u = P.sd_ptr[slice + 1];
+    const int send_u = P.ss_ptr[slice + 1], dend_u = dend_s;
     const int s_last = max(send_u - 1, 0), d_last = max(dend_u - 1, 0);
     uint32_t somA[U], somB[U], sd0A[U], sd0B[U];
     double sqcA[U], sqcB[U], dsA[U], dsB[U];
@@ -253,6 +277,9 @@
             if (TPC) {
                 h[q] = make_uint2(0xFFFFFFFFu, 0xFFFFFFFFu); sv[q] = 0.0;
                 if (H4 && RCD) { if ((idx + 64 * q - dbeg - lane) / 64 < my_d) { h[q].x = P.d_h4[idx + 64 * q]; h[q].y = __float_as_uint(P.d_w[idx + 64 * q]); } }
+                else if (TD) { if ((idx + 64 * q - dbeg - lane) / 64 < my_d) {
+                    if (NT) { h[q].x = __builtin_nontemporal_load(P.td_h + idx + 64 * q); sv[q] = __builtin_nontemporal_load(P.td_s + idx + 64 * q); }
+                    else { h[q].x = P.td_h[idx + 64 * q]; sv[q] = P.td_s[idx + 64 * q]; } } }
                 else if (H4) { if ((idx + 64 * q - dbeg - lane) / 64 < my_d) {
                     if (NT) { h[q].x = __builtin_nontemporal_load(P.d_h4 + idx + 64 * q); sv[q] = __builtin_nontemporal_load(P.d_s + idx + 64 * q); }
                     else { h[q].x = P.d_h4[idx + 64 * q]; sv[q] = P.d_s[idx + 64 * q]; } } }
@@ -291,7 +318,8 @@
     double a0 = 0, a1 = 0, a2 = 0;
     double en[3] = {0, 0, 0}, ep[3] = {0, 0, 0}, exn[3] = {0, 0, 0}, exq[3] = {0, 0, 0};
     const double ks = P.k_spring, ip = P.info_pos, isp = P.info_spatial;
-    if (TPC) {
+    const double dl[3] = {TD ? lgf[3 * self] : 0.0, TD ? lgf[3 * self + 1] : 0.0, TD ? lgf[3 * self + 2] : 0.0};
+    if (TPC && !TD) {
         const int tn = (int)(tp & 0xFFFFu) == REC_NONE ? ZROW : (int)(tp & 0xFFFFu), tq = (int)(tp >> 16) == REC_NONE ? ZROW : (int)(tp >> 16);
 #pragma unroll
         for (int k = 0; k < 3; ++k) { en[k] = ul[k] - lu[3 * tn + k]; ep[k] = ul[k] - lu[3 * tq + k]; }
@@ -314,6 +342,7 @@
             a0 += dot * v0; a1 += dot * v1; a2 += dot * v2;
         }
     };
+    double hd0 = 0, hd1 = 0, hd2 = 0;
     const double gfo[3] = {DF ? lgf[3 * self] : 0.0, DF ? lgf[3 * self + 1] : 0.0, DF ? lgf[3 * self + 2] : 0.0};
     const double gbo[3] = {DF ? lgb[3 * self] : 0.0, DF ? lgb[3 * self + 1] : 0.0, DF ? lgb[3 * self + 2] : 0.0};
     auto do_dampers = [&](const uint2* hd, const double* dsv, int idx) {
@@ -342,6 +371,13 @@
             const int o1 = (un || r1 == REC_NONE) ? ZROW : r1;
             const int o2 = H4 ? (pad ? ZROW : r2) : (un || r2 == REC_NONE) ? ZROW : r2;
             double g0, g1, g2;
+            if (TD) {
+                g0 = lgf[3 * o0] - dl[0];
+                g1 = lgf[3 * o0 + 1] - dl[1];
+                g2 = lgf[3 * o0 + 2] - dl[2];
+                hd0 += sv * g0; hd1 += sv * g1; hd2 += sv * g2;
+                continue;
+            }
             if (TPC) {
                 const bool fwd = (m16 & 2) == 0;
                 g0 = (fwd ? en[0] : ep[0]) - (lu[3 * o0] - lu[3 * o2]);
@@ -394,18 +430,27 @@
         }
     }
     a0 = sub_sum_t<T>(a0); a1 = sub_sum_t<T>(a1); a2 = sub_sum_t<T>(a2);
+    if (TD) { hd0 = sub_sum_t<T>(hd0); hd1 = sub_sum_t<T>(hd1); hd2 = sub_sum_t<T>(hd2); }
     if (t == 0) {
+        if (TD) { a0 += hd0; a1 += hd1; a2 += hd2; }
         P.wv[3 * row] = a0; P.wv[3 * row + 1] = a1; P.wv[3 * row + 2] = a2;
         part[0] = P.ecd ? 0.0 : rv0 * ul[0] + rv1 * ul[1] + rv2 * ul[2];
         part[1] = a0 * ul[0] + a1 * ul[1] + a2 * ul[2];
+        if (TD) {
+            const int nx = P.td_nxt[row];
+            if (nx >= 0) {
+                P.hn[3 * (size_t)nx] = -hd0; P.hn[3 * (size_t)nx + 1] = -hd1; P.hn[3 * (size_t)nx + 2] = -hd2;
+                part[1] -= hd0 * (ul[0] + dl[0]) + hd1 * (ul[1] + dl[1]) + hd2 * (ul[2] + dl[2]);
+            }
+        }
     }
     stamp(4);
     block_sum_store<9>(part, lds, tid, P.part_spmv + (size_t)b * NPART);
     stamp(5);
 }
-template <int T, bool DF, bool TPC = false, bool H4 = false, bool RCS = false, bool RCD = false, bool NT = false>
+template <int T, bool DF, bool TPC = false, bool H4 = false, bool RCS = false, bool RCD = false, bool NT = false, bool TD = false>
 __global__ __launch_bounds__(BLK, RCD ? 3 : 4) void k_spmv_f(Dev P, double lam, int cls, int it, double tol2) {
-    spmv_f_body<T, DF, TPC, H4, RCS, RCD, NT>(P, lam, cls, it, tol2, (int)blockIdx.x);
+    spmv_f_body<T, DF, TPC, H4, RCS, RCD, NT, TD>(P, lam, cls, it, tol2, (int)blockIdx.x);
 }
 
 __global__ __launch_bounds__(BLK) void k_reduce_ru(Dev P, int it) {
@@ -491,7 +536,8 @@
     const int sk_r = P.sh_vb0 * BLK + (int)blockIdx.x * SK_RPB + tid / SK_RL, sk_t = tid % SK_RL;
     const bool has_rows = SKR ? row_wg && sk_t == 0 : row_wg && 2 * pair < (P.sh_vb0 + n_vecblk) * BLK;
     const size_t o = SKR ? 3 * (size_t)sk_r : 6 * (size_t)pair;
-    double uu[6], pp[6], ww[6], ss[6], rr[6], xx[6], Di[12];
+    double uu[6], pp[6], ww[6], ss[6], rr[6], xx[6], Di[12], hh[6];
+    const bool td = !SKR && P.td;
     double ska[3] = {0, 0, 0};
     bool sk_add = false;
     if (SKR) {
@@ -522,6 +568,13 @@
             uu[2 * k] = a.x; uu[2 * k + 1] = a.y; pp[2 * k] = b.x; pp[2 * k + 1] = b.y;
             ww[2 * k] = c.x; ww[2 * k + 1] = c.y; ss[2 * k] = d.x; ss[2 * k + 1] = d.y;
             rr[2 * k] = e.x; rr[2 * k + 1] = e.y; xx[2 * k] = f.x; xx[2 * k + 1] = f.y;
+        }
+        if (td) {
+#pragma unroll
+            for (int k = 0; k < 3; ++k) {
+                const double2 h = *reinterpret_cast<const double2*>(P.hn + o + 2 * k);
+                hh[2 * k] = h.x; hh[2 * k + 1] = h.y;
+            }
         }
 #pragma unroll
         for (int k = 0; k < 6; ++k) {
@@ -639,7 +692,7 @@
 #pragma unroll
             for (int k = 0; k < 6; ++k) {
                 pp[k] = uu[k] + beta * pp[k];
-                ss[k] = ww[k] + beta * ss[k];
+                ss[k] = (td ? ww[k] + hh[k] : ww[k]) + beta * ss[k];
                 xx[k] += alpha * pp[k];
                 rr[k] -= alpha * ss[k];
             }
diff --git a/nr-slam_amd/csrc/nrs_engine_setup.hpp b/nr-slam_amd/csrc/nrs_engine_setup.hpp
--- a/nr-slam_amd/csrc/nrs_engine_setup.hpp
+++ b/nr-slam_amd/csrc/nrs_engine_setup.hpp
@@ -66,6 +66,12 @@
     const bool on = !e->nd && !d.fused && !d.coarse && !d.sh_on && n_skin == 0 && !c->opt.profile && (long)d.n_rows <= max_rows;
     e->spec_pcg = on;
     e->n_spec = on ? spec_sets(c) : 0;
+}
+
+static inline bool h4_carved(const Dev& d) { return d.plain && d.use_lds && !d.fused; }
+static inline bool td_carved(const Dev& d, size_t nnz_s, size_t nnz_d) { return h4_carved(d) && !d.sh_on && 12 * (nnz_s + nnz_d) <= ((size_t)128 << 20); }
+static inline bool h4_shape(const Dev& d) {
+    return h4_carved(d) && d.tp_ok && d.T == 2 && d.tile_rows + std::max(d.cap_h[0], d.cap_h[1]) + 2 < 4096 && d.sd_nnz > 0;
 }
 
 static void carve(ArenaPlan& A, Dev& d, bool has_X0, size_t nnz_s, size_t nnz_d, size_t n_slices, size_t n_halo, Engine* e) {
@@ -103,7 +109,15 @@
     d.rowrec = d.use_lds ? A.get_rows<RowRec>(1) : A.get<RowRec>(1);
     d.row_tp = d.plain ? A.get_rows<uint32_t>(1) : A.get<uint32_t>(1);
     d.row_cnt = d.plain ? A.get_rows<uint32_t>(1) : A.get<uint32_t>(1);
-    d.d_h4 = A.get<uint32_t>(d.plain && d.use_lds && !d.fused ? nnz_d : 1);
+    d.d_h4 = A.get<uint32_t>(h4_carved(d) ? nnz_d : 1);
+    {
+        const bool td = td_carved(d, nnz_s, nnz_d);
+        d.td_h = A.get<uint32_t>(td ? nnz_d : 1); d.td_s = A.get<double>(td ? nnz_d : 1); d.td_pos = A.get<int>(td ? nnz_d : 1);
+        d.td_end = A.get<int>(td ? n_slices : 1); d.td_cnt = A.get<uint32_t>(td ? nr : 1); d.td_nxt = A.get<int>(td ? nr : 1);
+        d.hn = A.get<double>(td ? 3 * nr : 1);
+        const size_t ntl = td ? (size_t)d.n_regblk * (size_t)std::max(1, d.max_halo) : 1;
+        d.td_rows = A.get<int>(ntl); d.td_rnx = A.get<int>(ntl); d.td_nh = A.get<int>(td ? (size_t)d.n_regblk : 1);
+    }
     d.s_g = A.get<double>(3 * us);
     d.d_s = A.get<double>(nnz_d);
     d.Hpp = A.get<double>(21 * K);
@@ -155,11 +169,12 @@
         q.part_apply = A.get<double>((size_t)d.n_vecblk); q.part_rchi = A.get<double>((size_t)d.n_groups); q.part_reg = A.get<double>(2 * (size_t)d.n_regblk);
         q.scal = A.get<double>(SC_N); q.flags = A.get<int>(8); q.abort = A.get<int>(1);
         q.sk_part = q.sk_chi = nullptr;
-        q.rv = q.uv3 = q.pv = q.sv = q.wv = q.Dinv = q.Hppinv = q.rp = q.rp2 = q.up = q.up2 = q.pp = q.sp = nullptr;
+        q.rv = q.uv3 = q.pv = q.sv = q.wv = q.hn = q.Dinv = q.Hppinv = q.rp = q.rp2 = q.up = q.up2 = q.pp = q.sp = nullptr;
         q.part_spmv = q.part_ru = q.red = q.part_ec = nullptr;
         if (!e->spec_pcg) continue;
         double** rows[] = {&q.rv, &q.uv3, &q.pv, &q.sv, &q.wv};
         for (auto p : rows) *p = A.get_rows<double>(3);
+        q.hn = A.get<double>(td_carved(d, nnz_s, nnz_d) ? 3 * nr : 1);
         q.Dinv = A.get_rows<double>(6);
         q.Hppinv = A.get<double>(36 * K);
         double** poses[] = {&q.rp, &q.rp2, &q.up, &q.up2, &q.pp, &q.sp};
@@ -203,13 +218,114 @@
 static void engine_compact_headers(nrs_ctx* c, Engine* e) {
     Dev& d = e->d;
     d.h4 = 0; d.rc = 0; d.nt = 0;
-    if (!(d.plain && d.tp_ok && d.use_lds && !d.fused && d.T == 2) || c->env("NRS_NO_H4")) return;
-    if (d.tile_rows + std::max(d.cap_h[0], d.cap_h[1]) + 2 >= 4096 || d.sd_nnz <= 0) return;
+    if (!h4_shape(d) || c->env("NRS_NO_H4")) return;
     hipLaunchKernelGGL(k_compact_headers, dim3((unsigned)(((size_t)d.sd_nnz + 255) / 256)), dim3(256), 0, c->stream, (size_t)d.sd_nnz, d.d_hdr, d.d_h4);
     d.h4 = 1;
     if (const char* v = c->env("NRS_RC")) d.rc = atoi(v) & 3;
     d.nt = 12 * ((size_t)d.ss_nnz + (size_t)d.sd_nnz) > ((size_t)128 << 20);
     if (const char* v = c->env("NRS_NT")) d.nt = atoi(v) != 0;
+}
+
+__global__ __launch_bounds__(32) void k_td_derive(Dev P, int* fail) {
+    __shared__ int smax;
+    constexpr int T = 2, R = 32;
+    const int slice = blockIdx.x, rl = threadIdx.x, row = slice * R + rl;
+    if (rl == 0) smax = 0;
+    __syncthreads();
+    const int beg = P.sd_ptr[slice];
+    const int nd = (int)(P.row_cnt[row] >> 16);
+    int nc = 0;
+    for (int j = 0; j < nd; ++j) {
+        const int idx = beg + 64 * (j / T) + rl * T + j % T;
+        const uint2 h8 = P.d_hdr[idx];
+        const uint32_t m16 = h8.y >> 16;
+        const uint32_t h = m16 == REC_NONE ? 0xFFFFFFFFu : ((h8.x & 0xFFFu) | ((h8.y & 0xFFFu) << 12) | ((m16 & 0xFFu) << 24));
+        if (h == 0xFFFFFFFFu || ((h >> 24) & 2u)) continue;
+        const int q = beg + 64 * (nc / T) + rl * T + nc % T;
+        P.td_h[q] = h; P.td_pos[idx] = q; ++nc;
+    }
+    P.td_cnt[row] = (uint32_t)nc;
+    const int b = row / P.tile_rows;
+    auto glob = [&](int tile, int l) { return l < P.tile_rows ? tile * P.tile_rows + l : P.halo_rows[P.halo_ptr[tile] + l - P.tile_rows]; };
+    const uint32_t tp = P.row_tp[row];
+    int nx = -1;
+    if ((tp & 0xFFFFu) != REC_NONE) {
+        nx = glob(b, (int)(tp & 0xFFFFu));
+        const uint32_t tq = P.row_tp[nx];
+        if ((tq >> 16) == REC_NONE || glob(nx / P.tile_rows, (int)(tq >> 16)) != row) atomicOr(fail, 4);
+    } else if (nc > 0) atomicOr(fail, 2);
+    if (nd > 0 && (P.rflag[row] & RF_FIXED)) atomicOr(fail, 1);
+    P.td_nxt[row] = nx;
+    atomicMax(&smax, (nc + T - 1) / T);
+    __syncthreads();
+    if (rl == 0) P.td_end[slice] = beg + 64 * smax;
+}
+__global__ __launch_bounds__(256) void k_td_stage(Dev P, int* cap) {
+    __shared__ int map[4096];
+    __shared__ int nh;
+    const int b = blockIdx.x, tid = threadIdx.x;
+    const int hb = P.halo_ptr[b], hc = P.halo_ptr[b + 1] - hb, ns = P.halo_ns[b], base = P.tile_rows + ns, nloc = P.tile_rows + hc;
+    for (int i = tid; i < nloc; i += BLK) map[i] = 0;
+    __syncthreads();
+    for (int w = 0; w < 4; ++w)
+        for (int idx = P.sd_ptr[4 * b + w] + tid; idx < P.td_end[4 * b + w]; idx += BLK) {
+            const uint32_t h = P.td_h[idx];
+            if (h != 0xFFFFFFFFu && (int)(h & 0xFFFu) >= base) map[h & 0xFFFu] = 1;
+        }
+    __syncthreads();
+    if (tid == 0) {
+        int n = ns;
+        for (int i = base; i < nloc; ++i) if (map[i]) map[i] = P.tile_rows + n++;
+        nh = n;
+        P.td_nh[b] = n;
+        atomicMax(cap, n);
+    }
+    __syncthreads();
+    const size_t so = (size_t)b * P.max_halo;
+    for (int i = tid; i < hc; i += BLK) {
+        const int old = P.tile_rows + i, nw = old < base ? old : map[old];
+        if (old < base || nw > 0) {
+            const int r = P.halo_rows[hb + i];
+            P.td_rows[so + nw - P.tile_rows] = r; P.td_rnx[so + nw - P.tile_rows] = P.td_nxt[r];
+        }
+    }
+    for (int w = 0; w < 4; ++w)
+        for (int idx = P.sd_ptr[4 * b + w] + tid; idx < P.td_end[4 * b + w]; idx += BLK) {
+            const uint32_t h = P.td_h[idx];
+            if (h == 0xFFFFFFFFu) continue;
+            const int o = (int)(h & 0xFFFu), nw = o < base ? o : map[o];
+            P.td_h[idx] = (h & 0xFF000000u) | (uint32_t)nw;
+        }
+    (void)nh;
+}
+static int engine_td_setup(nrs_ctx* c, Engine* e, bool skinned) {
+    Dev& d = e->d;
+    d.td = 0;
+    auto log = [&](int fail) {
+        if (c->env("NRS_TIMING")) fprintf(stderr, "[nrs] two-incidence dampers: %s (h4 %d rc %d sharded %d fused %d dform %d skinned %d derivation %d, staged halo cap %d of %d)\n",
+                                          d.td ? "on" : "off", d.h4, d.rc, d.sh_on, d.fused, d.dform, (int)skinned, fail, d.td_cap, std::max(d.cap_h[0], d.cap_h[1]));
+    };
+    if (!h4_shape(d) || !td_carved(d, (size_t)d.ss_nnz, (size_t)d.sd_nnz) || d.rc || d.dform || skinned || c->env("NRS_NO_TD")) { log(-1); return NRS_OK; }
+    const size_t n_slices = 4 * (size_t)d.n_regblk, nr = (size_t)d.n_rows;
+    NRS_HIP(c, hipMemsetAsync(d.td_h, 0xFF, sizeof(uint32_t) * (size_t)d.sd_nnz, c->stream));
+    NRS_HIP(c, hipMemsetAsync(d.td_pos, 0xFF, sizeof(int) * (size_t)d.sd_nnz, c->stream));
+    NRS_HIP(c, hipMemsetAsync(d.td_s, 0, sizeof(double) * (size_t)d.sd_nnz, c->stream));
+    NRS_HIP(c, hipMemsetAsync(d.hn, 0, sizeof(double) * 3 * nr, c->stream));
+    for (int j = 0; j < e->n_spec; ++j)
+        if (e->spec_pcg) NRS_HIP(c, hipMemsetAsync(e->spec[j].hn, 0, sizeof(double) * 3 * nr, c->stream));
+    NRS_HIP(c, hipMemsetAsync(d.flags, 0, sizeof(int) * 8, c->stream));
+    hipLaunchKernelGGL(k_td_derive, dim3((unsigned)n_slices), dim3(32), 0, c->stream, d, d.flags + 5);
+    hipLaunchKernelGGL(k_td_stage, dim3((unsigned)d.n_regblk), dim3(BLK), 0, c->stream, d, d.flags + 6);
+    NRS_HIP(c, hipGetLastError());
+    int fl[2] = {0, 0};
+    NRS_HIP(c, hipMemcpyAsync(fl, d.flags + 5, sizeof(int) * 2, hipMemcpyDeviceToHost, c->stream));
+    NRS_HIP(c, hipStreamSynchronize(c->stream));
+    NRS_HIP(c, hipMemsetAsync(d.flags, 0, sizeof(int) * 8, c->stream));
+    d.td_cap = fl[1];
+    const int fail = fl[0] | (std::max(td_lds_bytes(d, 0), td_lds_bytes(d, 1)) > 64 * 1024 - 512 ? 8 : 0);
+    d.td = fail ? 0 : 1;
+    log(fail);
+    return NRS_OK;
 }
 
 template <class F>
@@ -1059,6 +1175,7 @@
     e->d.h_flags = c->pin_flags;
     if (e->n_spec > 0) NRS_TRY(spec_prepare(c, e));
     engine_compact_headers(c, e);
+    NRS_TRY(engine_td_setup(c, e, s.n_skin > 0));
     NRS_HIP(c, hipStreamSynchronize(c->stream));
     mark("pinned+sync");
     if (s.n_skin > 0) {
diff --git a/nr-slam_amd/csrc/nrs_engine_types.hpp b/nr-slam_amd/csrc/nrs_engine_types.hpp
--- a/nr-slam_amd/csrc/nrs_engine_types.hpp
+++ b/nr-slam_amd/csrc/nrs_engine_types.hpp
@@ -59,6 +59,16 @@
     int nt;
     uint32_t* d_h4; int h4;
     uint32_t* row_cnt;
+    int td;
+    uint32_t* td_h;
+    double* td_s;
+    int* td_pos;
+    int* td_end;
+    uint32_t* td_cnt;
+    int* td_nxt;
+    int* td_rows; int* td_rnx; int* td_nh;
+    int td_cap;
+    double* hn;
     RowRec* rowrec;
     Pose* lin_pose; double* lin_xl;
     Pose* pose[2]; double* xl[2];
@@ -134,6 +144,7 @@
     double* pk; double* pk_loc;
 };
 
+inline size_t td_lds_bytes(const Dev& d, int cls) { return sizeof(double) * 3 * (size_t)(2 * (d.tile_rows + d.td_cap + 1) + d.tile_rows + d.cap_s[cls] + 1); }
 inline int rc_of(const Dev& d, int cls) {
     if (!(d.rc & 2)) return d.rc;
     return sizeof(double) * 3 * (size_t)(2 * (d.tile_rows + d.cap_h[cls]) + 2) > 64 * 1024 - 512 ? (d.rc & 1) : d.rc;
@@ -150,6 +161,7 @@
     Pose* pose; double* xl;
     double* h_scal; int* h_flags;
     double *rv, *uv3, *pv, *sv, *wv, *Dinv, *Hppinv;
+    double* hn;
     double *rp, *rp2, *up, *up2, *pp, *sp;
     double *part_spmv, *part_ru, *red, *part_ec;
 };
```

Measured after the change: 2088 LM iters/s, median of 6. 1.04x the previous value.
